# bayespy/bayespy

Measured on AMD Instinct MI355X. Metric: VB iterations/sec, PCA N=10000000 D=128 K=32, higher is better.
Workload: dtype f64

## Files before the change

### bayespy_amd/csrc/vmp_common.h

```cpp
#pragma once

#include <hip/hip_runtime.h>
#include <stdint.h>
#include <stdio.h>
#include <string.h>
#include <math.h>

#include "../../include/vmp_hip.h"

#define VMP_EV_RING 64

constexpr int VMP_NME = 16;

struct vmp_xpass_desc {
    const double *Y;
    int64_t ldy, N;
    int D, K;
    double *X;
    int64_t ldx;
    int lay;
    const double *A;
    int buf;
};

struct vmp_ctx {
    int device;
    hipStream_t stream;
    int num_cu;
    int timing;
    hipEvent_t ev[3 * VMP_EV_RING];
    int64_t ev_n;
    hipStream_t xs;
    hipEvent_t ev_xfork, ev_xdone;
    int x_pending;
    hipEvent_t ev_xbuf[2];
    int x_buf_pending[2];
    int64_t x_count;
    int xs_cus;
    int x_hold, x_held;
    vmp_xpass_desc x_desc;
    int64_t x_launched, x_superseded;
    double *sweep_ctl;
    int64_t sweeps_enqueued;
    unsigned int *sweep_tickets;
    int64_t sweep_mid_launches;
    unsigned long long *sweep_stamps;
    int sweep_stamp_rows;
    double *sweep_sf;
    double sweep_sf_key[7];
    int sweep_sf_valid;
    hipStream_t ms[3];
    hipEvent_t me[VMP_NME];
    int gram_pending;
    int gram_D, gram_K;
    double *gram_state;
    double *gram_P;
    void *comm;
    int comm_rank, comm_world;
    void *queue;
    char err[512];
};

enum { VMP_SWEEP_NSTAMP = VMP_PCA_SWEEP_NSTAMP };

enum { VMP_SWEEP_STOP = 0, VMP_SWEEP_L = 1, VMP_SWEEP_EXECUTED = 2, VMP_SWEEP_SKIPPED = 3,
       VMP_SWEEP_CTL_LEN = 8 };

enum { VMP_SWEEP_SF_TAU = 0, VMP_SWEEP_SF_ALPHA = 4, VMP_SWEEP_SF_LOG2PI = 8, VMP_SWEEP_SF_LOGXPREC = 9,
       VMP_SWEEP_SF_LEN = 10 };

struct vmp_sweep_tail {
    const double *P;
    int nb;
    double *ctl;
    double *slot;
    int first;
    int compare;
    double l0, tol;
    int norder;
    int order[8];
};

int32_t vmp_pca_sweep_covered(int32_t D, int32_t K);
int32_t vmp_pca_launch_sweep_head(vmp_ctx *ctx, int32_t D, int32_t K, int64_t n_total, double x_prec,
                                  double a0t, double b0t, double a0a, double b0a, double *state,
                                  const double *stop);
int32_t vmp_pca_launch_sweep_tail(vmp_ctx *ctx, int32_t D, int32_t K, int64_t n_total, double x_prec,
                                  double a0t, double b0t, double a0a, double b0a, double *state,
                                  const vmp_sweep_tail &t);

int32_t vmp_pca_launch_sweep_mid(vmp_ctx *ctx, int32_t D, int32_t K, int64_t n_total, double x_prec,
                                 double a0t, double b0t, double a0a, double b0a, double *state,
                                 double *P, const vmp_sweep_tail &t, unsigned int *ticket,
                                 unsigned long long *stamps, int32_t stamp_level);
int32_t vmp_pca_sweep_constants(vmp_ctx *ctx, int32_t D, int32_t K, int64_t n_total, double x_prec,
                                double a0t, double b0t, double a0a, double b0a);
int32_t vmp_pca_launch_sweep_head_wide(vmp_ctx *ctx, int32_t D, int32_t K, int64_t n_total,
                                       double x_prec, double a0t, double b0t, double a0a, double b0a,
                                       double *state);
int32_t vmp_pca_launch_gram_fast(vmp_ctx *ctx, int32_t D, int32_t K, double *state);

int32_t vmp_pca_ensure_gram(vmp_ctx *ctx);
int32_t vmp_pca_launch_held(vmp_ctx *ctx);

int32_t vmp_queue_flush(vmp_ctx *ctx);
int32_t vmp_queue_commit(vmp_ctx *ctx);
int32_t destroy_small_queue(vmp_ctx *ctx);
extern const char *vmp_flush_cause;
#define VMP_FLUSH_SMALL(ctx)                                   \
    do {                                                       \
        if ((ctx) && (ctx)->queue) {                           \
            vmp_flush_cause = __func__;                        \
            const int32_t rc__ = vmp_queue_flush(ctx);         \
            if (rc__ != VMP_OK) return rc__;                   \
        }                                                      \
    } while (0)

static inline hipEvent_t *vmp_next_events(vmp_ctx *ctx)
{
    hipEvent_t *e = ctx->ev + 3 * (ctx->ev_n % VMP_EV_RING);
    ctx->ev_n += 1;
    return e;
}

#define VMP_SET_ERR(ctx, ...)                                         \
    do {                                                              \
        if (ctx) snprintf((ctx)->err, sizeof((ctx)->err), __VA_ARGS__); \
    } while (0)

#define VMP_HIP_CHECK(ctx, expr)                                                   \
    do {                                                                           \
        hipError_t e__ = (expr);                                                   \
        if (e__ != hipSuccess) {                                                   \
            VMP_SET_ERR(ctx, "%s failed: %s (%s:%d)", #expr, hipGetErrorString(e__), \
                        __FILE__, __LINE__);                                       \
            return VMP_ERR_HIP;                                                    \
        }                                                                          \
    } while (0)

#define VMP_REQUIRE(ctx, cond, code, ...)   \
    do {                                    \
        if (!(cond)) {                      \
            VMP_SET_ERR(ctx, __VA_ARGS__);  \
            return (code);                  \
        }                                   \
    } while (0)

int vmp_tune_get(const char *key, int dflt);

typedef double v4f64 __attribute__((ext_vector_type(4)));
typedef double v2f64 __attribute__((ext_vector_type(2)));

int32_t vmp_launch_spd_mfma(vmp_ctx *ctx, bool moments, int32_t n, int64_t batch, const double *A,
                            const double *rhs, double *Ainv, double *vec_out, double *logdet,
                            int32_t *info);


__host__ __device__ inline double vmp_digamma(double x)
{
    if (!(x > 0.0)) {
        if (x == 0.0) return -INFINITY;
        double r = 1.0 - x;
        double s = 0.0;
        while (r < 10.0) { s -= 1.0 / r; r += 1.0; }
        double inv = 1.0 / r, inv2 = inv * inv;
        double ser = inv2 * (1.0 / 12 - inv2 * (1.0 / 120 - inv2 * (1.0 / 252 - inv2 * (1.0 / 240 - inv2 * (1.0 / 132 - inv2 * (691.0 / 32760 - inv2 * (1.0 / 12)))))));
        double psi1mx = s + log(r) - 0.5 * inv - ser;
        return psi1mx - M_PI / tan(M_PI * x);
    }
    double s = 0.0;
    while (x < 10.0) { s -= 1.0 / x; x += 1.0; }
    double inv = 1.0 / x, inv2 = inv * inv;
    double ser = inv2 * (1.0 / 12 - inv2 * (1.0 / 120 - inv2 * (1.0 / 252 - inv2 * (1.0 / 240 - inv2 * (1.0 / 132 - inv2 * (691.0 / 32760 - inv2 * (1.0 / 12)))))));
    return s + log(x) - 0.5 * inv - ser;
}

__host__ __device__ inline double vmp_lgamma(double x)
{
    if (!(x > 0.0)) return INFINITY;
    double shift = 0.0;
    double prod = 1.0;
    while (x < 10.0) {
        prod *= x;
        x += 1.0;
        if (prod > 1e150) { shift += log(prod); prod = 1.0; }
    }
    shift += log(prod);
    double inv = 1.0 / x, inv2 = inv * inv;
    double ser = inv * (1.0 / 12 - inv2 * (1.0 / 360 - inv2 * (1.0 / 1260 - inv2 * (1.0 / 1680 - inv2 * (1.0 / 1188 - inv2 * (691.0 / 360360 - inv2 * (1.0 / 156)))))));
    return (x - 0.5) * log(x) - x + 0.91893853320467274178 + ser - shift;
}

#if defined(__clang__)
#define VMP_NO_CONTRACT _Pragma("clang fp contract(off)")
#else
#define VMP_NO_CONTRACT
#endif

__host__ __device__ inline double vmp_two_sum(double a, double b, double *e)
{
    VMP_NO_CONTRACT
    const double s = a + b, bb = s - a;
    *e = (a - (s - bb)) + (b - bb);
    return s;
}

__host__ __device__ inline double vmp_lgamma_dd(double x, double dx, double *lo)
{
    VMP_NO_CONTRACT
    if (!(x >= 10.0) || !(x < 4e15)) {
        *lo = dx == 0.0 ? 0.0 : dx * vmp_digamma(x);
        return vmp_lgamma(x);
    }
    int e;
    double m = frexp(x, &e);
    if (m < 0.70710678118654752440) { m *= 2.0; e -= 1; }
    const double A = (double)e * 6.93147180369123816490e-01;
    const double B = (double)e * 1.90821492927058770002e-10 + log(m);
    const double w = x - 0.5;
    const double p = w * A, pe = fma(w, A, -p);
    const double q = w * B, qe = fma(w, B, -q);
    double e1, e2;
    const double s1 = vmp_two_sum(p, -x, &e1);
    const double s2 = vmp_two_sum(s1, q, &e2);
    const double inv = 1.0 / x, inv2 = inv * inv;
    const double ser = inv * (1.0 / 12 - inv2 * (1.0 / 360 - inv2 * (1.0 / 1260 - inv2 * (1.0 / 1680 - inv2 * (1.0 / 1188 - inv2 * (691.0 / 360360 - inv2 * (1.0 / 156)))))));
    const double small = ((pe + qe) + (e1 + e2)) + (0.91893853320467274178 + ser)
                         + dx * ((A + B) - 0.5 * inv);
    return vmp_two_sum(s2, small, lo);
}

__host__ __device__ inline double vmp_trigamma(double x)
{
    if (!(x > 0.0)) return (x == 0.0) ? INFINITY : NAN;
    double s = 0.0;
    while (x < 10.0) { s += 1.0 / (x * x); x += 1.0; }
    double inv = 1.0 / x, inv2 = inv * inv;
    double ser = inv * inv2 * (1.0 / 6 - inv2 * (1.0 / 30 - inv2 * (1.0 / 42 - inv2 * (1.0 / 30 - inv2 * (5.0 / 66 - inv2 * (691.0 / 2730 - inv2 * (7.0 / 6)))))));
    return s + inv + 0.5 * inv2 + ser;
}

__host__ __device__ inline double vmp_invpsi(double x)
{
    const double psi1 = -0.57721566490153286061;
    double y = x >= -2.22 ? exp(x) + 0.5 : -1.0 / (x - psi1);
    for (int i = 0; i < 5; ++i) y = y - (vmp_digamma(y) - x) / vmp_trigamma(y);
    return y;
}

#ifdef __HIPCC__
__device__ inline void logdet_accumulate(double piv, double &prod, double &ld)
{
    prod *= piv;
    if (!(prod < 1e120 && prod > 1e-120)) {
        ld += log(prod);
        prod = 1.0;
    }
}

__device__ inline double logdet_finish(double prod, double ld) { return ld + log(prod); }

__device__ inline double fast_recip(double x)
{
    double r = __builtin_amdgcn_rcp(x);
    r = r * (2.0 - x * r);
    r = r * (2.0 - x * r);
    return r;
}

__device__ inline void lds_fence()
{
    asm volatile("s_waitcnt lgkmcnt(0)" ::: "memory");
}


__device__ inline double wave_spd_inverse(double v, int D, int i, int j, bool act, double *M,
                                          double *logdet, int *bad)
{
    double ld = 0.0, prod = 1.0;
    const int l = threadIdx.x & 63;
    for (int p = 0; p < D; ++p) {
        M[l] = v;
        lds_fence();
        const double piv = M[p * D + p];
        const double ci = act ? M[i * D + p] : 0.0, rj = act ? M[p * D + j] : 0.0;
        if (!(piv > 0.0)) *bad = 1;
        logdet_accumulate(piv, prod, ld);
        const double d = fast_recip(piv);
        if (i == p) v = (j == p) ? d : rj * d;
        else if (j == p) v = -ci * d;
        else v = v - ci * rj * d;
        lds_fence();
    }
    *logdet = logdet_finish(prod, ld);
    return v;
}

__device__ __forceinline__ double exp_nonpos(double x)
{
    x = fmax(x, -800.0);
    const double k = __builtin_rint(x * 1.4426950408889634074);
    double r = __builtin_fma(k, -6.93147180369123816490e-01, x);
    r = __builtin_fma(k, -1.90821492927058770002e-10, r);
    double p = 1.0 / 479001600.0;
    p = __builtin_fma(p, r, 1.0 / 39916800.0);
    p = __builtin_fma(p, r, 1.0 / 3628800.0);
    p = __builtin_fma(p, r, 1.0 / 362880.0);
    p = __builtin_fma(p, r, 1.0 / 40320.0);
    p = __builtin_fma(p, r, 1.0 / 5040.0);
    p = __builtin_fma(p, r, 1.0 / 720.0);
    p = __builtin_fma(p, r, 1.0 / 120.0);
    p = __builtin_fma(p, r, 1.0 / 24.0);
    p = __builtin_fma(p, r, 1.0 / 6.0);
    p = __builtin_fma(p, r, 0.5);
    p = __builtin_fma(p, r, 1.0);
    p = __builtin_fma(p, r, 1.0);
    return __builtin_ldexp(p, (int)k);
}

__device__ inline double wave_sum(double v)
{
#pragma unroll
    for (int off = 32; off > 0; off >>= 1) v += __shfl_down(v, off, 64);
    return v;
}

template <int NT>
__device__ inline double block_sum(double v, double *red)
{
    v = wave_sum(v);
    __syncthreads();
    if ((threadIdx.x & 63) == 0) red[threadIdx.x >> 6] = v;
    __syncthreads();
    double s = 0.0;
#pragma unroll
    for (int i = 0; i < NT / 64; ++i) s += red[i];
    return s;
}

__device__ __forceinline__ double group16_max(double v)
{
#pragma unroll
    for (int off = 8; off > 0; off >>= 1) v = fmax(v, __shfl_xor(v, off, 16));
    return v;
}

__device__ __forceinline__ double group16_sum(double v)
{
#pragma unroll
    for (int off = 8; off > 0; off >>= 1) v += __shfl_xor(v, off, 16);
    return v;
}

template <int NT>
__device__ __forceinline__ void block_halve_sum(double *v, int tid)
{
    for (int off = NT / 2; off > 0; off >>= 1) {
        if (tid < off) v[tid] += v[tid + off];
        __syncthreads();
    }
}

struct PmmArgs {
    int64_t N, chunk;
    int D, K;
    const uint16_t *x;
    const int32_t *labels;
    const double *l, *lb;
    const double *c;
    double *part;
    double *r_out;
};

void vmp_pmm_launch_pass(vmp_ctx *ctx, int64_t nc, bool hidden, const PmmArgs &a);
#endif
```

### bayespy_amd/csrc/vmp_ctx.hip

```cpp
#include "vmp_common.h"

#include <new>

static char g_err[512] = "no context";

namespace {
struct tune_entry { char key[32]; int value; };
tune_entry g_tune[128];
int g_ntune = 0;
bool g_tune_env = false;
}

extern "C" char **environ;

static void tune_from_env()
{
    g_tune_env = true;
    for (char **e = environ; e && *e; ++e) {
        if (strncmp(*e, "VMP_TUNE_", 9) != 0) continue;
        const char *eq = strchr(*e, '=');
        if (!eq) continue;
        const size_t len = (size_t)(eq - (*e + 9));
        if (len == 0 || len >= sizeof(g_tune[0].key) || g_ntune >= (int)(sizeof(g_tune) / sizeof(g_tune[0])))
            continue;
        memcpy(g_tune[g_ntune].key, *e + 9, len);
        g_tune[g_ntune].key[len] = 0;
        g_tune[g_ntune].value = atoi(eq + 1);
        g_ntune += 1;
    }
}

int vmp_tune_get(const char *key, int dflt)
{
    if (!g_tune_env) tune_from_env();
    for (int i = 0; i < g_ntune; ++i)
        if (strcmp(g_tune[i].key, key) == 0) return g_tune[i].value;
    return dflt;
}

extern "C" {

int32_t vmp_tune_set(const char *key, int32_t value)
{
    if (!key || strlen(key) >= sizeof(g_tune[0].key)) return VMP_ERR_INVALID;
    if (!g_tune_env) tune_from_env();
    for (int i = 0; i < g_ntune; ++i)
        if (strcmp(g_tune[i].key, key) == 0) {
            g_tune[i].value = value;
            return VMP_OK;
        }
    if (g_ntune >= (int)(sizeof(g_tune) / sizeof(g_tune[0]))) return VMP_ERR_INVALID;
    strcpy(g_tune[g_ntune].key, key);
    g_tune[g_ntune].value = value;
    g_ntune += 1;
    return VMP_OK;
}

#ifndef VMP_BUILD_ID
#define VMP_BUILD_ID "unknown"
#endif
const char *vmp_version(void) { return "libvmp_hip 0.2 (gfx950) build " VMP_BUILD_ID; }

int32_t vmp_ctx_create(int32_t device, void *stream, vmp_ctx **out)
{
    if (!out) return VMP_ERR_INVALID;
    *out = nullptr;
    int ndev = 0;
    hipError_t e = hipGetDeviceCount(&ndev);
    if (e != hipSuccess || ndev <= 0) {
        snprintf(g_err, sizeof(g_err), "no HIP device visible (%s)", hipGetErrorString(e));
        return VMP_ERR_HIP;
    }
    if (device < 0 || device >= ndev) {
        snprintf(g_err, sizeof(g_err), "device %d out of range [0,%d)", device, ndev);
        return VMP_ERR_INVALID;
    }
    vmp_ctx *ctx = new (std::nothrow) vmp_ctx();
    if (!ctx) return VMP_ERR_HIP;
    ctx->device = device;
    ctx->stream = (hipStream_t)stream;
    ctx->timing = 0;
    ctx->err[0] = 0;
    for (int i = 0; i < 3 * VMP_EV_RING; ++i) ctx->ev[i] = nullptr;
    ctx->ev_n = 0;
    ctx->xs = nullptr;
    ctx->ev_xfork = ctx->ev_xdone = nullptr;
    ctx->x_pending = 0;
    ctx->x_buf_pending[0] = ctx->x_buf_pending[1] = 0;
    ctx->x_count = 0;
    ctx->ev_xbuf[0] = ctx->ev_xbuf[1] = nullptr;
    ctx->xs_cus = 0;
    ctx->x_hold = ctx->x_held = 0;
    ctx->x_launched = ctx->x_superseded = 0;
    ctx->sweep_ctl = nullptr;
    ctx->sweeps_enqueued = 0;
    ctx->sweep_tickets = nullptr;
    ctx->sweep_mid_launches = 0;
    ctx->sweep_stamps = nullptr;
    ctx->sweep_stamp_rows = 0;
    ctx->sweep_sf = nullptr;
    ctx->sweep_sf_valid = 0;
    for (int i = 0; i < 3; ++i) ctx->ms[i] = nullptr;
    for (int i = 0; i < VMP_NME; ++i) ctx->me[i] = nullptr;
    ctx->comm = nullptr;
    ctx->queue = nullptr;
    ctx->comm_rank = 0;
    ctx->comm_world = 1;
    VMP_HIP_CHECK(ctx, hipSetDevice(device));
    int cu = 0;
    VMP_HIP_CHECK(ctx, hipDeviceGetAttribute(&cu, hipDeviceAttributeMultiprocessorCount, device));
    ctx->num_cu = cu > 0 ? cu : 256;
    *out = ctx;
    return VMP_OK;
}

int32_t vmp_ctx_destroy(vmp_ctx *ctx)
{
    if (!ctx) return VMP_OK;
    (void)destroy_small_queue(ctx);
    (void)vmp_comm_destroy(ctx);
    (void)vmp_pca_launch_held(ctx);
    for (int i = 0; i < 3 * VMP_EV_RING; ++i)
        if (ctx->ev[i]) (void)hipEventDestroy(ctx->ev[i]);
    if (ctx->xs) {
        (void)hipStreamSynchronize(ctx->xs);
        (void)hipStreamDestroy(ctx->xs);
    }
    for (int i = 0; i < 3; ++i)
        if (ctx->ms[i]) {
            (void)hipStreamSynchronize(ctx->ms[i]);
            (void)hipStreamDestroy(ctx->ms[i]);
        }
    for (int i = 0; i < VMP_NME; ++i)
        if (ctx->me[i]) (void)hipEventDestroy(ctx->me[i]);
    if (ctx->sweep_ctl) (void)hipFree(ctx->sweep_ctl);
    if (ctx->sweep_tickets) (void)hipFree(ctx->sweep_tickets);
    if (ctx->sweep_stamps) (void)hipFree(ctx->sweep_stamps);
    if (ctx->sweep_sf) (void)hipFree(ctx->sweep_sf);
    if (ctx->ev_xfork) (void)hipEventDestroy(ctx->ev_xfork);
    if (ctx->ev_xdone) (void)hipEventDestroy(ctx->ev_xdone);
    for (int i = 0; i < 2; ++i)
        if (ctx->ev_xbuf[i]) (void)hipEventDestroy(ctx->ev_xbuf[i]);
    delete ctx;
    return VMP_OK;
}

int32_t vmp_ctx_set_stream(vmp_ctx *ctx, void *stream)
{
    if (!ctx) return VMP_ERR_INVALID;
    if ((hipStream_t)stream != ctx->stream) VMP_FLUSH_SMALL(ctx);
    ctx->stream = (hipStream_t)stream;
    return VMP_OK;
}

int32_t vmp_ctx_sync(vmp_ctx *ctx)
{
    if (!ctx) return VMP_ERR_INVALID;
    VMP_FLUSH_SMALL(ctx);
    {
        const int32_t rcg = vmp_pca_ensure_gram(ctx);
        if (rcg != VMP_OK) return rcg;
        const int32_t rch = vmp_pca_launch_held(ctx);
        if (rch != VMP_OK) return rch;
    }
    VMP_HIP_CHECK(ctx, hipStreamSynchronize(ctx->stream));
    if (ctx->xs) VMP_HIP_CHECK(ctx, hipStreamSynchronize(ctx->xs));
    for (int i = 0; i < 3; ++i)
        if (ctx->ms[i]) VMP_HIP_CHECK(ctx, hipStreamSynchronize(ctx->ms[i]));
    return VMP_OK;
}

int32_t vmp_ctx_num_cu(vmp_ctx *ctx) { return ctx ? ctx->num_cu : 0; }

struct vmp_graph {
    hipGraph_t graph;
    hipGraphExec_t exec;
};

int32_t vmp_graph_begin(vmp_ctx *ctx)
{
    VMP_REQUIRE(ctx, ctx, VMP_ERR_INVALID, "null context");
    VMP_REQUIRE(ctx, ctx->stream != nullptr, VMP_ERR_INVALID,
                "the legacy default stream cannot record: give the context a stream of its own");
    VMP_FLUSH_SMALL(ctx);
    VMP_HIP_CHECK(ctx, hipStreamBeginCapture(ctx->stream, hipStreamCaptureModeThreadLocal));
    return VMP_OK;
}

int32_t vmp_graph_end(vmp_ctx *ctx, void **graph)
{
    VMP_REQUIRE(ctx, ctx && graph, VMP_ERR_INVALID, "null argument");
    *graph = nullptr;
    const int32_t rcq = vmp_queue_flush(ctx);
    hipGraph_t g = nullptr;
    hipError_t e = hipStreamEndCapture(ctx->stream, &g);
    if (rcq != VMP_OK) {
        if (g) (void)hipGraphDestroy(g);
        return rcq;
    }
    VMP_HIP_CHECK(ctx, e);
    hipGraphExec_t x = nullptr;
    e = hipGraphInstantiate(&x, g, nullptr, nullptr, 0);
    if (e != hipSuccess) {
        (void)hipGraphDestroy(g);
        VMP_HIP_CHECK(ctx, e);
    }
    const int32_t rcc = vmp_queue_commit(ctx);
    if (rcc != VMP_OK) {
        (void)hipGraphExecDestroy(x);
        (void)hipGraphDestroy(g);
        return rcc;
    }
    vmp_graph *h = new (std::nothrow) vmp_graph{g, x};
    if (!h) {
        (void)hipGraphExecDestroy(x);
        (void)hipGraphDestroy(g);
        VMP_REQUIRE(ctx, false, VMP_ERR_HIP, "out of host memory");
    }
    *graph = h;
    return VMP_OK;
}

int32_t vmp_graph_launch(vmp_ctx *ctx, void *graph)
{
    VMP_REQUIRE(ctx, ctx && graph, VMP_ERR_INVALID, "null argument");
    VMP_FLUSH_SMALL(ctx);
    VMP_HIP_CHECK(ctx, hipGraphLaunch(reinterpret_cast<vmp_graph *>(graph)->exec, ctx->stream));
    return VMP_OK;
}

int32_t vmp_graph_destroy(vmp_ctx *ctx, void *graph)
{
    (void)ctx;
    if (!graph) return VMP_OK;
    vmp_graph *h = reinterpret_cast<vmp_graph *>(graph);
    (void)hipGraphExecDestroy(h->exec);
    (void)hipGraphDestroy(h->graph);
    delete h;
    return VMP_OK;
}

const char *vmp_last_error(vmp_ctx *ctx) { return ctx ? ctx->err : g_err; }

int32_t vmp_ctx_set_timing(vmp_ctx *ctx, int32_t enabled)
{
    if (!ctx) return VMP_ERR_INVALID;
    if (enabled && !ctx->ev[0]) {
        VMP_HIP_CHECK(ctx, hipSetDevice(ctx->device));
        for (int i = 0; i < 3 * VMP_EV_RING; ++i) VMP_HIP_CHECK(ctx, hipEventCreate(&ctx->ev[i]));
    }
    ctx->timing = enabled ? 1 : 0;
    ctx->ev_n = 0;
    return VMP_OK;
}

int32_t vmp_pass_times_ms(vmp_ctx *ctx, double *ms_pass, double *ms_reduce, int32_t cap,
                          int32_t *count)
{
    VMP_REQUIRE(ctx, ctx && count && cap >= 0, VMP_ERR_INVALID, "null argument");
    VMP_REQUIRE(ctx, ctx->timing && ctx->ev[0], VMP_ERR_INVALID,
                "timing not enabled (vmp_ctx_set_timing)");
    {
        const int32_t rch = vmp_pca_launch_held(ctx);
        if (rch != VMP_OK) return rch;
    }
    int64_t n = ctx->ev_n < VMP_EV_RING ? ctx->ev_n : VMP_EV_RING;
    if (n > cap) n = cap;
    for (int64_t i = 0; i < n; ++i) {
        hipEvent_t *e = ctx->ev + 3 * ((ctx->ev_n - n + i) % VMP_EV_RING);
        VMP_HIP_CHECK(ctx, hipEventSynchronize(e[2]));
        float a = 0.f, b = 0.f;
        VMP_HIP_CHECK(ctx, hipEventElapsedTime(&a, e[0], e[1]));
        VMP_HIP_CHECK(ctx, hipEventElapsedTime(&b, e[1], e[2]));
        if (ms_pass) ms_pass[i] = a;
        if (ms_reduce) ms_reduce[i] = b;
    }
    *count = (int32_t)n;
    ctx->ev_n = 0;
    return VMP_OK;
}

int32_t vmp_malloc(vmp_ctx *ctx, size_t bytes, void **ptr)
{
    if (!ctx || !ptr) return VMP_ERR_INVALID;
    VMP_HIP_CHECK(ctx, hipSetDevice(ctx->device));
    VMP_HIP_CHECK(ctx, hipMalloc(ptr, bytes ? bytes : 8));
    return VMP_OK;
}

int32_t vmp_free(vmp_ctx *ctx, void *ptr)
{
    if (!ctx) return VMP_ERR_INVALID;
    if (ptr) VMP_HIP_CHECK(ctx, hipFree(ptr));
    return VMP_OK;
}

int32_t vmp_memcpy_h2d(vmp_ctx *ctx, void *dst, const void *src, size_t bytes)
{
    VMP_FLUSH_SMALL(ctx);
    if (!ctx) return VMP_ERR_INVALID;
    VMP_HIP_CHECK(ctx, hipMemcpyAsync(dst, src, bytes, hipMemcpyHostToDevice, ctx->stream));
    VMP_HIP_CHECK(ctx, hipStreamSynchronize(ctx->stream));
    return VMP_OK;
}

int32_t vmp_memcpy_d2h(vmp_ctx *ctx, void *dst, const void *src, size_t bytes)
{
    VMP_FLUSH_SMALL(ctx);
    if (!ctx) return VMP_ERR_INVALID;
    VMP_HIP_CHECK(ctx, hipMemcpyAsync(dst, src, bytes, hipMemcpyDeviceToHost, ctx->stream));
    VMP_HIP_CHECK(ctx, hipStreamSynchronize(ctx->stream));
    return VMP_OK;
}

int32_t vmp_memset_zero(vmp_ctx *ctx, void *dst, size_t bytes)
{
    VMP_FLUSH_SMALL(ctx);
    if (!ctx) return VMP_ERR_INVALID;
    VMP_HIP_CHECK(ctx, hipMemsetAsync(dst, 0, bytes, ctx->stream));
    return VMP_OK;
}

struct CopyMany {
    const double *src[24];
    double *dst[24];
    int64_t count[24];
};

__global__ void __launch_bounds__(256) copy_many_kernel(CopyMany a)
{
    const int c = blockIdx.y;
    const double *s = a.src[c];
    double *d = a.dst[c];
    const int64_t n = a.count[c];
    for (int64_t i = (int64_t)blockIdx.x * 256 + threadIdx.x; i < n; i += (int64_t)gridDim.x * 256)
        d[i] = s[i];
}

int32_t vmp_copy_many(vmp_ctx *ctx, int32_t n, const double *const *src, double *const *dst,
                      const int64_t *count)
{
    VMP_REQUIRE(ctx, ctx != nullptr, VMP_ERR_INVALID, "null context");
    VMP_REQUIRE(ctx, n >= 0 && (n == 0 || (src && dst && count)), VMP_ERR_INVALID, "null argument");
    VMP_FLUSH_SMALL(ctx);
    for (int32_t b = 0; b < n; b += 24) {
        CopyMany a;
        memset(&a, 0, sizeof(a));
        const int m = (n - b) < 24 ? (n - b) : 24;
        int64_t most = 0;
        for (int i = 0; i < m; ++i) {
            a.src[i] = src[b + i];
            a.dst[i] = dst[b + i];
            a.count[i] = count[b + i];
            VMP_REQUIRE(ctx, a.count[i] >= 0 && (a.count[i] == 0 || (a.src[i] && a.dst[i])),
                        VMP_ERR_INVALID, "vmp_copy_many: bad entry %d", b + i);
            if (a.count[i] > most) most = a.count[i];
        }
        int64_t gx = (most + 1023) / 1024;
        if (gx < 1) gx = 1;
        if (gx > 1024) gx = 1024;
        hipLaunchKernelGGL(copy_many_kernel, dim3((unsigned)gx, (unsigned)m), dim3(256), 0,
                           ctx->stream, a);
        VMP_HIP_CHECK(ctx, hipGetLastError());
    }
    return VMP_OK;
}

struct PackArgs {
    const void *src[48];
    int64_t count[48];
    int32_t kind[48];
};

__global__ void __launch_bounds__(64) pack_outputs_kernel(PackArgs a, double *__restrict__ out,
                                                           int base)
{
    const int e = blockIdx.x;
    const int kind = a.kind[e];
    if (kind == 0) {
        if (threadIdx.x == 0) out[base + e] = *reinterpret_cast<const double *>(a.src[e]);
        return;
    }
    int bad = 0;
    const int64_t n = a.count[e];
    if (kind == 1) {
        const int32_t *f = reinterpret_cast<const int32_t *>(a.src[e]);
        for (int64_t i = threadIdx.x; i < n; i += 64) bad |= (f[i] != 0);
    } else {
        const double *f = reinterpret_cast<const double *>(a.src[e]);
        for (int64_t i = threadIdx.x; i < n; i += 64) bad |= (f[i] != 0.0);
    }
    const unsigned long long m = __ballot(bad);
    if (threadIdx.x == 0) out[base + e] = m ? 1.0 : 0.0;
}

int32_t vmp_pack_outputs(vmp_ctx *ctx, int32_t n, const void *const *src, const int64_t *count,
                         const int32_t *kind, double *out)
{
    VMP_REQUIRE(ctx, ctx != nullptr, VMP_ERR_INVALID, "null context");
    VMP_REQUIRE(ctx, n >= 0 && (n == 0 || (src && count && kind && out)), VMP_ERR_INVALID,
                "null argument");
    VMP_FLUSH_SMALL(ctx);
    for (int32_t b = 0; b < n; b += 48) {
        PackArgs a;
        memset(&a, 0, sizeof(a));
        const int m = (n - b) < 48 ? (n - b) : 48;
        for (int i = 0; i < m; ++i) {
            a.src[i] = src[b + i];
            a.count[i] = count[b + i];
            a.kind[i] = kind[b + i];
            VMP_REQUIRE(ctx, a.src[i] && a.kind[i] >= 0 && a.kind[i] <= 2 && a.count[i] >= 0,
                        VMP_ERR_INVALID, "vmp_pack_outputs: bad entry %d", b + i);
        }
        hipLaunchKernelGGL(pack_outputs_kernel, dim3((unsigned)m), dim3(64), 0, ctx->stream, a, out,
                           (int)b);
        VMP_HIP_CHECK(ctx, hipGetLastError());
    }
    return VMP_OK;
}

}
```

### bayespy_amd/csrc/vmp_pca.hip

```cpp
#include "vmp_common.h"
#include "vmp_stop_rule.h"

namespace {

constexpr int TN = 32;
constexpr int SZ = TN + 2;
constexpr int NT = 256;
constexpr int MAX_KP = 64;
constexpr int MAX_DP = 256;

inline int pow2_blocks(int x, int unit)
{
    int b = (x + unit - 1) / unit;
    int p = 1;
    while (p < b) p <<= 1;
    return p;
}

inline void fill_layout(int D, int K, vmp_pca_layout *L)
{
    const int64_t DP = 32 * pow2_blocks(D, 32);
    const int64_t KP = 16 * pow2_blocks(K, 16);
    int64_t o = 0;
    L->DP = DP;
    L->KP = KP;
    L->off_S = o;      L->len_S = (DP + KP) * KP; o += L->len_S;
    L->off_Syy = o;    o += 8;
    L->off_tau = o;    o += 8;
    L->off_alpha = o;  o += 4 * KP;
    L->off_W = o;      o += (int64_t)D * KP;
    L->off_CW = o;     o += KP * KP;
    L->off_Sww = o;    o += KP * KP;
    L->off_CX = o;     o += KP * KP;
    L->off_A = o;      o += KP * DP;
    L->off_G = o;      o += DP * DP;
    L->off_scal = o;   o += 8;
    L->off_L = o;      o += 8;
    L->off_mu = o;     o += (int64_t)D * KP;
    L->off_mstat = o;  o += 2 * KP;
    L->total = (o + 7) / 8 * 8;
}

__device__ inline v4f64 mfma_f64(double a, double b, v4f64 c)
{
    return __builtin_amdgcn_mfma_f64_16x16x4f64(a, b, c, 0, 0, 0);
}

template <int DB, int KT, bool COMPUTE_X>
__global__ void __launch_bounds__(NT, (DB >= 8 || DB * KT > 8) ? 1 : 2)
pca_pass_kernel(const double *__restrict__ Y, int64_t ldy, int64_t N, int D, int K,
                const double *__restrict__ Apad, double *__restrict__ X, int64_t ldx,
                double *__restrict__ P, int64_t ntiles)
{
    constexpr int DP = 32 * DB, KP = 16 * KT, ZR = DP + KP;
    constexpr int YP = DP / 16;
    constexpr int XP = KP / 16;
    constexpr int KS1 = DP / 4;
    constexpr int T1 = KT * (TN / 16);
    constexpr int R1 = (T1 + 3) / 4;
    constexpr int T2 = (2 * DB + KT) * KT;
    constexpr int R2 = (T2 + 3) / 4;

    __shared__ double Z[ZR * SZ];

    const int tid = threadIdx.x;
    const int w = tid >> 6, l = tid & 63;
    const int l15 = l & 15, l4 = l >> 4;
    const int lrow = tid >> 4;
    const int lcol = (tid & 15) * 2;
    const int it1 = w % KT;
    const int jt2 = w % KT;

    double afrag[COMPUTE_X ? KS1 : 1];
    if (COMPUTE_X) {
        const double *arow = Apad + (int64_t)(it1 * 16 + l15) * DP;
#pragma unroll
        for (int q = 0; q < KS1; ++q) afrag[q] = arow[32 * (q >> 3) + (q & 7) + 8 * l4];
    }

    v4f64 acc2[R2];
#pragma unroll
    for (int m = 0; m < R2; ++m) acc2[m] = v4f64{0.0, 0.0, 0.0, 0.0};

    v2f64 yreg[YP];

    auto load_tile = [&](int64_t tile) {
        const int64_t n = tile * TN + lcol;
#pragma unroll
        for (int p = 0; p < YP; ++p) {
            const int row = p * 16 + lrow;
            v2f64 v = v2f64{0.0, 0.0};
            if (row < D) {
                const double *src = Y + (int64_t)row * ldy + n;
                if (n + 1 < N) v = *reinterpret_cast<const v2f64 *>(src);
                else if (n < N) v.x = src[0];
            }
            yreg[p] = v;
        }
    };

    int64_t tile = blockIdx.x;
    if (tile < ntiles) load_tile(tile);

    for (; tile < ntiles; tile += gridDim.x) {
        const int64_t n0 = tile * TN;
#pragma unroll
        for (int p = 0; p < YP; ++p)
            *reinterpret_cast<v2f64 *>(&Z[(p * 16 + lrow) * SZ + lcol]) = yreg[p];
        if (!COMPUTE_X) {
#pragma unroll
            for (int p = 0; p < XP; ++p) {
                const int row = p * 16 + lrow;
                const int64_t n = n0 + lcol;
                v2f64 v = v2f64{0.0, 0.0};
                if (row < K) {
                    const double *src = X + (int64_t)row * ldx + n;
                    if (n + 1 < N) { v.x = src[0]; v.y = src[1]; }
                    else if (n < N) v.x = src[0];
                }
                *reinterpret_cast<v2f64 *>(&Z[(DP + row) * SZ + lcol]) = v;
            }
        }
        __syncthreads();

        const int64_t next = tile + gridDim.x;
        if (next < ntiles) load_tile(next);

        if (COMPUTE_X) {
#pragma unroll
            for (int m = 0; m < R1; ++m) {
                const int t1 = w + 4 * m;
                if (t1 < T1) {
                    const int jt = t1 / KT;
                    const double *zb = Z + jt * 16 + l15 + 8 * l4 * SZ;
                    v4f64 c0 = v4f64{0.0, 0.0, 0.0, 0.0};
                    v4f64 c1 = v4f64{0.0, 0.0, 0.0, 0.0};
#pragma unroll
                    for (int q = 0; q < KS1; q += 2) {
                        const double b0 = zb[(32 * (q >> 3) + (q & 7)) * SZ];
                        const double b1 = zb[(32 * ((q + 1) >> 3) + ((q + 1) & 7)) * SZ];
                        c0 = mfma_f64(afrag[q], b0, c0);
                        c1 = mfma_f64(afrag[q + 1], b1, c1);
                    }
                    c0 += c1;
                    const int n = jt * 16 + l15;
                    const bool nok = (n0 + n) < N;
#pragma unroll
                    for (int r = 0; r < 4; ++r) {
                        const int k = it1 * 16 + l4 + 4 * r;
                        Z[(DP + k) * SZ + n] = c0[r];
                        if (nok && k < K) X[(int64_t)k * ldx + n0 + n] = c0[r];
                    }
                }
            }
            __syncthreads();
        }

        {
            const double *zbB = Z + (DP + jt2 * 16 + l15) * SZ + l4;
            const double *zbA = Z + l15 * SZ + l4;
#pragma unroll
            for (int q = 0; q < TN / 4; ++q) {
                const double b = zbB[4 * q];
#pragma unroll
                for (int m = 0; m < R2; ++m) {
                    const int t2 = w + 4 * m;
                    if (t2 < T2) {
                        const int it2 = t2 / KT;
                        const double a = zbA[it2 * 16 * SZ + 4 * q];
                        acc2[m] = mfma_f64(a, b, acc2[m]);
                    }
                }
            }
        }
        __syncthreads();
    }

    double *Pb = P + (int64_t)blockIdx.x * (ZR * KP);
#pragma unroll
    for (int m = 0; m < R2; ++m) {
        const int t2 = w + 4 * m;
        if (t2 < T2) {
            const int it2 = t2 / KT;
#pragma unroll
            for (int r = 0; r < 4; ++r) {
                const int row = it2 * 16 + l4 + 4 * r;
                Pb[row * KP + jt2 * 16 + l15] = acc2[m][r];
            }
        }
    }
}

__global__ void __launch_bounds__(NT)
reduce_partials_kernel(const double *__restrict__ P, int nb, int len, double *__restrict__ S)
{
    const int e = blockIdx.x * NT + threadIdx.x;
    if (e >= len) return;
    double s0 = 0.0, s1 = 0.0, s2 = 0.0, s3 = 0.0;
    int b = 0;
    for (; b + 3 < nb; b += 4) {
        s0 += P[(int64_t)b * len + e];
        s1 += P[(int64_t)(b + 1) * len + e];
        s2 += P[(int64_t)(b + 2) * len + e];
        s3 += P[(int64_t)(b + 3) * len + e];
    }
    for (; b < nb; ++b) s0 += P[(int64_t)b * len + e];
    S[e] = (s0 + s1) + (s2 + s3);
}

__global__ void __launch_bounds__(NT)
sumsq_kernel(const double *__restrict__ Y, int64_t ldy, int64_t N, int D,
             double *__restrict__ partial)
{
    __shared__ double red[NT / 64];
    double s = 0.0;
    const int64_t npairs = (N + 1) / 2;
    const int64_t total = npairs * D;
    for (int64_t i = (int64_t)blockIdx.x * NT + threadIdx.x; i < total;
         i += (int64_t)gridDim.x * NT) {
        const int64_t d = i / npairs;
        const int64_t n = (i - d * npairs) * 2;
        const double *src = Y + d * ldy + n;
        if (n + 1 < N) {
            const v2f64 v = *reinterpret_cast<const v2f64 *>(src);
            s += v.x * v.x + v.y * v.y;
        } else {
            s += src[0] * src[0];
        }
    }
    s = block_sum<NT>(s, red);
    if (threadIdx.x == 0) partial[blockIdx.x] = s;
}

__global__ void __launch_bounds__(NT)
sum_partials_kernel(const double *__restrict__ partial, int n, double *__restrict__ out)
{
    __shared__ double red[NT / 64];
    double s = 0.0;
    for (int i = threadIdx.x; i < n; i += NT) s += partial[i];
    s = block_sum<NT>(s, red);
    if (threadIdx.x == 0) out[0] = s;
}

constexpr int xpass_occ(int DB, int KT, int OCC)
{
    return KT * DB * 4096 > 80 * 1024 ? 1 : (KT * DB * 4096 > 53 * 1024 ? (OCC < 2 ? OCC : 2) : OCC);
}

template <int DB, int KT, bool GUARD, int OCC, int NTM = 0, int LAY = 0, int MF = 0, bool IL = false>
__global__ void __launch_bounds__(NT, xpass_occ(DB, KT, OCC))
pca_xpass_kernel(const double *__restrict__ Y, int64_t ldy, int64_t N, int D, int K,
                 const double *__restrict__ Apad, double *__restrict__ X, int64_t ldx,
                 int64_t tile0, int64_t tile1)
{
    constexpr int DP = 32 * DB;
    constexpr int KS = DP / 4;
    constexpr int NCH = (DB < 2) ? 2 : DB;
    constexpr int CH = KS / NCH;
    constexpr bool YT = (LAY & 1) != 0, XT = (LAY & 2) != 0;
    static_assert(!(GUARD && LAY != 0), "tile-major arrays are padded: no guarded instance");

    __shared__ double Af[KT * KS * 64];

    const int tid = threadIdx.x;
    const int l = tid & 63;
    const int l15 = l & 15, l4 = l >> 4;
    const int w = __builtin_amdgcn_readfirstlane(tid >> 6);

    for (int e = tid; e < KT * KS * 64; e += NT) {
        const int lane = e & 63, fq = e >> 6;
        const int it = fq / KS, q = fq - it * KS;
        Af[e] = Apad[(int64_t)(it * 16 + (lane & 15)) * DP + 4 * q + (lane >> 4)];
    }
    __syncthreads();

    const double *Afl = MF ? Af + 16 * l4 + (l & 3) : Af + l;
    const uint32_t yoff = (uint32_t)(((int64_t)l4 * ldy + 2 * l15) * 8);
    const uint32_t xoff = (uint32_t)(((int64_t)l4 * ldx + 2 * l15) * 8);

    v2f64 buf[2][CH];
    const int64_t stride = (int64_t)gridDim.x * 4;

    auto issue = [&](int64_t tile, int c, v2f64 *dst) {
        if (YT) {
            const char *base = reinterpret_cast<const char *>(Y)
                               + ((tile * ((DP + (IL ? 16 * KT : 0)) * TN)
                                   + (int64_t)(c * CH) * (4 * TN)) << 3);
#pragma unroll
            for (int i = 0; i < CH; ++i) {
                const v2f64 *src = reinterpret_cast<const v2f64 *>(base + i * (4 * TN * 8) + l * 16);
                dst[i] = (NTM & 1) ? __builtin_nontemporal_load(src) : *src;
            }
            return;
        }
        const char *base = reinterpret_cast<const char *>(Y)
                           + ((tile * TN + (int64_t)(4 * c * CH) * ldy) << 3);
        if (!GUARD) {
#pragma unroll
            for (int i = 0; i < CH; ++i) {
                const v2f64 *src = reinterpret_cast<const v2f64 *>(
                    base + ((int64_t)(4 * i) * ldy << 3) + yoff);
                dst[i] = (NTM & 1) ? __builtin_nontemporal_load(src) : *src;
            }
        } else {
            const int64_t n = tile * TN + 2 * l15;
#pragma unroll
            for (int i = 0; i < CH; ++i) {
                const int row = 4 * (c * CH + i) + l4;
                v2f64 v = v2f64{0.0, 0.0};
                if (row < D) {
                    const double *src = reinterpret_cast<const double *>(
                        base + ((int64_t)(4 * i) * ldy << 3) + yoff);
                    if (n + 1 < N) v = *reinterpret_cast<const v2f64 *>(src);
                    else if (n < N) v.x = src[0];
                }
                dst[i] = v;
            }
        }
    };

    constexpr bool STG = false;
    auto first_chunk = [&](int64_t t) { return STG ? (int)(t & (NCH - 1)) : 0; };
    int64_t tile = tile0 + (int64_t)blockIdx.x * 4 + w;
    if (tile < tile1) issue(tile, first_chunk(tile), buf[0]);

    for (; tile < tile1; tile += stride) {
        v4f64 acc[KT][2];
#pragma unroll
        for (int it = 0; it < KT; ++it) {
            acc[it][0] = v4f64{0.0, 0.0, 0.0, 0.0};
            acc[it][1] = v4f64{0.0, 0.0, 0.0, 0.0};
        }
        const int rot = first_chunk(tile);
#pragma unroll
        for (int c = 0; c < NCH; ++c) {
            const int cc = STG ? ((c + rot) & (NCH - 1)) : c;
            if (c + 1 < NCH) issue(tile, STG ? ((c + 1 + rot) & (NCH - 1)) : c + 1, buf[(c + 1) & 1]);
            else if (tile + stride < tile1) issue(tile + stride, first_chunk(tile + stride), buf[(c + 1) & 1]);
            asm volatile("" ::: "memory");
            const double *Afc = Afl + cc * (CH * 64);
#pragma unroll
            for (int i = 0; i < CH; ++i) {
                const v2f64 b = buf[c & 1][i];
#pragma unroll
                for (int it = 0; it < KT; ++it) {
                    if (MF) {
#pragma unroll
                        for (int R = 0; R < 4; ++R) {
                            const double a = Afc[(it * KS + i) * 64 + 4 * R];
                            acc[it][0][R] = __builtin_amdgcn_mfma_f64_4x4x4f64(a, b.x, acc[it][0][R], 0, 0, 0);
                            acc[it][1][R] = __builtin_amdgcn_mfma_f64_4x4x4f64(a, b.y, acc[it][1][R], 0, 0, 0);
                        }
                    } else {
                        const double a = Afc[(it * KS + i) * 64];
                        acc[it][0] = mfma_f64(a, b.x, acc[it][0]);
                        acc[it][1] = mfma_f64(a, b.y, acc[it][1]);
                    }
                }
            }
        }
        char *xbase = reinterpret_cast<char *>(X) + ((tile * TN) << 3);
        if (XT) {
            char *xt = reinterpret_cast<char *>(X)
                       + ((tile * (((IL ? DP : 0) + 16 * KT) * TN)) << 3) + l * 16;
#pragma unroll
            for (int it = 0; it < KT; ++it)
#pragma unroll
                for (int r = 0; r < 4; ++r) {
                    v2f64 *dstp = reinterpret_cast<v2f64 *>(xt + (it * 16 + 4 * r) * (TN * 8));
                    const v2f64 val = v2f64{acc[it][0][r], acc[it][1][r]};
                    if (NTM & 2) __builtin_nontemporal_store(val, dstp);
                    else *dstp = val;
                }
        } else if (!GUARD) {
#pragma unroll
            for (int it = 0; it < KT; ++it)
#pragma unroll
                for (int r = 0; r < 4; ++r) {
                    v2f64 *dstp = reinterpret_cast<v2f64 *>(
                        xbase + ((int64_t)(it * 16 + 4 * r) * ldx << 3) + xoff);
                    const v2f64 val = v2f64{acc[it][0][r], acc[it][1][r]};
                    if (NTM & 2) __builtin_nontemporal_store(val, dstp);
                    else *dstp = val;
                }
        } else {
            const int64_t n = tile * TN + 2 * l15;
#pragma unroll
            for (int it = 0; it < KT; ++it) {
#pragma unroll
                for (int r = 0; r < 4; ++r) {
                    const int k = it * 16 + l4 + 4 * r;
                    if (k < K) {
                        double *dst = reinterpret_cast<double *>(
                            xbase + ((int64_t)(it * 16 + 4 * r) * ldx << 3) + xoff);
                        if (n + 1 < N)
                            *reinterpret_cast<v2f64 *>(dst) = v2f64{acc[it][0][r], acc[it][1][r]};
                        else if (n < N)
                            dst[0] = acc[it][0][r];
                    }
                }
            }
        }
    }
}

constexpr int LD = MAX_KP + 1;

__global__ void __launch_bounds__(NT)
pca_init_state_kernel(vmp_pca_layout L, int K, double a0t, double b0t, double a0a, double b0a,
                      double *st)
{
    const int tid = threadIdx.x;
    if (tid == 0) {
        st[L.off_tau + 0] = a0t;
        st[L.off_tau + 1] = b0t;
        st[L.off_tau + 2] = a0t / b0t;
        st[L.off_tau + 3] = vmp_digamma(a0t) - log(b0t);
    }
    for (int k = tid; k < K; k += NT) {
        st[L.off_alpha + 0 * L.KP + k] = a0a;
        st[L.off_alpha + 1 * L.KP + k] = b0a;
        st[L.off_alpha + 2 * L.KP + k] = a0a / b0a;
        st[L.off_alpha + 3 * L.KP + k] = vmp_digamma(a0a) - log(b0a);
    }
}

constexpr int GR = 8;
__global__ void __launch_bounds__(NT)
pca_gram_stats_kernel(vmp_pca_layout L, int D, int K, const double *__restrict__ st_in,
                      double *__restrict__ st, double *__restrict__ P, const double *stop)
{
    extern __shared__ double lds[];
    if (stop && stop[VMP_SWEEP_STOP] != 0.0) return;
    const int DP = (int)L.DP, KP = (int)L.KP;
    const int LA = DP + 1;
    double *As = lds;
    double *Gs = As + KP * LA;
    double *Ss = Gs + GR * DP;
    const int tid = threadIdx.x;
    const int r0 = blockIdx.x * GR;
    const double *A = st_in + L.off_A;
    const double *G = st_in + L.off_G;
    for (int e = tid; e < K * DP; e += NT) {
        const int k = e / DP, d = e - k * DP;
        As[k * LA + d] = A[(int64_t)k * DP + d];
    }
    for (int e = tid; e < GR * DP; e += NT) Gs[e] = G[(int64_t)r0 * DP + e];
    __syncthreads();
    for (int e = tid; e < GR * K; e += NT) {
        const int r = e / K, k = e - r * K;
        double s = 0.0;
        for (int d = 0; d < D; ++d) s += Gs[r * DP + d] * As[k * LA + d];
        Ss[r * LD + k] = s;
        if (r0 + r < D) st[L.off_S + (int64_t)(r0 + r) * KP + k] = s;
    }
    __syncthreads();
    double *Pb = P + (int64_t)blockIdx.x * KP * KP;
    for (int e = tid; e < KP * KP; e += NT) {
        const int k = e / KP, k2 = e - k * KP;
        double s = 0.0;
        if (k < K && k2 < K) {
#pragma unroll
            for (int r = 0; r < GR; ++r) s += As[k * LA + r0 + r] * Ss[r * LD + k2];
        }
        Pb[e] = s;
    }
}

__global__ void __launch_bounds__(NT)
pca_gram_copy_kernel(const double *__restrict__ Stmp, int KPx, int D, int Kx, int j0, int DP,
                     double *__restrict__ G)
{
    const int e = blockIdx.x * NT + threadIdx.x;
    if (e >= D * Kx) return;
    const int i = e / Kx, j = e - i * Kx;
    G[(int64_t)i * DP + j0 + j] = Stmp[(int64_t)i * KPx + j];
}

int env_int(const char *name, int dflt, int lo, int hi)
{
    const char *e = getenv(name);
    int v = e ? atoi(e) : dflt;
    if (v < lo) v = lo;
    if (v > hi) v = hi;
    return v;
}

int wgs_per_cu()
{
    static int v = -1;
    if (v < 0) v = env_int("VMP_PCA_WGS_PER_CU", 2, 1, 8);
    return v;
}

int pca_interleave() { return vmp_tune_get("pca_interleave", 0); }

int xpass_wgs_per_cu()
{
    static int v = -1;
    if (v < 0) v = env_int("VMP_PCA_XPASS_WGS_PER_CU", 3, 1, 8);
    return vmp_tune_get("xpass_wgs_per_cu", v);
}

int xpass_occupancy()
{
    static int v = -1;
    if (v < 0) v = env_int("VMP_PCA_XPASS_OCC", 3, 2, 3);
    return vmp_tune_get("xpass_occ", v);
}

int64_t max_grid(vmp_ctx *ctx) { return (int64_t)ctx->num_cu * wgs_per_cu(); }

int64_t partial_len(const vmp_pca_layout &L) { return (L.DP + MAX_KP) * MAX_KP; }

template <int DB, int KT>
void launch_fused(bool compute_x, dim3 grid, hipStream_t s, const double *Y, int64_t ldy,
                  int64_t N, int D, int K, const double *A, double *X, int64_t ldx, double *P,
                  int64_t ntiles)
{
    if (compute_x)
        hipLaunchKernelGGL((pca_pass_kernel<DB, KT, true>), grid, dim3(NT), 0, s, Y, ldy, N, D, K,
                           A, X, ldx, P, ntiles);
    else
        hipLaunchKernelGGL((pca_pass_kernel<DB, KT, false>), grid, dim3(NT), 0, s, Y, ldy, N, D,
                           K, A, X, ldx, P, ntiles);
}

#define VMP_FOR_EACH_INSTANCE(M)                                       \
    M(1, 1) M(2, 1) M(4, 1) M(8, 1) M(1, 2) M(2, 2) M(4, 2) M(8, 2)    \
    M(1, 4) M(2, 4) M(4, 4) M(8, 4)

int32_t check_pass_args(vmp_ctx *ctx, const void *Y, const void *X, const void *state,
                        const void *workspace, int64_t ldy, int64_t ldx, int64_t N, int D, int K)
{
    VMP_REQUIRE(ctx, ctx != nullptr, VMP_ERR_INVALID, "null context");
    VMP_REQUIRE(ctx, Y && X && state && workspace, VMP_ERR_INVALID, "null pointer argument");
    VMP_REQUIRE(ctx, D >= 1 && K >= 1 && N >= 0, VMP_ERR_INVALID, "bad dims D=%d K=%d N=%lld", D,
                K, (long long)N);
    VMP_REQUIRE(ctx, D <= MAX_DP && K <= MAX_KP, VMP_ERR_UNSUPPORTED,
                "fused PCA block supports D <= %d, K <= %d (got D=%d, K=%d)", MAX_DP, MAX_KP, D, K);
    VMP_REQUIRE(ctx, ldy >= N && ldx >= N, VMP_ERR_INVALID, "leading dimension smaller than N");
    VMP_REQUIRE(ctx, (ldy % 2) == 0 && ((uintptr_t)Y % 16) == 0, VMP_ERR_INVALID,
                "Y must be 16-byte aligned with an even leading dimension (ldy=%lld)",
                (long long)ldy);
    VMP_REQUIRE(ctx, (ldx % 2) == 0 && ((uintptr_t)X % 16) == 0, VMP_ERR_INVALID,
                "X must be 16-byte aligned with an even leading dimension (ldx=%lld)",
                (long long)ldx);
    VMP_REQUIRE(ctx, ldy < (int64_t)170000000 && ldx < (int64_t)170000000, VMP_ERR_UNSUPPORTED,
                "leading dimension >= 1.7e8 elements per shard is not supported "
                "(32-bit lane offsets); shard the plate over more ranks");
    return VMP_OK;
}

int32_t run_stats(vmp_ctx *ctx, bool compute_x, const double *Y, int64_t ldy, int64_t N, int D,
                  int Kx, double *Xs, int64_t ldx, const double *A, double *out_S, double *P,
                  bool timed)
{
    vmp_pca_layout Lx;
    fill_layout(D, Kx, &Lx);
    const int DB = (int)(Lx.DP / 32), KT = (int)(Lx.KP / 16);
    const int64_t ntiles = (N + TN - 1) / TN;
    int64_t g = ntiles < max_grid(ctx) ? ntiles : max_grid(ctx);
    if (g < 1) g = 1;
    hipStream_t s = ctx->stream;
    dim3 grid((unsigned)g);
    hipEvent_t *ev = (timed && ctx->timing) ? vmp_next_events(ctx) : nullptr;
    if (ev) VMP_HIP_CHECK(ctx, hipEventRecord(ev[0], s));
#define VMP_CASE(db, kt)                                                                     \
    if (DB == db && KT == kt)                                                                \
        launch_fused<db, kt>(compute_x, grid, s, Y, ldy, N, D, Kx, A, Xs, ldx, P, ntiles);   \
    else
    VMP_FOR_EACH_INSTANCE(VMP_CASE)
    {
        VMP_SET_ERR(ctx, "no kernel instance for DB=%d KT=%d", DB, KT);
        return VMP_ERR_UNSUPPORTED;
    }
#undef VMP_CASE
    VMP_HIP_CHECK(ctx, hipGetLastError());
    if (ev) VMP_HIP_CHECK(ctx, hipEventRecord(ev[1], s));
    const int len = (int)Lx.len_S;
    hipLaunchKernelGGL(reduce_partials_kernel, dim3((len + NT - 1) / NT), dim3(NT), 0, s, P,
                       (int)g, len, out_S);
    VMP_HIP_CHECK(ctx, hipGetLastError());
    if (ev) VMP_HIP_CHECK(ctx, hipEventRecord(ev[2], s));
    return VMP_OK;
}

int32_t ensure_plate_stream(vmp_ctx *ctx)
{
    if (ctx->xs) return VMP_OK;
    static const int reserve = env_int("VMP_PCA_RESERVE_CUS", 0, 0, 64);
    hipStream_t xs = nullptr;
    const int ncu = ctx->num_cu;
    ctx->xs_cus = ncu;
    if (reserve > 0 && ncu > 2 * reserve) {
        const int words = (ncu + 31) / 32;
        uint32_t mask[64];
        for (int w = 0; w < words && w < 64; ++w) mask[w] = 0;
        for (int c = 0; c < ncu; ++c) mask[c >> 5] |= (1u << (c & 31));
        const int step = ncu / reserve;
        for (int r = 0; r < reserve; ++r) {
            const int c = r * step + step / 2;
            mask[c >> 5] &= ~(1u << (c & 31));
        }
        if (hipExtStreamCreateWithCUMask(&xs, (uint32_t)words, mask) != hipSuccess) {
            (void)hipGetLastError();
            xs = nullptr;
        } else {
            ctx->xs_cus = ncu - reserve;
        }
    }
    if (!xs) VMP_HIP_CHECK(ctx, hipStreamCreateWithFlags(&xs, hipStreamNonBlocking));
    ctx->xs = xs;
    VMP_HIP_CHECK(ctx, hipEventCreateWithFlags(&ctx->ev_xfork, hipEventDisableTiming));
    VMP_HIP_CHECK(ctx, hipEventCreateWithFlags(&ctx->ev_xdone, hipEventDisableTiming));
    for (int i = 0; i < 2; ++i)
        VMP_HIP_CHECK(ctx, hipEventCreateWithFlags(&ctx->ev_xbuf[i], hipEventDisableTiming));
    return VMP_OK;
}

int64_t plate_stream_A_offset(vmp_ctx *ctx, const vmp_pca_layout &L)
{
    return (max_grid(ctx) + 1) * partial_len(L) + 4096;
}

double *plate_stream_A(vmp_ctx *ctx, const vmp_pca_layout &L, void *workspace)
{
    return reinterpret_cast<double *>(workspace) + plate_stream_A_offset(ctx, L);
}

int32_t join_plate_stream(vmp_ctx *ctx)
{
    const int32_t rc = vmp_pca_launch_held(ctx);
    if (rc != VMP_OK) return rc;
    if (ctx->x_pending) {
        VMP_HIP_CHECK(ctx, hipStreamWaitEvent(ctx->stream, ctx->ev_xdone, 0));
        ctx->x_pending = 0;
    }
    return VMP_OK;
}

int32_t run_gram_stats(vmp_ctx *ctx, const vmp_pca_layout &L, int D, int K, double *state,
                       double *P, hipStream_t s, const double *stop = nullptr, bool reduce = true)
{
    const int nb = (int)(L.DP / GR);
    const size_t lds = ((size_t)L.KP * (L.DP + 1) + (size_t)GR * L.DP + (size_t)GR * LD)
                       * sizeof(double);
    static bool attr_set = false;
    if (!attr_set) {
        VMP_HIP_CHECK(ctx, hipFuncSetAttribute((const void *)pca_gram_stats_kernel,
                                               hipFuncAttributeMaxDynamicSharedMemorySize,
                                               160 * 1024));
        attr_set = true;
    }
    hipLaunchKernelGGL(pca_gram_stats_kernel, dim3(nb), dim3(NT), lds, s, L, D, K, state, state,
                       P, stop);
    VMP_HIP_CHECK(ctx, hipGetLastError());
    if (!reduce) return VMP_OK;
    const int len = (int)(L.KP * L.KP);
    hipLaunchKernelGGL(reduce_partials_kernel, dim3((len + NT - 1) / NT), dim3(NT), 0, s, P, nb,
                       len, state + L.off_S + L.DP * L.KP);
    VMP_HIP_CHECK(ctx, hipGetLastError());
    return VMP_OK;
}

template <bool TO_TILED>
__global__ void __launch_bounds__(NT)
pca_tile_kernel(double *__restrict__ R, int64_t ld, int64_t N, int rows, int RP,
                double *__restrict__ T, int64_t ntiles, int64_t tstride)
{
    const int tid = threadIdx.x;
    const int c2 = (tid & 15) * 2;
    for (int64_t tile = blockIdx.x; tile < ntiles; tile += gridDim.x) {
        const int64_t n = tile * TN + c2;
        double *tb = T + tile * tstride;
        for (int row = tid >> 4; row < RP; row += NT / 16) {
            double *rp = R + (int64_t)row * ld + n;
            v2f64 *tp = reinterpret_cast<v2f64 *>(tb + row * TN + c2);
            if (TO_TILED) {
                v2f64 v = v2f64{0.0, 0.0};
                if (row < rows) {
                    if (n + 1 < N) v = *reinterpret_cast<const v2f64 *>(rp);
                    else if (n < N) v.x = rp[0];
                }
                *tp = v;
            } else if (row < rows) {
                const v2f64 v = *tp;
                if (n + 1 < N) *reinterpret_cast<v2f64 *>(rp) = v;
                else if (n < N) rp[0] = v.x;
            }
        }
    }
}

int32_t launch_xpass(vmp_ctx *ctx, const vmp_xpass_desc &d, bool on_plate)
{
    const double *Y = d.Y, *A = d.A;
    double *X = d.X;
    const int64_t ldy = d.ldy, N = d.N, ldx = d.ldx;
    const int D = d.D, K = d.K, lay = d.lay;
    vmp_pca_layout L;
    fill_layout(D, K, &L);
    const int DB = (int)(L.DP / 32), KT = (int)(L.KP / 16);
    const int64_t ntiles = (N + TN - 1) / TN;
    const bool exact = (D == L.DP && K == L.KP);
    const bool padded = (ldy >= ntiles * TN && ldx >= ntiles * TN);
    const int64_t nfast = lay ? ntiles : (exact ? (padded ? ntiles : N / TN) : 0);
    const int occ = xpass_occupancy();
    const int ntm = vmp_tune_get("xpass_nt", env_int("VMP_PCA_XPASS_NT", 3, 0, 3));
    const int mf4 = vmp_tune_get("xpass_mfma4", env_int("VMP_PCA_XPASS_MFMA4", 0, 0, 1));
    hipStream_t s = on_plate ? ctx->xs : ctx->stream;
    const int64_t gmax = (int64_t)(on_plate ? ctx->xs_cus : ctx->num_cu) * xpass_wgs_per_cu();
    hipEvent_t *ev = ctx->timing ? vmp_next_events(ctx) : nullptr;
    if (ev) VMP_HIP_CHECK(ctx, hipEventRecord(ev[0], s));
    for (int pass = 0; pass < 2; ++pass) {
        const bool guard = (pass == 1);
        const int64_t t0 = guard ? nfast : 0, t1 = guard ? ntiles : nfast;
        if (t1 <= t0) continue;
        int64_t g = (t1 - t0 + 3) / 4;
        if (g > gmax) g = gmax;
        const dim3 grid((unsigned)g);
#define VMP_XP(db, kt, gd, oc, nt, ly)                                                          \
    hipLaunchKernelGGL((pca_xpass_kernel<db, kt, gd, oc, nt, ly>), grid, dim3(NT), 0, s, Y, ldy, \
                       N, D, K, A, X, ldx, t0, t1)
#define VMP_XP4(db, kt, oc, ly)                                                                  \
    hipLaunchKernelGGL((pca_xpass_kernel<db, kt, false, oc, 3, ly, 1>), grid, dim3(NT), 0, s, Y,  \
                       ldy, N, D, K, A, X, ldx, t0, t1)
        if (lay == 3 && pca_interleave()) {
            if (DB == 4 && KT == 2)
                hipLaunchKernelGGL((pca_xpass_kernel<4, 2, false, 3, 3, 3, 0, true>), grid, dim3(NT),
                                   0, s, Y, ldy, N, D, K, A, X, ldx, t0, t1);
            else if (DB == 2 && KT == 1)
                hipLaunchKernelGGL((pca_xpass_kernel<2, 1, false, 3, 3, 3, 0, true>), grid, dim3(NT),
                                   0, s, Y, ldy, N, D, K, A, X, ldx, t0, t1);
            else {
                VMP_SET_ERR(ctx, "pca_interleave: no instance for DB=%d KT=%d", DB, KT);
                return VMP_ERR_UNSUPPORTED;
            }
            VMP_HIP_CHECK(ctx, hipGetLastError());
            continue;
        }
#define VMP_CASE(db, kt)                                                                        \
    if (DB == db && KT == kt) {                                                                 \
        if (guard) VMP_XP(db, kt, true, 2, 0, 0);                                               \
        else if (mf4 && lay == 1 && ntm == 3) VMP_XP4(db, kt, 2, 1);                            \
        else if (mf4 && lay == 0 && ntm == 3) VMP_XP4(db, kt, 2, 0);                            \
        else if (lay == 3 && kt < 4 && ntm == 3) VMP_XP(db, kt, false, 3, 3, 3);                \
        else if (lay == 3 && kt < 4) VMP_XP(db, kt, false, 3, 0, 3);                            \
        else if (lay == 3) VMP_XP(db, kt, false, 2, 0, 3);                                      \
        else if (lay == 1 && kt < 4 && ntm == 3) VMP_XP(db, kt, false, 3, 3, 1);                \
        else if (lay == 1 && kt < 4) VMP_XP(db, kt, false, 3, 0, 1);                            \
        else if (lay == 1) VMP_XP(db, kt, false, 2, 0, 1);                                      \
        else if (ntm == 3 && kt < 4) VMP_XP(db, kt, false, 3, 3, 0);                            \
        else if (occ >= 3 && kt < 4) VMP_XP(db, kt, false, 3, 0, 0);                            \
        else VMP_XP(db, kt, false, 2, 0, 0);                                                    \
    } else
        VMP_FOR_EACH_INSTANCE(VMP_CASE)
        {
            VMP_SET_ERR(ctx, "no kernel instance for DB=%d KT=%d", DB, KT);
            return VMP_ERR_UNSUPPORTED;
        }
#undef VMP_CASE
#undef VMP_XP4
#undef VMP_XP
        VMP_HIP_CHECK(ctx, hipGetLastError());
    }
    if (ev) {
        VMP_HIP_CHECK(ctx, hipEventRecord(ev[1], s));
        VMP_HIP_CHECK(ctx, hipEventRecord(ev[2], s));
    }
    if (on_plate) {
        VMP_HIP_CHECK(ctx, hipEventRecord(ctx->ev_xdone, s));
        ctx->x_pending = 1;
        VMP_HIP_CHECK(ctx, hipEventRecord(ctx->ev_xbuf[d.buf], s));
        ctx->x_buf_pending[d.buf] = 1;
    }
    ctx->x_launched += 1;
    return VMP_OK;
}

int64_t xpass_written_cols(const vmp_xpass_desc &d)
{
    vmp_pca_layout L;
    fill_layout(d.D, d.K, &L);
    const int64_t whole = (d.N + TN - 1) / TN * TN;
    const bool exact = (d.D == L.DP && d.K == L.KP);
    return (d.lay || (exact && d.ldy >= whole && d.ldx >= whole)) ? whole : d.N;
}

bool xpass_supersedes(const vmp_xpass_desc &d, const vmp_xpass_desc &old)
{
    return d.X == old.X && d.N == old.N && d.D == old.D && d.K == old.K && d.ldx == old.ldx &&
           d.lay == old.lay && xpass_written_cols(d) >= xpass_written_cols(old);
}

int32_t issue_xpass(vmp_ctx *ctx, const double *Y, int64_t ldy, int64_t N, int D, int K, double *X,
                    int64_t ldx, double *state, void *workspace, int lay)
{
    int32_t rc;
    vmp_pca_layout L;
    fill_layout(D, K, &L);
    hipStream_t m = ctx->stream;
    const int overlap = vmp_tune_get("plate_stream", env_int("VMP_PCA_PLATE_STREAM", 1, 0, 1));
    vmp_xpass_desc d = {Y, ldy, N, D, K, X, ldx, lay, state + L.off_A, -1};
    if (!overlap) {
        rc = join_plate_stream(ctx);
        if (rc != VMP_OK) return rc;
    } else {
        rc = ensure_plate_stream(ctx);
        if (rc != VMP_OK) return rc;
        if (ctx->x_held) {
            if (xpass_supersedes(d, ctx->x_desc)) {
                ctx->x_held = 0;
                ctx->x_superseded += 1;
            } else {
                rc = vmp_pca_launch_held(ctx);
                if (rc != VMP_OK) return rc;
            }
        }
        const int b = (int)(ctx->x_count & 1);
        ctx->x_count += 1;
        double *Ax = plate_stream_A(ctx, L, workspace) + (int64_t)b * L.KP * L.DP;
        if (ctx->x_buf_pending[b]) {
            VMP_HIP_CHECK(ctx, hipStreamWaitEvent(m, ctx->ev_xbuf[b], 0));
            ctx->x_buf_pending[b] = 0;
        }
        VMP_HIP_CHECK(ctx, hipMemcpyAsync(Ax, state + L.off_A,
                                          (size_t)(L.KP * L.DP) * sizeof(double),
                                          hipMemcpyDeviceToDevice, m));
        VMP_HIP_CHECK(ctx, hipEventRecord(ctx->ev_xfork, m));
        VMP_HIP_CHECK(ctx, hipStreamWaitEvent(ctx->xs, ctx->ev_xfork, 0));
        d.A = Ax;
        d.buf = b;
    }
    if (overlap && ctx->x_hold) {
        ctx->x_desc = d;
        ctx->x_held = 1;
    } else {
        rc = launch_xpass(ctx, d, overlap != 0);
        if (rc != VMP_OK) return rc;
    }
    return VMP_OK;
}

int32_t run_xpass(vmp_ctx *ctx, const double *Y, int64_t ldy, int64_t N, int D, int K, double *X,
                  int64_t ldx, double *state, void *workspace, int lay)
{
    int32_t rc = issue_xpass(ctx, Y, ldy, N, D, K, X, ldx, state, workspace, lay);
    if (rc != VMP_OK) return rc;
    vmp_pca_layout L;
    fill_layout(D, K, &L);
    hipStream_t m = ctx->stream;
    if (vmp_tune_get("pca_fuse_gram", env_int("VMP_PCA_FUSE_GRAM", 0, 0, 1)) && L.KP <= 32 &&
        D <= 128) {
        ctx->gram_pending = 1;
        ctx->gram_D = D;
        ctx->gram_K = K;
        ctx->gram_state = state;
        ctx->gram_P = reinterpret_cast<double *>(workspace);
        return VMP_OK;
    }
    return run_gram_stats(ctx, L, D, K, state, reinterpret_cast<double *>(workspace), m);
}

}

int32_t vmp_pca_launch_held(vmp_ctx *ctx)
{
    if (!ctx || !ctx->x_held) return VMP_OK;
    ctx->x_held = 0;
    return launch_xpass(ctx, ctx->x_desc, true);
}

int32_t vmp_pca_ensure_gram(vmp_ctx *ctx)
{
    if (!ctx || !ctx->gram_pending) return VMP_OK;
    ctx->gram_pending = 0;
    vmp_pca_layout L;
    fill_layout(ctx->gram_D, ctx->gram_K, &L);
    return run_gram_stats(ctx, L, ctx->gram_D, ctx->gram_K, ctx->gram_state, ctx->gram_P,
                          ctx->stream);
}

extern "C" {

int32_t vmp_pca_get_layout(int32_t D, int32_t K, vmp_pca_layout *out)
{
    if (!out || D < 1 || K < 1) return VMP_ERR_INVALID;
    if (D > MAX_DP || K > MAX_KP) return VMP_ERR_UNSUPPORTED;
    fill_layout(D, K, out);
    return VMP_OK;
}

int32_t vmp_pca_workspace_bytes(vmp_ctx *ctx, int32_t D, int32_t K, size_t *bytes)
{
    VMP_REQUIRE(ctx, ctx && bytes, VMP_ERR_INVALID, "null argument");
    VMP_REQUIRE(ctx, D >= 1 && K >= 1, VMP_ERR_INVALID, "bad dims");
    VMP_REQUIRE(ctx, D <= MAX_DP && K <= MAX_KP, VMP_ERR_UNSUPPORTED,
                "fused PCA block supports D <= %d, K <= %d", MAX_DP, MAX_KP);
    vmp_pca_layout L;
    fill_layout(D, K, &L);
    *bytes = (size_t)(plate_stream_A_offset(ctx, L) + 2 * L.KP * L.DP) * sizeof(double);
    return VMP_OK;
}

int32_t vmp_pca_init_state(vmp_ctx *ctx, int32_t D, int32_t K, double a0_tau, double b0_tau,
                           double a0_alpha, double b0_alpha, double *state)
{
    VMP_REQUIRE(ctx, ctx && state, VMP_ERR_INVALID, "null argument");
    vmp_pca_layout L;
    int32_t rc = vmp_pca_get_layout(D, K, &L);
    VMP_REQUIRE(ctx, rc == VMP_OK, rc, "unsupported dims D=%d K=%d", D, K);
    VMP_REQUIRE(ctx, a0_tau > 0 && b0_tau > 0 && a0_alpha > 0 && b0_alpha > 0, VMP_ERR_INVALID,
                "Gamma prior parameters must be positive");
    VMP_HIP_CHECK(ctx, hipMemsetAsync(state, 0, (size_t)L.total * sizeof(double), ctx->stream));
    hipLaunchKernelGGL(pca_init_state_kernel, dim3(1), dim3(NT), 0, ctx->stream, L, K, a0_tau,
                       b0_tau, a0_alpha, b0_alpha, state);
    VMP_HIP_CHECK(ctx, hipGetLastError());
    return VMP_OK;
}

int32_t vmp_pca_syy(vmp_ctx *ctx, const double *Y, int64_t ldy, int64_t N, int32_t D, int32_t K,
                    double *state, void *workspace)
{
    VMP_REQUIRE(ctx, ctx && Y && state && workspace, VMP_ERR_INVALID, "null argument");
    VMP_REQUIRE(ctx, (ldy % 2) == 0 && ((uintptr_t)Y % 16) == 0 && ldy >= N, VMP_ERR_INVALID,
                "Y must be 16-byte aligned with an even leading dimension >= N");
    vmp_pca_layout L;
    int32_t rc = vmp_pca_get_layout(D, K, &L);
    VMP_REQUIRE(ctx, rc == VMP_OK, rc, "unsupported dims D=%d K=%d", D, K);
    double *partial = reinterpret_cast<double *>(workspace);
    int64_t work = ((N + 1) / 2) * D;
    int64_t g = (work + NT - 1) / NT;
    if (g > 2048) g = 2048;
    if (g < 1) g = 1;
    hipLaunchKernelGGL(sumsq_kernel, dim3((unsigned)g), dim3(NT), 0, ctx->stream, Y, ldy, N, D,
                       partial);
    hipLaunchKernelGGL(sum_partials_kernel, dim3(1), dim3(NT), 0, ctx->stream, partial, (int)g,
                       state + L.off_Syy);
    VMP_HIP_CHECK(ctx, hipGetLastError());
    return VMP_OK;
}

int32_t vmp_pca_gram(vmp_ctx *ctx, const double *Y, int64_t ldy, int64_t N, int32_t D, int32_t K,
                     double *state, void *workspace)
{
    if (ctx) ctx->gram_pending = 0;
    int32_t rc = check_pass_args(ctx, Y, Y, state, workspace, ldy, ldy, N, D, K);
    if (rc != VMP_OK) return rc;
    vmp_pca_layout L;
    fill_layout(D, K, &L);
    double *P = reinterpret_cast<double *>(workspace);
    double *tmpS = P + max_grid(ctx) * partial_len(L);
    for (int j0 = 0; j0 < D; j0 += MAX_KP) {
        const int Kx = (D - j0) < MAX_KP ? (D - j0) : MAX_KP;
        vmp_pca_layout Lx;
        fill_layout(D, Kx, &Lx);
        double *Xs = const_cast<double *>(Y) + (int64_t)j0 * ldy;
        rc = run_stats(ctx, false, Y, ldy, N, D, Kx, Xs, ldy, state + L.off_A, tmpS, P, false);
        if (rc != VMP_OK) return rc;
        const int n = D * Kx;
        hipLaunchKernelGGL(pca_gram_copy_kernel, dim3((n + NT - 1) / NT), dim3(NT), 0, ctx->stream,
                           tmpS, (int)Lx.KP, D, Kx, j0, (int)L.DP, state + L.off_G);
        VMP_HIP_CHECK(ctx, hipGetLastError());
    }
    return VMP_OK;
}

int32_t vmp_pca_stats_from_x(vmp_ctx *ctx, const double *Y, int64_t ldy, int64_t N, int32_t D,
                             int32_t K, const double *X, int64_t ldx, double *state,
                             void *workspace)
{
    if (ctx) ctx->gram_pending = 0;
    int32_t rc = check_pass_args(ctx, Y, X, state, workspace, ldy, ldx, N, D, K);
    if (rc != VMP_OK) return rc;
    vmp_pca_layout L;
    fill_layout(D, K, &L);
    rc = join_plate_stream(ctx);
    if (rc != VMP_OK) return rc;
    return run_stats(ctx, false, Y, ldy, N, D, K, const_cast<double *>(X), ldx, state + L.off_A,
                     state + L.off_S, reinterpret_cast<double *>(workspace), false);
}

int32_t vmp_pca_pass(vmp_ctx *ctx, const double *Y, int64_t ldy, int64_t N, int32_t D, int32_t K,
                     double *X, int64_t ldx, double *state, void *workspace)
{
    if (ctx) ctx->gram_pending = 0;
    int32_t rc = check_pass_args(ctx, Y, X, state, workspace, ldy, ldx, N, D, K);
    if (rc != VMP_OK) return rc;
    vmp_pca_layout L;
    fill_layout(D, K, &L);
    rc = join_plate_stream(ctx);
    if (rc != VMP_OK) return rc;
    return run_stats(ctx, true, Y, ldy, N, D, K, X, ldx, state + L.off_A, state + L.off_S,
                     reinterpret_cast<double *>(workspace), true);
}

int32_t vmp_pca_xpass(vmp_ctx *ctx, const double *Y, int64_t ldy, int64_t N, int32_t D, int32_t K,
                      double *X, int64_t ldx, double *state, void *workspace)
{
    int32_t rc = check_pass_args(ctx, Y, X, state, workspace, ldy, ldx, N, D, K);
    if (rc != VMP_OK) return rc;
    return run_xpass(ctx, Y, ldy, N, D, K, X, ldx, state, workspace, 0);
}

int32_t vmp_pca_tiled_doubles(int32_t D, int32_t K, int64_t N, int64_t *y_doubles,
                              int64_t *x_doubles)
{
    if (D < 1 || K < 1 || N < 0) return VMP_ERR_INVALID;
    if (D > MAX_DP || K > MAX_KP) return VMP_ERR_UNSUPPORTED;
    vmp_pca_layout L;
    fill_layout(D, K, &L);
    const int64_t ntiles = (N + TN - 1) / TN;
    if (y_doubles) *y_doubles = ntiles * (L.DP + (pca_interleave() ? L.KP : 0)) * TN;
    if (x_doubles) *x_doubles = ntiles * L.KP * TN;
    return VMP_OK;
}

int32_t vmp_pca_tile_y(vmp_ctx *ctx, const double *Y, int64_t ldy, int64_t N, int32_t D, int32_t K,
                       double *Yt)
{
    VMP_REQUIRE(ctx, ctx && Y && Yt, VMP_ERR_INVALID, "null argument");
    VMP_REQUIRE(ctx, (ldy % 2) == 0 && ((uintptr_t)Y % 16) == 0 && ((uintptr_t)Yt % 16) == 0
                && ldy >= N, VMP_ERR_INVALID,
                "Y must be 16-byte aligned with an even leading dimension >= N");
    vmp_pca_layout L;
    int32_t rc = vmp_pca_get_layout(D, K, &L);
    VMP_REQUIRE(ctx, rc == VMP_OK, rc, "unsupported dims D=%d K=%d", D, K);
    const int64_t ntiles = (N + TN - 1) / TN;
    if (ntiles == 0) return VMP_OK;
    int64_t g = ntiles < (int64_t)ctx->num_cu * 16 ? ntiles : (int64_t)ctx->num_cu * 16;
    hipLaunchKernelGGL(pca_tile_kernel<true>, dim3((unsigned)g), dim3(NT), 0, ctx->stream,
                       const_cast<double *>(Y), ldy, N, D, (int)L.DP, Yt, ntiles,
                       (int64_t)(L.DP + (pca_interleave() ? L.KP : 0)) * TN);
    VMP_HIP_CHECK(ctx, hipGetLastError());
    return VMP_OK;
}

int32_t vmp_pca_tile_x(vmp_ctx *ctx, int32_t to_tiled, double *X, int64_t ldx, int64_t N,
                       int32_t D, int32_t K, double *Xt)
{
    VMP_REQUIRE(ctx, ctx && X && Xt, VMP_ERR_INVALID, "null argument");
    VMP_REQUIRE(ctx, (ldx % 2) == 0 && ((uintptr_t)X % 16) == 0 && ((uintptr_t)Xt % 16) == 0
                && ldx >= N, VMP_ERR_INVALID,
                "X must be 16-byte aligned with an even leading dimension >= N");
    vmp_pca_layout L;
    int32_t rc = vmp_pca_get_layout(D, K, &L);
    VMP_REQUIRE(ctx, rc == VMP_OK, rc, "unsupported dims D=%d K=%d", D, K);
    rc = join_plate_stream(ctx);
    if (rc != VMP_OK) return rc;
    const int64_t ntiles = (N + TN - 1) / TN;
    if (ntiles == 0) return VMP_OK;
    int64_t g = ntiles < (int64_t)ctx->num_cu * 16 ? ntiles : (int64_t)ctx->num_cu * 16;
    const int64_t xts = (int64_t)(L.KP + (pca_interleave() ? L.DP : 0)) * TN;
    if (to_tiled)
        hipLaunchKernelGGL(pca_tile_kernel<true>, dim3((unsigned)g), dim3(NT), 0, ctx->stream, X,
                           ldx, N, K, (int)L.KP, Xt, ntiles, xts);
    else
        hipLaunchKernelGGL(pca_tile_kernel<false>, dim3((unsigned)g), dim3(NT), 0, ctx->stream, X,
                           ldx, N, K, (int)L.KP, Xt, ntiles, xts);
    VMP_HIP_CHECK(ctx, hipGetLastError());
    return VMP_OK;
}

int32_t vmp_pca_xpass_tiled(vmp_ctx *ctx, const double *Yt, int64_t N, int32_t D, int32_t K,
                            double *X, int64_t ldx, int32_t x_tiled, double *state,
                            void *workspace)
{
    VMP_REQUIRE(ctx, ctx != nullptr, VMP_ERR_INVALID, "null context");
    VMP_REQUIRE(ctx, Yt && X && state && workspace, VMP_ERR_INVALID, "null pointer argument");
    VMP_REQUIRE(ctx, D >= 1 && K >= 1 && N >= 0, VMP_ERR_INVALID, "bad dims D=%d K=%d N=%lld", D,
                K, (long long)N);
    VMP_REQUIRE(ctx, D <= MAX_DP && K <= MAX_KP, VMP_ERR_UNSUPPORTED,
                "fused PCA block supports D <= %d, K <= %d (got D=%d, K=%d)", MAX_DP, MAX_KP, D, K);
    VMP_REQUIRE(ctx, ((uintptr_t)Yt % 16) == 0 && ((uintptr_t)X % 16) == 0, VMP_ERR_INVALID,
                "tile-major arrays must be 16-byte aligned");
    const int64_t ntiles = (N + TN - 1) / TN;
    if (!x_tiled) {
        VMP_REQUIRE(ctx, (ldx % 2) == 0 && ldx >= ntiles * TN, VMP_ERR_INVALID,
                    "row-major X beside a tile-major Y needs KP rows of an even leading "
                    "dimension >= 32 ceil(N/32) (ldx=%lld)", (long long)ldx);
        VMP_REQUIRE(ctx, ldx < (int64_t)170000000, VMP_ERR_UNSUPPORTED,
                    "leading dimension >= 1.7e8 elements per shard is not supported");
    }
    return run_xpass(ctx, Yt, 0, N, D, K, X, ldx, state, workspace, x_tiled ? 3 : 1);
}

int32_t vmp_pca_xjoin(vmp_ctx *ctx)
{
    {
        const int32_t rcg = vmp_pca_ensure_gram(ctx);
        if (rcg != VMP_OK) return rcg;
    }
    VMP_REQUIRE(ctx, ctx, VMP_ERR_INVALID, "null argument");
    return join_plate_stream(ctx);
}

int32_t vmp_pca_hold_passes(vmp_ctx *ctx, int32_t on)
{
    VMP_REQUIRE(ctx, ctx, VMP_ERR_INVALID, "null argument");
    if (on) {
        if (vmp_tune_get("pca_hold_passes", env_int("VMP_PCA_HOLD_PASSES", 1, 0, 1)))
            ctx->x_hold = 1;
        return VMP_OK;
    }
    ctx->x_hold = 0;
    return vmp_pca_launch_held(ctx);
}

int32_t vmp_pca_pass_counts(vmp_ctx *ctx, int64_t *launched, int64_t *superseded)
{
    VMP_REQUIRE(ctx, ctx, VMP_ERR_INVALID, "null argument");
    if (launched) *launched = ctx->x_launched;
    if (superseded) *superseded = ctx->x_superseded;
    return VMP_OK;
}

int32_t vmp_pca_sweeps(vmp_ctx *ctx, int32_t D, int32_t K, int64_t n_total, double x_prec,
                       double a0_tau, double b0_tau, double a0_alpha, double b0_alpha,
                       const double *Y, int64_t ldy, int64_t N, double *X, int64_t ldx, int32_t lay,
                       double *state, void *workspace, int32_t n, double *ring, double tol,
                       int32_t compare, double l0, int32_t norder, const int32_t *order)
{
    VMP_REQUIRE(ctx, ctx != nullptr, VMP_ERR_INVALID, "null context");
    if (!vmp_tune_get("pca_sweeps", env_int("VMP_PCA_SWEEPS", 1, 0, 1)))
        return VMP_PCA_SWEEPS_NOT_BUILT;
    if (vmp_pca_sweep_covered(D, K) != VMP_OK) return VMP_PCA_SWEEPS_NOT_BUILT;
    VMP_REQUIRE(ctx, ring && order, VMP_ERR_INVALID, "null pointer argument");
    VMP_REQUIRE(ctx, n >= 1 && n <= VMP_PCA_MAX_SWEEPS, VMP_ERR_INVALID,
                "between 1 and %d sweeps per call", VMP_PCA_MAX_SWEEPS);
    VMP_REQUIRE(ctx, norder >= 1 && norder <= VMP_BOUND_MAX_ORDER, VMP_ERR_INVALID,
                "between 1 and %d bound terms", VMP_BOUND_MAX_ORDER);
    for (int i = 0; i < norder; ++i)
        VMP_REQUIRE(ctx, order[i] >= -1 && order[i] < VMP_BOUND_TERMS, VMP_ERR_INVALID,
                    "bound term %d out of range", order[i]);
    VMP_REQUIRE(ctx, lay == 0 || lay == 1 || lay == 3, VMP_ERR_INVALID, "unknown layout %d", lay);
    VMP_REQUIRE(ctx, x_prec > 0 && a0_tau > 0 && b0_tau > 0 && a0_alpha > 0 && b0_alpha > 0,
                VMP_ERR_INVALID, "x_prec and the Gamma prior parameters must be positive");
    int32_t rc;
    if (lay == 0) {
        rc = check_pass_args(ctx, Y, X, state, workspace, ldy, ldx, N, D, K);
        if (rc != VMP_OK) return rc;
    } else {
        VMP_REQUIRE(ctx, Y && X && state && workspace && N >= 0, VMP_ERR_INVALID,
                    "null pointer argument");
        VMP_REQUIRE(ctx, ((uintptr_t)Y % 16) == 0 && ((uintptr_t)X % 16) == 0, VMP_ERR_INVALID,
                    "tile-major arrays must be 16-byte aligned");
        if (lay == 1)
            VMP_REQUIRE(ctx, (ldx % 2) == 0 && ldx >= (N + TN - 1) / TN * TN && ldx < (int64_t)170000000,
                        VMP_ERR_INVALID, "row-major X beside a tile-major Y needs KP rows of an even "
                        "leading dimension >= 32 ceil(N/32) (ldx=%lld)", (long long)ldx);
    }
    rc = vmp_pca_ensure_gram(ctx);
    if (rc != VMP_OK) return rc;
    if (!ctx->sweep_ctl) {
        VMP_HIP_CHECK(ctx, hipMalloc(&ctx->sweep_ctl, VMP_SWEEP_CTL_LEN * sizeof(double)));
        VMP_HIP_CHECK(ctx, hipMemsetAsync(ctx->sweep_ctl, 0, VMP_SWEEP_CTL_LEN * sizeof(double),
                                          ctx->stream));
    }
    vmp_pca_layout L;
    fill_layout(D, K, &L);
    double *P = reinterpret_cast<double *>(workspace);
    vmp_sweep_tail t;
    t.P = P;
    t.nb = (int)(L.DP / GR);
    t.ctl = ctx->sweep_ctl;
    t.compare = compare ? 1 : 0;
    t.l0 = l0;
    t.tol = tol;
    t.norder = norder;
    for (int i = 0; i < 8; ++i) t.order[i] = i < norder ? order[i] : -1;
    const bool ticket = n > 1 && ((uintptr_t)state % 16) == 0 &&
                        vmp_tune_get("pca_sweep_ticket", env_int("VMP_PCA_SWEEP_TICKET", 1, 0, 1));
    if (ticket) {
        rc = vmp_pca_sweep_constants(ctx, D, K, n_total, x_prec, a0_tau, b0_tau, a0_alpha, b0_alpha);
        if (rc != VMP_OK) return rc;
    }
    const int stamp_level = ticket ? vmp_tune_get("pca_sweep_stamps", 0) : 0;
    const bool stamps = stamp_level != 0;
    if (stamps) {
        const size_t bytes = (size_t)VMP_PCA_MAX_SWEEPS * VMP_SWEEP_NSTAMP * sizeof(unsigned long long);
        if (!ctx->sweep_stamps) VMP_HIP_CHECK(ctx, hipMalloc(&ctx->sweep_stamps, bytes));
        VMP_HIP_CHECK(ctx, hipMemsetAsync(ctx->sweep_stamps, 0,
                                          (size_t)(n - 1) * VMP_SWEEP_NSTAMP * sizeof(unsigned long long),
                                          ctx->stream));
        ctx->sweep_stamp_rows = n - 1;
    }
    if (ticket) {
        if (!ctx->sweep_tickets) {
            VMP_HIP_CHECK(ctx, hipMalloc(&ctx->sweep_tickets,
                                         VMP_PCA_MAX_SWEEPS * sizeof(unsigned int)));
            VMP_HIP_CHECK(ctx, hipMemsetAsync(ctx->sweep_tickets, 0,
                                              VMP_PCA_MAX_SWEEPS * sizeof(unsigned int), ctx->stream));
        }
    }
    bool head_wide = ticket;
    if (head_wide && ctx->x_pending) {
        head_wide = hipEventQuery(ctx->ev_xdone) == hipSuccess;
        (void)hipGetLastError();
    }
    for (int i = 0; i < n; ++i) {
        const double *stop = i == 0 ? nullptr : ctx->sweep_ctl;
        const bool last = i + 1 == n;
        if (i == 0 && head_wide) {
            rc = vmp_pca_launch_sweep_head_wide(ctx, D, K, n_total, x_prec, a0_tau, b0_tau, a0_alpha,
                                                b0_alpha, state);
            if (rc != VMP_OK) return rc;
        } else if (!ticket || i == 0) {
            rc = vmp_pca_launch_sweep_head(ctx, D, K, n_total, x_prec, a0_tau, b0_tau, a0_alpha,
                                           b0_alpha, state, stop);
            if (rc != VMP_OK) return rc;
        }
        if (last) {
            rc = issue_xpass(ctx, Y, ldy, N, D, K, X, ldx, state, workspace, lay);
            if (rc != VMP_OK) return rc;
        } else {
            ctx->x_superseded += 1;
        }
        t.slot = ring + (int64_t)i * VMP_PCA_SWEEP_SLOT;
        t.first = i == 0;
        if (ticket && !last) {
            rc = vmp_pca_launch_sweep_mid(ctx, D, K, n_total, x_prec, a0_tau, b0_tau, a0_alpha,
                                          b0_alpha, state, P, t, ctx->sweep_tickets + i,
                                          stamps ? ctx->sweep_stamps + (size_t)i * VMP_SWEEP_NSTAMP
                                                 : nullptr, stamp_level);
            if (rc != VMP_OK) return rc;
            ctx->sweep_mid_launches += 1;
        } else {
            rc = run_gram_stats(ctx, L, D, K, state, P, ctx->stream, stop, false);
            if (rc != VMP_OK) return rc;
            rc = vmp_pca_launch_sweep_tail(ctx, D, K, n_total, x_prec, a0_tau, b0_tau, a0_alpha,
                                           b0_alpha, state, t);
            if (rc != VMP_OK) return rc;
        }
        ctx->sweeps_enqueued += 1;
    }
    return VMP_OK;
}

int32_t vmp_pca_sweep_counts(vmp_ctx *ctx, int64_t *enqueued, int64_t *executed, int64_t *skipped)
{
    VMP_REQUIRE(ctx, ctx, VMP_ERR_INVALID, "null argument");
    double c[VMP_SWEEP_CTL_LEN] = {0.0};
    if (ctx->sweep_ctl) {
        VMP_HIP_CHECK(ctx, hipStreamSynchronize(ctx->stream));
        VMP_HIP_CHECK(ctx, hipMemcpy(c, ctx->sweep_ctl, sizeof(c), hipMemcpyDeviceToHost));
    }
    if (enqueued) *enqueued = ctx->sweeps_enqueued;
    if (executed) *executed = (int64_t)c[VMP_SWEEP_EXECUTED];
    if (skipped) *skipped = (int64_t)c[VMP_SWEEP_SKIPPED];
    return VMP_OK;
}

int32_t vmp_pca_sweep_mid_count(vmp_ctx *ctx, int64_t *launches)
{
    VMP_REQUIRE(ctx, ctx && launches, VMP_ERR_INVALID, "null argument");
    *launches = ctx->sweep_mid_launches;
    return VMP_OK;
}

int32_t vmp_pca_sweep_stamps(vmp_ctx *ctx, uint64_t *out, int32_t max_rows, int32_t *rows,
                             int32_t *allocated)
{
    VMP_REQUIRE(ctx, ctx && rows && max_rows >= 0 && (out || max_rows == 0), VMP_ERR_INVALID,
                "null argument");
    if (allocated) *allocated = ctx->sweep_stamps ? 1 : 0;
    *rows = 0;
    if (!ctx->sweep_stamps) return VMP_OK;
    const int n = ctx->sweep_stamp_rows < max_rows ? ctx->sweep_stamp_rows : max_rows;
    if (n > 0) {
        VMP_HIP_CHECK(ctx, hipStreamSynchronize(ctx->stream));
        VMP_HIP_CHECK(ctx, hipMemcpy(out, ctx->sweep_stamps,
                                     (size_t)n * VMP_SWEEP_NSTAMP * sizeof(unsigned long long),
                                     hipMemcpyDeviceToHost));
    }
    *rows = n;
    return VMP_OK;
}

int32_t vmp_pca_gram_stats_form(vmp_ctx *ctx, int32_t D, int32_t K, double *state, void *workspace,
                                int32_t form)
{
    VMP_REQUIRE(ctx, ctx && state && workspace, VMP_ERR_INVALID, "null argument");
    vmp_pca_layout L;
    const int32_t rc = vmp_pca_get_layout(D, K, &L);
    VMP_REQUIRE(ctx, rc == VMP_OK, rc, "unsupported dims D=%d K=%d", D, K);
    double *P = reinterpret_cast<double *>(workspace);
    if (form == 0) return run_gram_stats(ctx, L, D, K, state, P, ctx->stream, nullptr, false);
    VMP_REQUIRE(ctx, form == 1, VMP_ERR_INVALID, "form %d (0 or 1)", form);
    return vmp_pca_launch_gram_fast(ctx, D, K, state);
}

int32_t vmp_pca_last_pass_ms(vmp_ctx *ctx, double *ms_pass, double *ms_reduce)
{
    VMP_REQUIRE(ctx, ctx != nullptr, VMP_ERR_INVALID, "null argument");
    {
        const int32_t rch = vmp_pca_launch_held(ctx);
        if (rch != VMP_OK) return rch;
    }
    VMP_REQUIRE(ctx, ctx->timing && ctx->ev[0] && ctx->ev_n > 0, VMP_ERR_INVALID,
                "no timed pass (vmp_ctx_set_timing)");
    hipEvent_t *e = ctx->ev + 3 * ((ctx->ev_n - 1) % VMP_EV_RING);
    VMP_HIP_CHECK(ctx, hipEventSynchronize(e[2]));
    float a = 0.f, b = 0.f;
    VMP_HIP_CHECK(ctx, hipEventElapsedTime(&a, e[0], e[1]));
    VMP_HIP_CHECK(ctx, hipEventElapsedTime(&b, e[1], e[2]));
    if (ms_pass) *ms_pass = a;
    if (ms_reduce) *ms_reduce = b;
    return VMP_OK;
}

}
```

### bayespy_amd/csrc/vmp_pca_small.hip

```cpp
#include "vmp_common.h"
#include "vmp_sweep.h"
#include "vmp_stop_rule.h"

#include <stdlib.h>
#include <string.h>
#include <type_traits>

namespace {


struct small_args {
    vmp_pca_layout L;
    int D, K;
    double n_total, x_prec, a0t, b0t, a0a, b0a;
    int has_mean;
};

__device__ inline double ww_centred(const small_args &a, const double *st, int k)
{
    const vmp_pca_layout &L = a.L;
    double v = st[L.off_Sww + k * L.KP + k];
    if (a.has_mean) v += st[L.off_mstat + L.KP + k] - 2.0 * st[L.off_mstat + k];
    return v;
}

__device__ inline double sxx_total(const double *st, const vmp_pca_layout &L, double n_total,
                                   int i, int j)
{
    const double *S = st + L.off_S;
    const double m = 0.5 * (S[(L.DP + i) * L.KP + j] + S[(L.DP + j) * L.KP + i]);
    return n_total * st[L.off_CX + i * L.KP + j] + m;
}

__device__ __noinline__ double sf_lgamma(double x) { return vmp_lgamma(x); }
__device__ __noinline__ double sf_digamma(double x) { return vmp_digamma(x); }
__device__ __noinline__ double sf_log(double x) { return log(x); }

template <int KP, int NTQ>
__device__ void gj_inverse(double *M, int n, double *logdet, int *bad)
{
    constexpr int LDM = KP + 1;
    constexpr int E = KP * KP / NTQ;
    const int tid = threadIdx.x;
    double ld = 0.0, prod = 1.0;
    int isbad = 0;
#pragma unroll 1
    for (int p = 0; p < n; ++p) {
        __syncthreads();
        const double piv = M[p * LDM + p];
        double ci[E], rj[E], me[E];
#pragma unroll
        for (int m = 0; m < E; ++m) {
            const int e = tid + m * NTQ;
            const int i = e / KP, j = e % KP;
            ci[m] = M[i * LDM + p];
            rj[m] = M[p * LDM + j];
            me[m] = M[i * LDM + j];
        }
        if (!(piv > 0.0)) isbad = 1;
        prod *= piv;
        if (!(prod < 1e120 && prod > 1e-120)) {
            ld += sf_log(prod);
            prod = 1.0;
        }
        const double d = fast_recip(piv);
        __syncthreads();
#pragma unroll
        for (int m = 0; m < E; ++m) {
            const int e = tid + m * NTQ;
            const int i = e / KP, j = e % KP;
            double v;
            if (i == p) v = (j == p) ? d : rj[m] * d;
            else if (j == p) v = -ci[m] * d;
            else v = me[m] - ci[m] * rj[m] * d;
            M[i * LDM + j] = v;
        }
    }
    __syncthreads();
    if (tid == 0) {
        *logdet = ld + sf_log(prod);
        if (isbad) *bad = 1;
    }
    __syncthreads();
}

struct no_side {
    __device__ __forceinline__ void operator()() const {}
};
template <int KP, class SIDE = no_side>
__device__ __forceinline__ void sweep_inverse(double *M, int n, double *logdet, int *bad,
                                              const SIDE &side = SIDE())
{
    static_assert(KP == 16 || KP == 32, "one 32 x 32 register tile set");
    constexpr int LDM = KP + 1;
    __syncthreads();
    if (threadIdx.x < 64) {
        const int l = threadIdx.x, l15 = l & 15, l4 = l >> 4;
        v4f64 T[2][2];
#pragma unroll
        for (int tr = 0; tr < 2; ++tr)
#pragma unroll
            for (int tc = 0; tc < 2; ++tc)
#pragma unroll
                for (int r = 0; r < 4; ++r) {
                    const int row = 16 * tr + l4 + 4 * r, col = 16 * tc + l15;
                    T[tr][tc][r] = (row < KP && col < KP) ? M[row * LDM + col]
                                                          : (row == col ? 1.0 : 0.0);
                }
        double prod = 1.0, ld = 0.0;
        int isbad = 0;
        vmp_sweep::sweep_upto<0>(T, (n + 3) / 4, l15, l4, prod, ld, isbad);
#pragma unroll
        for (int tr = 0; tr < KP / 16; ++tr)
#pragma unroll
            for (int tc = 0; tc < KP / 16; ++tc)
#pragma unroll
                for (int r = 0; r < 4; ++r) {
                    const int row = 16 * tr + l4 + 4 * r, col = 16 * tc + l15;
                    M[row * LDM + col] = (row < 4 * ((n + 3) / 4) && col < 4 * ((n + 3) / 4))
                                             ? -T[tr][tc][r] : T[tr][tc][r];
                }
        if (l == 0) {
            *logdet = vmp_sweep::sweep_logdet(prod, ld);
            if (isbad) *bad = 1;
        }
    } else {
        side();
    }
    __syncthreads();
}

enum { SP_ENTRY = 0, SP_LDS_FILLED, SP_SYX, SP_PXX, SP_TICKET, SP_ACQUIRE,
       SP_T_PARTIALS, SP_T_LOADS, SP_T_PXX, SP_T_BLOCKSUMS, SP_T_TAU_ALPHA, SP_T_BOUND, SP_T_RING,
       SP_H_LAMBDA, SP_H_INV1, SP_H_W, SP_H_SWW, SP_H_INV2, SP_H_A, SP_COUNT,
       SP_S_STATE = SP_COUNT, SP_S_RING, SP_COUNT2 };
static_assert(SP_COUNT2 <= VMP_SWEEP_NSTAMP, "stamp row length");
struct stamps_off {
    __device__ __forceinline__ void operator()(int) const {}
    __device__ __forceinline__ void side(int) const {}
    __device__ __forceinline__ void drain() const {}
};
struct stamps_on {
    unsigned long long *t;
    int level;
    __device__ __forceinline__ void operator()(int i) const
    {
        if (threadIdx.x == 0) t[i] = wall_clock64();
    }
    __device__ __forceinline__ void side(int i) const
    {
        if (level >= 2 && threadIdx.x == 64) t[i] = wall_clock64();
    }
    __device__ __forceinline__ void drain() const { asm volatile("s_waitcnt vmcnt(0)" ::: "memory"); }
};

template <int KP, int NTQ>
struct small_lds {
    static constexpr int LDM = KP + 1;
    static constexpr int RB = (KP == 64) ? 16 : 32;
    double M[KP * LDM];
    double Sb[RB * LDM];
    double Wb[RB * LDM];
    double red[NTQ / 64 + 1];
    double logdet;
    int bad;
};

template <int KP, int NTQ>
__device__ void op_update_w(const small_args &a, double *st, small_lds<KP, NTQ> &s)
{
    constexpr int LDM = KP + 1, RB = small_lds<KP, NTQ>::RB, E = KP * KP / NTQ;
    const vmp_pca_layout &L = a.L;
    const int tid = threadIdx.x, D = a.D, K = a.K;
    const double tau = st[L.off_tau + 2];
#pragma unroll
    for (int m = 0; m < E; ++m) {
        const int e = tid + m * NTQ;
        const int i = e / KP, j = e % KP;
        double v = (i == j) ? 1.0 : 0.0;
        if (i < K && j < K) {
            v = tau * sxx_total(st, L, a.n_total, i, j);
            if (i == j) v += st[L.off_alpha + 2 * KP + i];
        }
        s.M[i * LDM + j] = v;
    }
    gj_inverse<KP, NTQ>(s.M, K, &s.logdet, &s.bad);
#pragma unroll
    for (int m = 0; m < E; ++m) {
        const int e = tid + m * NTQ;
        const int i = e / KP, j = e % KP;
        if (i < K && j < K) st[L.off_CW + i * KP + j] = s.M[i * LDM + j];
    }
    const double *Syx = st + L.off_S;
    double *W = st + L.off_W;
    double sw[E];
#pragma unroll
    for (int m = 0; m < E; ++m) sw[m] = 0.0;
    for (int r0 = 0; r0 < D; r0 += RB) {
        const int nr = (D - r0) < RB ? (D - r0) : RB;
        __syncthreads();
#pragma unroll 1
        for (int e = tid; e < RB * KP; e += NTQ) {
            const int r = e / KP, k = e % KP;
            double v = (r < nr && k < K) ? Syx[(r0 + r) * KP + k] : 0.0;
            if (a.has_mean && r < nr && k < K)
                v = tau * v + st[L.off_alpha + 2 * KP + k] * st[L.off_mu + (r0 + r) * KP + k];
            s.Sb[r * LDM + k] = v;
        }
        __syncthreads();
#pragma unroll 1
        for (int e = tid; e < RB * KP; e += NTQ) {
            const int r = e / KP, k = e % KP;
            double acc = 0.0;
            if (k < K)
#pragma unroll 4
                for (int j = 0; j < K; ++j) acc += s.Sb[r * LDM + j] * s.M[j * LDM + k];
            if (!a.has_mean) acc *= tau;
            s.Wb[r * LDM + k] = acc;
            if (r < nr && k < K) W[(r0 + r) * KP + k] = acc;
        }
        __syncthreads();
#pragma unroll
        for (int m = 0; m < E; ++m) {
            const int e = tid + m * NTQ;
            const int i = e / KP, j = e % KP;
            double acc = 0.0;
#pragma unroll 4
            for (int r = 0; r < RB; ++r) acc += s.Wb[r * LDM + i] * s.Wb[r * LDM + j];
            sw[m] += acc;
        }
    }
#pragma unroll
    for (int m = 0; m < E; ++m) {
        const int e = tid + m * NTQ;
        const int i = e / KP, j = e % KP;
        if (i < K && j < K)
            st[L.off_Sww + i * KP + j] = (double)D * s.M[i * LDM + j] + sw[m];
    }
    if (tid == 0) st[L.off_scal + 0] = s.logdet;
    if (a.has_mean) {
        __threadfence_block();
        __syncthreads();
        for (int k = tid; k < K; k += NTQ) {
            double m1 = 0.0, m2 = 0.0;
            for (int d = 0; d < D; ++d) {
                const double mu = st[L.off_mu + d * KP + k];
                m1 += mu * W[d * KP + k];
                m2 += mu * mu;
            }
            st[L.off_mstat + k] = m1;
            st[L.off_mstat + KP + k] = m2;
        }
    }
}

template <int KP, int NTQ>
__device__ void op_prepare_x(const small_args &a, double *st, small_lds<KP, NTQ> &s)
{
    constexpr int LDM = KP + 1, RB = small_lds<KP, NTQ>::RB, E = KP * KP / NTQ;
    const vmp_pca_layout &L = a.L;
    const int tid = threadIdx.x, D = a.D, K = a.K;
    const int DP = (int)L.DP;
    const double tau = st[L.off_tau + 2];
#pragma unroll
    for (int m = 0; m < E; ++m) {
        const int e = tid + m * NTQ;
        const int i = e / KP, j = e % KP;
        double v = (i == j) ? 1.0 : 0.0;
        if (i < K && j < K) {
            v = tau * 0.5 * (st[L.off_Sww + i * KP + j] + st[L.off_Sww + j * KP + i]);
            if (i == j) v += a.x_prec;
        }
        s.M[i * LDM + j] = v;
    }
    gj_inverse<KP, NTQ>(s.M, K, &s.logdet, &s.bad);
#pragma unroll
    for (int m = 0; m < E; ++m) {
        const int e = tid + m * NTQ;
        const int i = e / KP, j = e % KP;
        if (i < K && j < K) st[L.off_CX + i * KP + j] = s.M[i * LDM + j];
    }
    const double *W = st + L.off_W;
    for (int r0 = 0; r0 < D; r0 += RB) {
        const int nr = (D - r0) < RB ? (D - r0) : RB;
        __syncthreads();
#pragma unroll 1
        for (int e = tid; e < RB * KP; e += NTQ) {
            const int r = e / KP, k = e % KP;
            s.Wb[r * LDM + k] = (r < nr && k < K) ? W[(r0 + r) * KP + k] : 0.0;
        }
        __syncthreads();
#pragma unroll 1
        for (int e = tid; e < RB * KP; e += NTQ) {
            const int k = e / RB, r = e % RB;
            if (k < K && r < nr) {
                double acc = 0.0;
#pragma unroll 4
                for (int j = 0; j < K; ++j) acc += s.M[k * LDM + j] * s.Wb[r * LDM + j];
                st[L.off_A + (int64_t)k * DP + r0 + r] = tau * acc;
            }
        }
    }
    if (tid == 0) st[L.off_scal + 1] = s.logdet;
}

template <int NTQ>
__device__ double pca_residual(const small_args &a, const double *st, double *red)
{
    const vmp_pca_layout &L = a.L;
    const int tid = threadIdx.x, D = a.D, K = a.K;
    const int KP = (int)L.KP;
    double t1 = 0.0, t2 = 0.0;
#pragma unroll 4
    for (int e = tid; e < D * KP; e += NTQ) t1 += st[L.off_W + e] * st[L.off_S + e];
    for (int e = tid; e < K * K; e += NTQ) {
        const int i = e / K, j = e - i * K;
        t2 += st[L.off_Sww + i * KP + j] * sxx_total(st, L, a.n_total, i, j);
    }
    t1 = block_sum<NTQ>(t1, red);
    t2 = block_sum<NTQ>(t2, red);
    return st[L.off_Syy] - 2.0 * t1 + t2;
}

template <int NTQ>
__device__ void op_update_tau(const small_args &a, double *st, double *red)
{
    const vmp_pca_layout &L = a.L;
    const double resid = pca_residual<NTQ>(a, st, red);
    if (threadIdx.x == 0) {
        const double al = a.a0t + 0.5 * (double)a.D * a.n_total;
        const double be = a.b0t + 0.5 * resid;
        st[L.off_tau + 0] = al;
        st[L.off_tau + 1] = be;
        st[L.off_tau + 2] = al / be;
        st[L.off_tau + 3] = sf_digamma(al) - sf_log(be);
        st[L.off_scal + 2] = resid;
        if (!(be > 0.0)) st[L.off_scal + 3] = (double)VMP_ERR_FLOATING;
    }
}

template <int NTQ>
__device__ void op_update_alpha(const small_args &a, double *st)
{
    const vmp_pca_layout &L = a.L;
    const int KP = (int)L.KP;
    for (int k = threadIdx.x; k < a.K; k += NTQ) {
        const double al = a.a0a + 0.5 * (double)a.D;
        const double be = a.b0a + 0.5 * ww_centred(a, st, k);
        st[L.off_alpha + 0 * KP + k] = al;
        st[L.off_alpha + 1 * KP + k] = be;
        st[L.off_alpha + 2 * KP + k] = al / be;
        st[L.off_alpha + 3 * KP + k] = sf_digamma(al) - sf_log(be);
    }
}

__device__ inline double gamma_elbo(double a0, double b0, double a, double b, double x,
                                    double logx)
{
    const double g_p = a0 * sf_log(b0) - sf_lgamma(a0);
    const double g_q = a * sf_log(b) - sf_lgamma(a);
    return g_p - g_q + (b - b0) * x + (a0 - a) * logx;
}

template <int NTQ>
__device__ void op_lower_bound(const small_args &a, double *st, double *red)
{
    const vmp_pca_layout &L = a.L;
    const int tid = threadIdx.x, D = a.D, K = a.K;
    const int KP = (int)L.KP;
    const double resid = pca_residual<NTQ>(a, st, red);
    double trx = 0.0, sla = 0.0, saw = 0.0, lal = 0.0;
#pragma unroll 1
    for (int k = tid; k <= K; k += NTQ) {
        const bool is_tau = (k == K);
        const int64_t oa = is_tau ? L.off_tau : L.off_alpha + k;
        const int64_t sa = is_tau ? 1 : KP;
        const double al = st[oa], be = st[oa + sa], x = st[oa + 2 * sa], lx = st[oa + 3 * sa];
        const double g = gamma_elbo(is_tau ? a.a0t : a.a0a, is_tau ? a.b0t : a.b0a, al, be, x, lx);
        if (is_tau) {
            red[NTQ / 64] = g;
        } else {
            trx += sxx_total(st, L, a.n_total, k, k);
            sla += lx;
            saw += x * ww_centred(a, st, k);
            lal += g;
        }
    }
    trx = block_sum<NTQ>(trx, red);
    sla = block_sum<NTQ>(sla, red);
    saw = block_sum<NTQ>(saw, red);
    lal = block_sum<NTQ>(lal, red);
    if (tid == 0) {
        const double tau = st[L.off_tau + 2], logtau = st[L.off_tau + 3];
        const double Dd = (double)D, Kd = (double)K;
        const double LY = Dd * a.n_total * (-0.5 * sf_log(2.0 * M_PI) + 0.5 * logtau)
                          - 0.5 * tau * resid;
        const double LX = -0.5 * a.x_prec * trx
                          + a.n_total * (0.5 * Kd * sf_log(a.x_prec) - 0.5 * st[L.off_scal + 1]
                                         + 0.5 * Kd);
        const double LW = 0.5 * Dd * sla - 0.5 * saw + Dd * (-0.5 * st[L.off_scal + 0] + 0.5 * Kd);
        const double Lt = red[NTQ / 64];
        st[L.off_L + 0] = LY;
        st[L.off_L + 1] = LX;
        st[L.off_L + 2] = LW;
        st[L.off_L + 3] = Lt;
        st[L.off_L + 4] = lal;
        st[L.off_L + 5] = LY + LX + LW + Lt + lal;
        st[L.off_scal + 2] = resid;
    }
}

template <int KP, int NTQ, int OP>
__device__ __forceinline__ void run_op(const small_args &a, double *st, small_lds<KP, NTQ> &s)
{
    if constexpr (OP != 0) {
        __threadfence_block();
        __syncthreads();
    }
    if constexpr (OP == VMP_PCA_OP_W) op_update_w<KP, NTQ>(a, st, s);
    if constexpr (OP == VMP_PCA_OP_XPREP) op_prepare_x<KP, NTQ>(a, st, s);
    if constexpr (OP == VMP_PCA_OP_TAU) op_update_tau<NTQ>(a, st, s.red);
    if constexpr (OP == VMP_PCA_OP_ALPHA) op_update_alpha<NTQ>(a, st);
    if constexpr (OP == VMP_PCA_OP_ELBO) op_lower_bound<NTQ>(a, st, s.red);
}

template <int KP, int NTQ, int O0, int O1, int O2>
__global__ void __launch_bounds__(NTQ)
pca_small_kernel(small_args a, double *st)
{
    __shared__ small_lds<KP, NTQ> s;
    __builtin_amdgcn_s_setprio(3);
    if (threadIdx.x == 0) s.bad = 0;
    run_op<KP, NTQ, O0>(a, st, s);
    run_op<KP, NTQ, O1>(a, st, s);
    run_op<KP, NTQ, O2>(a, st, s);
    __syncthreads();
    if (threadIdx.x == 0 && s.bad) st[a.L.off_scal + 3] = (double)VMP_ERR_NOT_POSDEF;
}

constexpr int FAST_D = 128;
constexpr int NTF = 256;

struct lay32 {
    int DP, KP, off_S, off_Syy, off_tau, off_alpha, off_W, off_CW, off_Sww, off_CX, off_A,
        off_scal, off_L;
    __device__ explicit lay32(const vmp_pca_layout &l)
        : DP((int)l.DP), KP((int)l.KP), off_S((int)l.off_S), off_Syy((int)l.off_Syy),
          off_tau((int)l.off_tau), off_alpha((int)l.off_alpha), off_W((int)l.off_W),
          off_CW((int)l.off_CW), off_Sww((int)l.off_Sww), off_CX((int)l.off_CX),
          off_A((int)l.off_A), off_scal((int)l.off_scal), off_L((int)l.off_L) {}
};

__device__ __forceinline__ v4f64 wave_tile_mma(const double *As, int am, int ak, const double *Bs,
                                               int bk, int bn, int kc)
{
    const int l = threadIdx.x & 63, l15 = l & 15, l4 = l >> 4;
    v4f64 acc = {0.0, 0.0, 0.0, 0.0};
#pragma unroll 4
    for (int q = 0; q < kc; q += 4)
        acc = __builtin_amdgcn_mfma_f64_16x16x4f64(As[l15 * am + (q + l4) * ak],
                                                   Bs[(q + l4) * bk + l15 * bn], acc, 0, 0, 0);
    return acc;
}

__device__ __forceinline__ v4f64 wave_tile_mma_acc(v4f64 acc, const double *As, int am, int ak,
                                                   const double *Bs, int bk, int bn, int kc)
{
    const int l = threadIdx.x & 63, l15 = l & 15, l4 = l >> 4;
#pragma unroll 4
    for (int q = 0; q < kc; q += 4)
        acc = __builtin_amdgcn_mfma_f64_16x16x4f64(As[l15 * am + (q + l4) * ak],
                                                   Bs[(q + l4) * bk + l15 * bn], acc, 0, 0, 0);
    return acc;
}

template <int KP>
__device__ __forceinline__ void pca_head_body(const small_args &a, double *st)
{
    constexpr int LDM = KP + 1, E = KP * KP / NTF, RB = 32;
    __shared__ double M[KP * LDM];
    __shared__ double T[KP * LDM];
    __shared__ double SWb[RB * LDM];
    __shared__ double alm[KP];
    __shared__ double logdet;
    __shared__ int bad;
    constexpr int KT = KP / 16;
    constexpr int NB = FAST_D / RB;
    constexpr int NLB = RB * KP / NTF;
    constexpr int TPB = 2 * KT;
    constexpr int WT = (TPB + 3) / 4;
    constexpr int ST = (KT * KT + 3) / 4;
    const lay32 L(a.L);
    int tid = threadIdx.x;
    const int D = a.D, K = a.K;
    const int DP = (int)L.DP;
    const int nb = (D + RB - 1) / RB;
    __builtin_amdgcn_s_setprio(3);
    if (tid == 0) bad = 0;
    const double tau = st[L.off_tau + 2];
    {
        double cx[E], sx[E];
#pragma unroll
        for (int m = 0; m < E; ++m) {
            const int e = tid + m * NTF;
            const int i = e / KP, j = e % KP;
            const bool in = (i < K && j < K);
            cx[m] = in ? st[L.off_CX + i * KP + j] : 0.0;
            sx[m] = in ? st[L.off_S + (L.DP + i) * KP + j] : 0.0;
        }
        if (tid < KP) alm[tid] = tid < K ? st[L.off_alpha + 2 * KP + tid] : 0.0;
#pragma unroll
        for (int m = 0; m < E; ++m) {
            const int e = tid + m * NTF;
            M[(e / KP) * LDM + (e % KP)] = cx[m];
            T[(e / KP) * LDM + (e % KP)] = sx[m];
        }
    }
    __syncthreads();
    {
        double lam[E];
#pragma unroll
        for (int m = 0; m < E; ++m) {
            const int e = tid + m * NTF;
            const int i = e / KP, j = e % KP;
            double x = (i == j) ? 1.0 : 0.0;
            if (i < K && j < K) {
                x = tau * (a.n_total * M[i * LDM + j] + 0.5 * (T[i * LDM + j] + T[j * LDM + i]));
                if (i == j) x += alm[i];
            }
            lam[m] = x;
        }
        __syncthreads();
#pragma unroll
        for (int m = 0; m < E; ++m) {
            const int e = tid + m * NTF;
            M[(e / KP) * LDM + (e % KP)] = lam[m];
        }
    }
    asm volatile("" : "+v"(tid));
    sweep_inverse<KP>(M, K, &logdet, &bad);
    asm volatile("" : "+v"(tid));
#pragma unroll
    for (int m = 0; m < E; ++m) {
        const int e = tid + m * NTF;
        const int i = e / KP, j = e % KP;
        if (i < K && j < K) st[L.off_CW + i * KP + j] = M[i * LDM + j];
    }
    if (tid == 0) st[L.off_scal + 0] = logdet;
    int w = tid >> 6, l15 = tid & 15, l4 = (tid & 63) >> 4;
    double v[NB][NLB];
#pragma unroll
    for (int b = 0; b < NB; ++b)
#pragma unroll
        for (int m = 0; m < NLB; ++m) {
            const int e = tid + m * NTF;
            const int r = b * RB + e / KP, k = e % KP;
            v[b][m] = (r < D && k < K) ? st[L.off_S + r * KP + k] : 0.0;
        }
    v4f64 wt[WT];
    v4f64 sacc[ST];
#pragma unroll
    for (int t = 0; t < ST; ++t) sacc[t] = v4f64{0.0, 0.0, 0.0, 0.0};
#pragma unroll
    for (int b = 0; b < NB; ++b) {
        if (b < nb) {
#pragma unroll
            for (int m = 0; m < NLB; ++m) {
                const int e = tid + m * NTF;
                SWb[(e / KP) * LDM + (e % KP)] = v[b][m];
            }
            __syncthreads();
#pragma unroll
            for (int t = 0; t < WT; ++t) {
                const int tile = w + 4 * t;
                if (tile < TPB)
                    wt[t] = wave_tile_mma(SWb + (tile / KT) * 16 * LDM, LDM, 1,
                                             M + (tile % KT) * 16, LDM, 1, KP);
            }
            __syncthreads();
#pragma unroll
            for (int t = 0; t < WT; ++t) {
                const int tile = w + 4 * t;
                if (tile < TPB) {
#pragma unroll
                    for (int r = 0; r < 4; ++r) {
                        const int lr = (tile / KT) * 16 + l4 + 4 * r, k = (tile % KT) * 16 + l15;
                        const double x = tau * wt[t][r];
                        SWb[lr * LDM + k] = x;
                        const int row = b * RB + lr;
                        if (row < D && k < K) st[L.off_W + row * KP + k] = x;
                    }
                }
            }
            __syncthreads();
#pragma unroll
            for (int t = 0; t < ST; ++t) {
                const int tile = w + 4 * t;
                if (tile < KT * KT)
                    sacc[t] = wave_tile_mma_acc(sacc[t], SWb + (tile / KT) * 16, 1, LDM,
                                                SWb + (tile % KT) * 16, LDM, 1, RB);
            }
            __syncthreads();
        }
    }
#pragma unroll
    for (int t = 0; t < ST; ++t) {
        const int tile = w + 4 * t;
        if (tile < KT * KT) {
#pragma unroll
            for (int r = 0; r < 4; ++r) {
                const int i = (tile / KT) * 16 + l4 + 4 * r, j = (tile % KT) * 16 + l15;
                const double sww = (double)D * M[i * LDM + j] + sacc[t][r];
                T[i * LDM + j] = sww;
                if (i < K && j < K) st[L.off_Sww + i * KP + j] = sww;
            }
        }
    }
    __syncthreads();
#pragma unroll
    for (int m = 0; m < E; ++m) {
        const int e = tid + m * NTF;
        const int i = e / KP, j = e % KP;
        double x = (i == j) ? 1.0 : 0.0;
        if (i < K && j < K) {
            x = tau * 0.5 * (T[i * LDM + j] + T[j * LDM + i]);
            if (i == j) x += a.x_prec;
        }
        M[i * LDM + j] = x;
    }
    asm volatile("" : "+v"(tid));
    sweep_inverse<KP>(M, K, &logdet, &bad);
    asm volatile("" : "+v"(tid));
    w = tid >> 6, l15 = tid & 15, l4 = (tid & 63) >> 4;
#pragma unroll
    for (int m = 0; m < E; ++m) {
        const int e = tid + m * NTF;
        const int i = e / KP, j = e % KP;
        if (i < K && j < K) st[L.off_CX + i * KP + j] = M[i * LDM + j];
    }
    double wv[NB][NLB];
#pragma unroll
    for (int b = 0; b < NB; ++b)
#pragma unroll
        for (int m = 0; m < NLB; ++m) {
            const int e = tid + m * NTF;
            const int r = b * RB + e / KP, k = e % KP;
            wv[b][m] = (r < D && k < K) ? st[L.off_W + r * KP + k] : 0.0;
        }
#pragma unroll
    for (int b = 0; b < NB; ++b) {
        if (b < nb) {
#pragma unroll
            for (int m = 0; m < NLB; ++m) {
                const int e = tid + m * NTF;
                SWb[(e / KP) * LDM + (e % KP)] = wv[b][m];
            }
            __syncthreads();
#pragma unroll
            for (int t = 0; t < WT; ++t) {
                const int tile = w + 4 * t;
                if (tile < TPB) {
                    const int tk = tile % KT, td = tile / KT;
                    const v4f64 acc = wave_tile_mma(M + tk * 16 * LDM, LDM, 1, SWb + td * 16 * LDM, 1,
                                                    LDM, KP);
#pragma unroll
                    for (int r = 0; r < 4; ++r) {
                        const int k = tk * 16 + l4 + 4 * r, d = b * RB + td * 16 + l15;
                        if (k < K && d < D) st[L.off_A + k * DP + d] = tau * acc[r];
                    }
                }
            }
            __syncthreads();
        }
    }
    if (tid == 0) {
        st[L.off_scal + 1] = logdet;
        if (bad) st[L.off_scal + 3] = (double)VMP_ERR_NOT_POSDEF;
    }
}

template <int KP>
__global__ void __launch_bounds__(NTF, 5)
pca_head_fast_kernel(small_args a, double *st, const double *stop)
{
    if (stop && stop[VMP_SWEEP_STOP] != 0.0) return;
    pca_head_body<KP>(a, st);
}

constexpr int GB = 32;
constexpr int GRA = 8;
constexpr int TAIL_PLAIN = 0, TAIL_GRAM = 1, TAIL_SWEEP = 2;
template <int KP>
struct alignas(16) tail_lds {
    double Sw[KP * (KP + 1)];
    double Cx[KP * (KP + 1)];
    double Sx[KP * (KP + 1)];
    double al[4 * KP];
    double sc[8];
    double red[NTF / 64 + 1];
    double stop;
};
static_assert(sizeof(tail_lds<16>) % 16 == 0 && sizeof(tail_lds<32>) % 16 == 0, "tail_lds size");
template <int KP, int MODE>
__device__ __forceinline__ void pca_tail_body(const small_args &a, double *st, const vmp_sweep_tail *sw,
                                              tail_lds<KP> &s)
{
    constexpr bool GRAM = (MODE == TAIL_GRAM);
    constexpr int LDM = KP + 1, E = KP * KP / NTF;
    extern __shared__ __align__(16) double gl[];
    double *Sw = s.Sw, *Cx = s.Cx, *Sx = s.Sx, *al = s.al, *sc = s.sc, *red = s.red;
    const lay32 L(a.L);
    const int tid = threadIdx.x, D = a.D, K = a.K;
    if constexpr (MODE == TAIL_SWEEP) {
        if (!sw->first && sw->ctl[VMP_SWEEP_STOP] != 0.0) {
            if (tid == 0) {
                sw->slot[7] = 0.0;
                sw->ctl[VMP_SWEEP_SKIPPED] += 1.0;
            }
            return;
        }
    }
    __builtin_amdgcn_s_setprio(3);
    double t1 = 0.0;
    double sxx[E];
#pragma unroll
    for (int m = 0; m < E; ++m) sxx[m] = 0.0;
    if constexpr (MODE == TAIL_SWEEP) {
        const int nb = sw->nb;
#pragma unroll
        for (int m = 0; m < E; ++m) {
            const int e = tid + m * NTF;
            const double *p = sw->P + e;
            double s0 = 0.0, s1 = 0.0, s2 = 0.0, s3 = 0.0;
            int b = 0;
            for (; b + 3 < nb; b += 4) {
                s0 += p[b * (KP * KP)];
                s1 += p[(b + 1) * (KP * KP)];
                s2 += p[(b + 2) * (KP * KP)];
                s3 += p[(b + 3) * (KP * KP)];
            }
            for (; b < nb; ++b) s0 += p[b * (KP * KP)];
            sxx[m] = (s0 + s1) + (s2 + s3);
            st[L.off_S + L.DP * KP + e] = sxx[m];
        }
    }
    if constexpr (GRAM) {
        const int DP = L.DP, LA = DP + 1;
        double *As = gl, *Gs = As + KP * LA, *Ss = Gs + GB * LA;
        for (int e = tid; e < KP * DP; e += NTF) {
            const int k = e / DP, d = e - k * DP;
            As[k * LA + d] = (k < K && d < D) ? st[L.off_A + k * DP + d] : 0.0;
        }
        for (int r0 = 0; r0 < D; r0 += GB) {
            for (int e = tid; e < GB * DP; e += NTF) {
                const int r = e / DP, d = e - r * DP;
                Gs[r * LA + d] = (r0 + r < D && d < D) ? st[(int)a.L.off_G + (r0 + r) * DP + d] : 0.0;
            }
            __syncthreads();
#pragma unroll
            for (int m = 0; m < GB * KP / NTF; ++m) {
                const int e = tid + m * NTF;
                const int r = e / KP, k = e % KP;
                const double *gr = Gs + r * LA, *ar = As + k * LA;
                double s0 = 0.0, s1 = 0.0;
                for (int d = 0; d < D; d += 2) {
                    s0 += gr[d] * ar[d];
                    s1 += gr[d + 1] * ar[d + 1];
                }
                const double sv = s0 + s1;
                Ss[r * LDM + k] = sv;
                if (r0 + r < D) {
                    st[L.off_S + (r0 + r) * KP + k] = sv;
                    if (k < K) t1 += st[L.off_W + (r0 + r) * KP + k] * sv;
                }
            }
            __syncthreads();
#pragma unroll
            for (int m = 0; m < E; ++m) {
                const int e = tid + m * NTF;
                const int i = e / KP, j = e % KP;
                double s0 = 0.0;
#pragma unroll 8
                for (int r = 0; r < GB; ++r) s0 += As[i * LA + r0 + r] * Ss[r * LDM + j];
                sxx[m] += s0;
            }
            __syncthreads();
        }
#pragma unroll
        for (int m = 0; m < E; ++m) {
            const int e = tid + m * NTF;
            const int i = e / KP, j = e % KP;
            st[L.off_S + (L.DP + i) * KP + j] = (i < K && j < K) ? sxx[m] : 0.0;
        }
    }
    {
        double v0[E], v1[E], v2[E];
#pragma unroll
        for (int m = 0; m < E; ++m) {
            const int e = tid + m * NTF;
            const int i = e / KP, j = e % KP;
            const bool in = (i < K && j < K);
            v0[m] = in ? st[L.off_Sww + i * KP + j] : 0.0;
            v1[m] = in ? st[L.off_CX + i * KP + j] : 0.0;
            if constexpr (MODE != TAIL_PLAIN) v2[m] = in ? sxx[m] : 0.0;
            else v2[m] = in ? st[L.off_S + (L.DP + i) * KP + j] : 0.0;
        }
        if (tid == 0) {
            sc[4] = st[L.off_Syy];
            sc[5] = st[L.off_scal + 0];
            sc[6] = st[L.off_scal + 1];
        }
#pragma unroll
        for (int m = 0; m < E; ++m) {
            const int e = tid + m * NTF;
            const int i = e / KP, j = e % KP;
            Sw[i * LDM + j] = v0[m];
            Cx[i * LDM + j] = v1[m];
            Sx[i * LDM + j] = v2[m];
        }
    }
    if constexpr (!GRAM) {
        const int n = D * KP;
#pragma unroll 1
        for (int e0 = 0; e0 < n; e0 += 8 * NTF) {
            double w[8], y[8];
#pragma unroll
            for (int m = 0; m < 8; ++m) {
                const int e = e0 + tid + m * NTF;
                w[m] = e < n ? st[L.off_W + e] : 0.0;
                y[m] = e < n ? st[L.off_S + e] : 0.0;
            }
#pragma unroll
            for (int m = 0; m < 8; ++m) t1 += w[m] * y[m];
        }
    }
    __syncthreads();
    double t2 = 0.0, trx = 0.0;
#pragma unroll
    for (int m = 0; m < E; ++m) {
        const int e = tid + m * NTF;
        const int i = e / KP, j = e % KP;
        const double sxx = a.n_total * Cx[i * LDM + j] + 0.5 * (Sx[i * LDM + j] + Sx[j * LDM + i]);
        t2 += Sw[i * LDM + j] * sxx;
        if (i == j) trx += sxx;
    }
    t1 = block_sum<NTF>(t1, red);
    t2 = block_sum<NTF>(t2, red);
    trx = block_sum<NTF>(trx, red);
    const double resid = sc[4] - 2.0 * t1 + t2;
    if (tid == 64) {
        const double ta = a.a0t + 0.5 * (double)D * a.n_total;
        const double tb = a.b0t + 0.5 * resid;
        sc[0] = ta;
        sc[1] = tb;
        sc[2] = ta / tb;
        sc[3] = sf_digamma(ta) - sf_log(tb);
        st[L.off_tau + 0] = ta;
        st[L.off_tau + 1] = tb;
        st[L.off_tau + 2] = sc[2];
        st[L.off_tau + 3] = sc[3];
        st[L.off_scal + 2] = resid;
        if (!(tb > 0.0)) st[L.off_scal + 3] = (double)VMP_ERR_FLOATING;
        if constexpr (MODE == TAIL_SWEEP)
            sc[7] = !(tb > 0.0) ? (double)VMP_ERR_FLOATING : st[L.off_scal + 3];
        red[NTF / 64] = gamma_elbo(a.a0t, a.b0t, ta, tb, sc[2], sc[3]);
    }
    double sla = 0.0, saw = 0.0, lal = 0.0;
    if (tid < K) {
        const double aa = a.a0a + 0.5 * (double)D;
        const double ab = a.b0a + 0.5 * Sw[tid * LDM + tid];
        const double am = aa / ab, alg = sf_digamma(aa) - sf_log(ab);
        al[0 * KP + tid] = aa;
        al[1 * KP + tid] = ab;
        al[2 * KP + tid] = am;
        al[3 * KP + tid] = alg;
        st[L.off_alpha + 0 * KP + tid] = aa;
        st[L.off_alpha + 1 * KP + tid] = ab;
        st[L.off_alpha + 2 * KP + tid] = am;
        st[L.off_alpha + 3 * KP + tid] = alg;
        sla = alg;
        saw = am * Sw[tid * LDM + tid];
        lal = gamma_elbo(a.a0a, a.b0a, aa, ab, am, alg);
    }
    sla = block_sum<NTF>(sla, red);
    saw = block_sum<NTF>(saw, red);
    lal = block_sum<NTF>(lal, red);
    if (tid == 0) {
        const double tau = sc[2], logtau = sc[3];
        const double Dd = (double)D, Kd = (double)K;
        const double LY = Dd * a.n_total * (-0.5 * sf_log(2.0 * M_PI) + 0.5 * logtau)
                          - 0.5 * tau * resid;
        const double LX = -0.5 * a.x_prec * trx
                          + a.n_total * (0.5 * Kd * sf_log(a.x_prec) - 0.5 * sc[6] + 0.5 * Kd);
        const double LW = 0.5 * Dd * sla - 0.5 * saw + Dd * (-0.5 * sc[5] + 0.5 * Kd);
        const double Lt = red[NTF / 64];
        st[L.off_L + 0] = LY;
        st[L.off_L + 1] = LX;
        st[L.off_L + 2] = LW;
        st[L.off_L + 3] = Lt;
        st[L.off_L + 4] = lal;
        st[L.off_L + 5] = LY + LX + LW + Lt + lal;
        if constexpr (MODE == TAIL_SWEEP) {
            const double status = sc[7];
            double *slot = sw->slot;
            slot[0] = LY;
            slot[1] = LX;
            slot[2] = LW;
            slot[3] = Lt;
            slot[4] = lal;
            slot[5] = LY + LX + LW + Lt + lal;
            slot[6] = status;
            slot[7] = 1.0;
            al[0] = LY;
            al[1] = LX;
            al[2] = LW;
            al[3] = Lt;
            al[4] = lal;
            const double Lb = vmp_bound_sum(al, sw->order, sw->norder);
            const double L0 = sw->first ? sw->l0 : sw->ctl[VMP_SWEEP_L];
            int stop = status != 0.0;
            if (sw->compare && vmp_stop_rule(Lb, L0, sw->tol)) stop = 1;
            sw->ctl[VMP_SWEEP_STOP] = stop ? 1.0 : 0.0;
            s.stop = stop ? 1.0 : 0.0;
            sw->ctl[VMP_SWEEP_L] = Lb;
            sw->ctl[VMP_SWEEP_EXECUTED] += 1.0;
        }
    }
}

template <int KP, bool GRAM>
__global__ void __launch_bounds__(NTF)
pca_tail_fast_kernel(small_args a, double *st)
{
    __shared__ tail_lds<KP> s;
    pca_tail_body<KP, GRAM ? TAIL_GRAM : TAIL_PLAIN>(a, st, nullptr, s);
}

template <int KP>
__global__ void __launch_bounds__(NTF)
pca_tail_sweep_kernel(small_args a, double *st, vmp_sweep_tail sw)
{
    __shared__ tail_lds<KP> s;
    pca_tail_body<KP, TAIL_SWEEP>(a, st, &sw, s);
}

__host__ __device__ inline size_t gram_phase_a_wide_lds(int KP, int DP)
{
    return ((size_t)KP * (DP + 2) + (size_t)GRA * DP + (size_t)GRA * (KP + 1)) * sizeof(double);
}

template <int KP, class STAMP = stamps_off>
__device__ __forceinline__ void gram_phase_a_wide(const vmp_pca_layout &L, int D, int K, double *st,
                                                  double *lds, int blk, const STAMP &stamp = STAMP())
{
    constexpr int LDS_S = KP + 1, KT = KP / 16;
    constexpr int NA = KP * (FAST_D / 2) / NTF, NG = GRA * (FAST_D / 2) / NTF;
    const int DP = (int)L.DP, LA = DP + 2;
    const int DP2 = DP >> 1, sh = __builtin_ctz(DP2);
    double *As = lds;
    double *Gs = As + KP * LA;
    double *Ss = Gs + GRA * DP;
    const int tid = threadIdx.x;
    const int r0 = blk * GRA;
    const double *A = st + L.off_A;
    const double *G = st + L.off_G + (int64_t)r0 * DP;
    v2f64 av[NA], gv[NG];
#pragma unroll
    for (int m = 0; m < NA; ++m) {
        const int e = tid + m * NTF;
        const int k = e >> sh, c = (e & (DP2 - 1)) * 2;
        av[m] = *reinterpret_cast<const v2f64 *>(A + (k < K ? k : K - 1) * DP + c);
    }
#pragma unroll
    for (int m = 0; m < NG; ++m) {
        const int e = tid + m * NTF;
        gv[m] = *reinterpret_cast<const v2f64 *>(G + 2 * (e < GRA * DP2 ? e : GRA * DP2 - 1));
    }
#pragma unroll
    for (int m = 0; m < NA; ++m) {
        const int e = tid + m * NTF;
        const int k = e >> sh, c = (e & (DP2 - 1)) * 2;
        if (e < KP * DP2) *reinterpret_cast<v2f64 *>(As + k * LA + c) = k < K ? av[m] : v2f64{0.0, 0.0};
    }
#pragma unroll
    for (int m = 0; m < NG; ++m) {
        const int e = tid + m * NTF;
        if (e < GRA * DP2) *reinterpret_cast<v2f64 *>(Gs + 2 * e) = gv[m];
    }
    __syncthreads();
    stamp(SP_LDS_FILLED);
    {
        const int w = tid >> 6, l = tid & 63;
        if (w < 2 * KT) {
            const int k = (l & 15) + 16 * (w % KT), r = (l >> 4) + 4 * (w / KT);
            double s = 0.0;
            const int sl = l >> 4;
            const double *gx = Gs + (r - sl + (l & 3)) * DP + sl, *ax = As + k * LA + sl;
            const int D4 = D & ~3;
            int d = 0;
            for (; d + 32 <= D4; d += 32) {
                double gq[8], aq[8];
#pragma unroll
                for (int q = 0; q < 8; ++q) {
                    gq[q] = gx[d + 4 * q];
                    aq[q] = ax[d + 4 * q];
                }
#pragma unroll
                for (int q = 0; q < 8; ++q) s = __builtin_amdgcn_mfma_f64_4x4x4f64(gq[q], aq[q], s, 0, 0, 0);
            }
            for (; d < D4; d += 4) s = __builtin_amdgcn_mfma_f64_4x4x4f64(gx[d], ax[d], s, 0, 0, 0);
            if (D4 < D) {
                const double g4 = gx[D4], a4 = ax[D4];
                const bool in = D4 + sl < D;
                s = __builtin_amdgcn_mfma_f64_4x4x4f64(in ? g4 : 0.0, in ? a4 : 0.0, s, 0, 0, 0);
            }
            Ss[r * LDS_S + k] = s;
            if (r0 + r < D && k < K) st[L.off_S + (r0 + r) * KP + k] = s;
        }
    }
    __syncthreads();
    stamp(SP_SYX);
}

template <int KP>
__global__ void __launch_bounds__(NTF)
pca_gram_wide_kernel(vmp_pca_layout L, int D, int K, double *st)
{
    extern __shared__ __align__(16) double gl[];
    gram_phase_a_wide<KP>(L, D, K, st, gl, blockIdx.x);
}

template <int KP, class STAMP>
__device__ __forceinline__ void sweep_tail_wide(const small_args &a, double *st, const vmp_sweep_tail &sw,
                                                tail_lds<KP> &s, double *SW, const double *AL,
                                                const STAMP &stamp)
{
    constexpr int LDM = KP + 1, E = KP * KP / NTF, NW = FAST_D * KP / NTF;
    double *Sw = s.Sw, *Cx = s.Cx, *Sx = s.Sx, *al = s.al, *sc = s.sc, *red = s.red;
    const lay32 L(a.L);
    const int tid = threadIdx.x, D = a.D, K = a.K;
    __builtin_amdgcn_s_setprio(3);
    double t1 = 0.0;
    double ww[NW], wy[NW], es0[E], es1[E];
    {
        const int n = D * KP;
#pragma unroll
        for (int j = 0; j < NW; ++j) {
            const int e = tid + j * NTF;
            ww[j] = e < n ? st[L.off_W + e] : 0.0;
            wy[j] = e < n ? st[L.off_S + e] : 0.0;
        }
#pragma unroll
        for (int m = 0; m < E; ++m) {
            const int e = tid + m * NTF;
            const int i = e / KP, j = e % KP;
            const bool in = (i < K && j < K);
            es0[m] = in ? st[L.off_Sww + i * KP + j] : 0.0;
            es1[m] = in ? st[L.off_CX + i * KP + j] : 0.0;
        }
    }
    if (tid == 0) {
        sc[4] = st[L.off_Syy];
        sc[5] = st[L.off_scal + 0];
        sc[6] = st[L.off_scal + 1];
    }
#pragma unroll
    for (int m = 0; m < E; ++m) {
        const int e = tid + m * NTF;
        const int i = e / KP, j = e % KP;
        Sw[i * LDM + j] = es0[m];
        Cx[i * LDM + j] = es1[m];
    }
    {
        const int n = D * KP, jn = (n + 8 * NTF - 1) / (8 * NTF) * 8;
        const int nsw = L.DP * KP;
#pragma unroll
        for (int j = 0; j < NW; ++j) {
            const int e = tid + j * NTF;
            if (j < jn) t1 += ww[j] * wy[j];
            if (e < nsw) SW[(e / KP) * LDM + (e % KP)] = (e < n && e % KP < K) ? wy[j] : 0.0;
        }
    }
    __syncthreads();
    stamp(SP_T_LOADS);
    {
        constexpr int KT = KP / 16;
        const int LA = L.DP + 2;
        const int w = tid >> 6, l15 = tid & 15, l4 = (tid & 63) >> 4;
        const int nb = sw.nb, nb4 = nb & ~3;
        if (w < KT * KT) {
            const int ti = w / KT, tj = w % KT;
            const double *ar = AL + (16 * ti + l15) * LA + l4;
            const double *sr = SW + l4 * LDM + 16 * tj + l15;
            const auto group = [&](int b) {
                v4f64 p = {0.0, 0.0, 0.0, 0.0};
#pragma unroll
                for (int h = 0; h < GRA; h += 4)
                    p = __builtin_amdgcn_mfma_f64_16x16x4f64(ar[b * GRA + h], sr[(b * GRA + h) * LDM], p,
                                                             0, 0, 0);
                return p;
            };
            v4f64 acc[4];
#pragma unroll
            for (int q = 0; q < 4; ++q) acc[q] = v4f64{0.0, 0.0, 0.0, 0.0};
#pragma unroll 1
            for (int b = 0; b < nb4; b += 4) {
#pragma unroll
                for (int q = 0; q < 4; ++q) acc[q] += group(b + q);
            }
#pragma unroll 1
            for (int b = nb4; b < nb; ++b) acc[0] += group(b);
#pragma unroll
            for (int r = 0; r < 4; ++r) {
                const int k = 16 * ti + l4 + 4 * r, k2 = 16 * tj + l15;
                const bool in = (k < K && k2 < K);
                const double x = in ? (acc[0][r] + acc[1][r]) + (acc[2][r] + acc[3][r]) : 0.0;
                st[L.off_S + (L.DP + k) * KP + k2] = x;
                Sx[k * LDM + k2] = x;
            }
        }
    }
    __syncthreads();
    stamp(SP_T_PXX);
    double t2 = 0.0, trx = 0.0;
#pragma unroll
    for (int m = 0; m < E; ++m) {
        const int e = tid + m * NTF;
        const int i = e / KP, j = e % KP;
        const double sxx = a.n_total * Cx[i * LDM + j] + 0.5 * (Sx[i * LDM + j] + Sx[j * LDM + i]);
        t2 += Sw[i * LDM + j] * sxx;
        if (i == j) trx += sxx;
    }
    {
        double *r3 = al + 3 * KP;
        static_assert(KP >= 3 * (NTF / 64), "twelve words");
        t1 = wave_sum(t1);
        t2 = wave_sum(t2);
        trx = wave_sum(trx);
        if ((tid & 63) == 0) {
            r3[tid >> 6] = t1;
            r3[NTF / 64 + (tid >> 6)] = t2;
            r3[2 * (NTF / 64) + (tid >> 6)] = trx;
        }
        __syncthreads();
        t1 = t2 = trx = 0.0;
#pragma unroll
        for (int i = 0; i < NTF / 64; ++i) {
            t1 += r3[i];
            t2 += r3[NTF / 64 + i];
            trx += r3[2 * (NTF / 64) + i];
        }
    }
    stamp(SP_T_BLOCKSUMS);
    const double resid = sc[4] - 2.0 * t1 + t2;
    if (tid == 64) {
        const double ta = a.a0t + 0.5 * (double)D * a.n_total;
        const double tb = a.b0t + 0.5 * resid;
        sc[0] = ta;
        sc[1] = tb;
        sc[2] = ta / tb;
        red[0] = resid;
        red[1] = trx;
        st[L.off_tau + 0] = ta;
        st[L.off_tau + 1] = tb;
        st[L.off_tau + 2] = sc[2];
        st[L.off_scal + 2] = resid;
        if (!(tb > 0.0)) st[L.off_scal + 3] = (double)VMP_ERR_FLOATING;
    }
    if (tid < K) {
        const double aa = a.a0a + 0.5 * (double)D;
        const double ab = a.b0a + 0.5 * Sw[tid * LDM + tid];
        const double am = aa / ab;
        al[0 * KP + tid] = aa;
        al[1 * KP + tid] = ab;
        al[2 * KP + tid] = am;
        st[L.off_alpha + 0 * KP + tid] = aa;
        st[L.off_alpha + 1 * KP + tid] = ab;
        st[L.off_alpha + 2 * KP + tid] = am;
    }
    stamp(SP_T_TAU_ALPHA);
    stamp(SP_T_BOUND);
    stamp(SP_T_RING);
}

template <int KP, class STAMP>
struct defer_side {
    const small_args &a;
    double *st;
    const vmp_sweep_tail &sw;
    tail_lds<KP> &s;
    const double *sf;
    const STAMP &stamp;
    __device__ __forceinline__ void operator()() const
    {
        constexpr int LDM = KP + 1;
        if (threadIdx.x >= 128) return;
        const lay32 L(a.L);
        const int l = threadIdx.x - 64, D = a.D, K = a.K;
        const bool isa = l < K;
        const int k = isa ? l : 0;
        const double a0 = isa ? a.a0a : a.a0t, b0 = isa ? a.b0a : a.b0t;
        const double av = isa ? s.al[0 * KP + k] : s.sc[0];
        const double bv = isa ? s.al[1 * KP + k] : s.sc[1];
        const double mean = isa ? s.al[2 * KP + k] : s.sc[2];
        const double *c = sf + (isa ? VMP_SWEEP_SF_ALPHA : VMP_SWEEP_SF_TAU);
        const double dg = c[0], lga = c[1], lga0 = c[2], logb0 = c[3];
        const double logb = sf_log(bv);
        const double logx = dg - logb;
        const double g_p = a0 * logb0 - lga0;
        const double g_q = av * logb - lga;
        const double g = g_p - g_q + (bv - b0) * mean + (a0 - av) * logx;
        if (isa) st[L.off_alpha + 3 * KP + k] = logx;
        if (l == 32) st[L.off_tau + 3] = logx;
        stamp.side(SP_S_STATE);
        const double sla = 0.0 + wave_sum(isa ? logx : 0.0);
        const double saw = 0.0 + wave_sum(isa ? mean * s.Sw[k * LDM + k] : 0.0);
        const double lal = 0.0 + wave_sum(isa ? g : 0.0);
        const double logtau = __shfl(logx, 32, 64), Lt = __shfl(g, 32, 64);
        if (l == 0) {
            const double tau = s.sc[2], resid = s.red[0], trx = s.red[1];
            const double Dd = (double)D, Kd = (double)K;
            const double LY = Dd * a.n_total * (-0.5 * sf[VMP_SWEEP_SF_LOG2PI] + 0.5 * logtau)
                              - 0.5 * tau * resid;
            const double LX = -0.5 * a.x_prec * trx
                              + a.n_total * (0.5 * Kd * sf[VMP_SWEEP_SF_LOGXPREC] - 0.5 * s.sc[6] + 0.5 * Kd);
            const double LW = 0.5 * Dd * sla - 0.5 * saw + Dd * (-0.5 * s.sc[5] + 0.5 * Kd);
            st[L.off_L + 0] = LY;
            st[L.off_L + 1] = LX;
            st[L.off_L + 2] = LW;
            st[L.off_L + 3] = Lt;
            st[L.off_L + 4] = lal;
            st[L.off_L + 5] = LY + LX + LW + Lt + lal;
            const double status = !(s.sc[1] > 0.0) ? (double)VMP_ERR_FLOATING : st[L.off_scal + 3];
            double *slot = sw.slot;
            slot[0] = LY;
            slot[1] = LX;
            slot[2] = LW;
            slot[3] = Lt;
            slot[4] = lal;
            slot[5] = LY + LX + LW + Lt + lal;
            slot[6] = status;
            slot[7] = 1.0;
            double *al = s.al;
            al[0] = LY;
            al[1] = LX;
            al[2] = LW;
            al[3] = Lt;
            al[4] = lal;
            const double Lb = vmp_bound_sum(al, sw.order, sw.norder);
            const double L0 = sw.first ? sw.l0 : sw.ctl[VMP_SWEEP_L];
            int stop = status != 0.0;
            if (sw.compare && vmp_stop_rule(Lb, L0, sw.tol)) stop = 1;
            sw.ctl[VMP_SWEEP_STOP] = stop ? 1.0 : 0.0;
            s.stop = stop ? 1.0 : 0.0;
            sw.ctl[VMP_SWEEP_L] = Lb;
            sw.ctl[VMP_SWEEP_EXECUTED] += 1.0;
        }
        stamp.side(SP_S_RING);
    }
};

template <int KP, class STAMP, class SIDE = no_side>
__device__ __forceinline__ void pca_head_wide(const small_args &a, double *st, double *M, double *T,
                                              const double *alm, double tau, double *SW,
                                              const STAMP &stamp, const SIDE &side = SIDE(),
                                              const double *stopw = nullptr)
{
    constexpr bool DEFER = !std::is_same<SIDE, no_side>::value;
    constexpr int LDM = KP + 1, E = KP * KP / NTF, KT = KP / 16;
    constexpr int WT = FAST_D / 16 * KT / 4;
    constexpr int ST = (KT * KT + 3) / 4;
    __shared__ double logdet;
    __shared__ int bad;
    const lay32 L(a.L);
    const int tid = threadIdx.x, D = a.D, K = a.K, DP = (int)L.DP;
    const int nr = (D + 31) / 32 * 32;
    const int nt = nr / 16 * KT;
    const int w = tid >> 6, l15 = tid & 15, l4 = (tid & 63) >> 4;
    if (tid == 0) bad = 0;
    {
        double lam[E];
#pragma unroll
        for (int m = 0; m < E; ++m) {
            const int e = tid + m * NTF;
            const int i = e / KP, j = e % KP;
            double x = (i == j) ? 1.0 : 0.0;
            if (i < K && j < K) {
                x = tau * (a.n_total * M[i * LDM + j] + 0.5 * (T[i * LDM + j] + T[j * LDM + i]));
                if (i == j) x += alm[i];
            }
            lam[m] = x;
        }
        __syncthreads();
#pragma unroll
        for (int m = 0; m < E; ++m) {
            const int e = tid + m * NTF;
            M[(e / KP) * LDM + (e % KP)] = lam[m];
        }
    }
    stamp(SP_H_LAMBDA);
    if constexpr (DEFER) {
        sweep_inverse<KP>(M, K, &logdet, &bad, side);
        if (*stopw != 0.0) return;
    } else {
        sweep_inverse<KP>(M, K, &logdet, &bad);
    }
    stamp(SP_H_INV1);
#pragma unroll
    for (int m = 0; m < E; ++m) {
        const int e = tid + m * NTF;
        const int i = e / KP, j = e % KP;
        if (i < K && j < K) st[L.off_CW + i * KP + j] = M[i * LDM + j];
    }
    if (tid == 0) st[L.off_scal + 0] = logdet;
    v4f64 wt[WT];
#pragma unroll
    for (int t = 0; t < WT; ++t) {
        const int tile = w + 4 * t;
        if (tile < nt)
            wt[t] = wave_tile_mma(SW + (tile / KT) * 16 * LDM, LDM, 1, M + (tile % KT) * 16, LDM, 1, KP);
    }
    __syncthreads();
#pragma unroll
    for (int t = 0; t < WT; ++t) {
        const int tile = w + 4 * t;
        if (tile < nt) {
#pragma unroll
            for (int r = 0; r < 4; ++r) {
                const int row = (tile / KT) * 16 + l4 + 4 * r, k = (tile % KT) * 16 + l15;
                const double x = tau * wt[t][r];
                SW[row * LDM + k] = x;
                if (row < D && k < K) st[L.off_W + row * KP + k] = x;
            }
        }
    }
    __syncthreads();
    stamp(SP_H_W);
#pragma unroll
    for (int t = 0; t < ST; ++t) {
        const int tile = w + 4 * t;
        if (tile < KT * KT) {
            const v4f64 sacc = wave_tile_mma_acc(v4f64{0.0, 0.0, 0.0, 0.0}, SW + (tile / KT) * 16, 1, LDM,
                                                 SW + (tile % KT) * 16, LDM, 1, nr);
#pragma unroll
            for (int r = 0; r < 4; ++r) {
                const int i = (tile / KT) * 16 + l4 + 4 * r, j = (tile % KT) * 16 + l15;
                const double sww = (double)D * M[i * LDM + j] + sacc[r];
                T[i * LDM + j] = sww;
                if (i < K && j < K) st[L.off_Sww + i * KP + j] = sww;
            }
        }
    }
    __syncthreads();
    stamp(SP_H_SWW);
#pragma unroll
    for (int m = 0; m < E; ++m) {
        const int e = tid + m * NTF;
        const int i = e / KP, j = e % KP;
        double x = (i == j) ? 1.0 : 0.0;
        if (i < K && j < K) {
            x = tau * 0.5 * (T[i * LDM + j] + T[j * LDM + i]);
            if (i == j) x += a.x_prec;
        }
        M[i * LDM + j] = x;
    }
    const auto pad = [&]() {
        if (D == nr && K == KP) return;
        for (int e = tid - 64; e < nr * KP; e += NTF - 64)
            if (e / KP >= D || e % KP >= K) SW[(e / KP) * LDM + (e % KP)] = 0.0;
    };
    sweep_inverse<KP>(M, K, &logdet, &bad, pad);
    stamp(SP_H_INV2);
#pragma unroll
    for (int m = 0; m < E; ++m) {
        const int e = tid + m * NTF;
        const int i = e / KP, j = e % KP;
        if (i < K && j < K) st[L.off_CX + i * KP + j] = M[i * LDM + j];
    }
#pragma unroll
    for (int t = 0; t < WT; ++t) {
        const int tile = w + 4 * t;
        if (tile < nt) {
            const int tk = tile % KT, td = tile / KT;
            const v4f64 acc = wave_tile_mma(M + tk * 16 * LDM, LDM, 1, SW + td * 16 * LDM, 1, LDM, KP);
#pragma unroll
            for (int r = 0; r < 4; ++r) {
                const int k = tk * 16 + l4 + 4 * r, d = td * 16 + l15;
                if (k < K && d < D) st[L.off_A + k * DP + d] = tau * acc[r];
            }
        }
    }
    if (tid == 0) {
        st[L.off_scal + 1] = logdet;
        if (bad) st[L.off_scal + 3] = (double)VMP_ERR_NOT_POSDEF;
    }
    stamp.drain();
    stamp(SP_H_A);
}

__host__ __device__ inline size_t sweep_local_lds(int KP, int DP)
{
    return ((size_t)KP * (DP + 2) + (size_t)DP * (KP + 1) + 2) * sizeof(double);
}

template <int KP, class STAMP>
__device__ __forceinline__ void pca_sweep_mid_body(const small_args &a, double *st,
                                                   const vmp_sweep_tail &sw, unsigned int *ticket,
                                                   const double *sf, const STAMP &stamp)
{
    extern __shared__ __align__(16) double gl[];
    __shared__ tail_lds<KP> ts;
    const int tid = threadIdx.x;
    if (!sw.first && sw.ctl[VMP_SWEEP_STOP] != 0.0) {
        if (blockIdx.x == 0 && tid == 0) {
            sw.slot[7] = 0.0;
            sw.ctl[VMP_SWEEP_SKIPPED] += 1.0;
        }
        return;
    }
    stamp(SP_ENTRY);
    gram_phase_a_wide<KP, STAMP>(a.L, a.D, a.K, st, gl, blockIdx.x, stamp);
    asm volatile("s_waitcnt vmcnt(0)" ::: "memory");
    __syncthreads();
    stamp(SP_PXX);
    const int na = KP * ((int)a.L.DP + 2);
    double *SW = gl + na;
    unsigned int *word = reinterpret_cast<unsigned int *>(SW + (int)a.L.DP * (KP + 1));
    if (tid == 0) {
        __builtin_amdgcn_fence(__ATOMIC_RELEASE, "agent");
        asm volatile("s_waitcnt vmcnt(0)" ::: "memory");
        *word = __hip_atomic_fetch_add(ticket, 1u, __ATOMIC_RELAXED, __HIP_MEMORY_SCOPE_AGENT);
    }
    __syncthreads();
    if (*word != gridDim.x - 1) return;
    stamp(SP_TICKET);
    if (tid == 0) {
        __builtin_amdgcn_fence(__ATOMIC_ACQUIRE, "agent");
        asm volatile("s_waitcnt vmcnt(0)" ::: "memory");
        *ticket = 0u;
    }
    __syncthreads();
    stamp(SP_ACQUIRE);
    sweep_tail_wide<KP>(a, st, sw, ts, SW, gl, stamp);
    __syncthreads();
    const defer_side<KP, STAMP> side{a, st, sw, ts, sf, stamp};
    pca_head_wide<KP>(a, st, ts.Cx, ts.Sx, ts.al + 2 * KP, ts.sc[2], SW, stamp, side, &ts.stop);
}

template <int KP>
__global__ void __launch_bounds__(NTF)
pca_sweep_mid_kernel(small_args a, double *st, double *P, vmp_sweep_tail sw, unsigned int *ticket,
                     const double *sf)
{
    pca_sweep_mid_body<KP>(a, st, sw, ticket, sf, stamps_off());
}

template <int KP>
__global__ void __launch_bounds__(NTF)
pca_sweep_mid_stamped_kernel(small_args a, double *st, double *P, vmp_sweep_tail sw,
                             unsigned int *ticket, const double *sf, unsigned long long *out, int level)
{
    __shared__ unsigned long long stl[VMP_SWEEP_NSTAMP];
    if (threadIdx.x < VMP_SWEEP_NSTAMP) stl[threadIdx.x] = 0;
    __syncthreads();
    const stamps_on stamp{stl, level};
    pca_sweep_mid_body<KP>(a, st, sw, ticket, sf, stamp);
    if (threadIdx.x == 0 && stl[SP_T_LOADS] != 0)
        for (int i = 0; i < VMP_SWEEP_NSTAMP; ++i) out[i] = stl[i];
}

template <int KP>
__global__ void __launch_bounds__(NTF)
pca_head_wide_kernel(small_args a, double *st)
{
    constexpr int LDM = KP + 1, E = KP * KP / NTF, NW = FAST_D * KP / NTF;
    __shared__ __align__(16) double M[KP * LDM], T[KP * LDM], SW[FAST_D * LDM], alm[KP];
    const lay32 L(a.L);
    const int tid = threadIdx.x, D = a.D, K = a.K;
    const int n = D * KP, nsw = (D + 31) / 32 * 32 * KP;
    double cx[E], sx[E], wy[NW];
#pragma unroll
    for (int m = 0; m < E; ++m) {
        const int e = tid + m * NTF;
        const int i = e / KP, j = e % KP;
        const bool in = (i < K && j < K);
        cx[m] = in ? st[L.off_CX + i * KP + j] : 0.0;
        sx[m] = in ? st[L.off_S + (L.DP + i) * KP + j] : 0.0;
    }
#pragma unroll
    for (int j = 0; j < NW; ++j) {
        const int e = tid + j * NTF;
        wy[j] = (e < n && e % KP < K) ? st[L.off_S + e] : 0.0;
    }
    const double tau = st[L.off_tau + 2];
    if (tid < KP) alm[tid] = tid < K ? st[L.off_alpha + 2 * KP + tid] : 0.0;
#pragma unroll
    for (int m = 0; m < E; ++m) {
        const int e = tid + m * NTF;
        M[(e / KP) * LDM + (e % KP)] = cx[m];
        T[(e / KP) * LDM + (e % KP)] = sx[m];
    }
#pragma unroll
    for (int j = 0; j < NW; ++j) {
        const int e = tid + j * NTF;
        if (e < nsw) SW[(e / KP) * LDM + (e % KP)] = wy[j];
    }
    __syncthreads();
    pca_head_wide<KP>(a, st, M, T, alm, tau, SW, stamps_off());
}

__global__ void __launch_bounds__(64)
pca_sweep_sf_kernel(small_args a, double *sf)
{
    const int l = threadIdx.x;
    if (l >= VMP_SWEEP_SF_LEN) return;
    const double ta = a.a0t + 0.5 * (double)a.D * a.n_total;
    const double aa = a.a0a + 0.5 * (double)a.D;
    double v;
    switch (l) {
    case VMP_SWEEP_SF_TAU + 0: v = sf_digamma(ta); break;
    case VMP_SWEEP_SF_TAU + 1: v = sf_lgamma(ta); break;
    case VMP_SWEEP_SF_TAU + 2: v = sf_lgamma(a.a0t); break;
    case VMP_SWEEP_SF_TAU + 3: v = sf_log(a.b0t); break;
    case VMP_SWEEP_SF_ALPHA + 0: v = sf_digamma(aa); break;
    case VMP_SWEEP_SF_ALPHA + 1: v = sf_lgamma(aa); break;
    case VMP_SWEEP_SF_ALPHA + 2: v = sf_lgamma(a.a0a); break;
    case VMP_SWEEP_SF_ALPHA + 3: v = sf_log(a.b0a); break;
    case VMP_SWEEP_SF_LOG2PI: v = sf_log(2.0 * M_PI); break;
    default: v = sf_log(a.x_prec); break;
    }
    sf[l] = v;
}

template <int FORM>
__global__ void __launch_bounds__(64)
mfma_order_probe_kernel(int n, const double *A, const double *B, const double *C, double *Dm)
{
    const int l = threadIdx.x, lo = l & 15, k = l >> 4;
    for (int t = 0; t < n; ++t) {
        if constexpr (FORM == 0) {
            const double *Ct = C + (size_t)t * 256;
            double *Dt = Dm + (size_t)t * 256;
            v4f64 c;
#pragma unroll
            for (int r = 0; r < 4; ++r) c[r] = Ct[(k + 4 * r) * 16 + lo];
            const v4f64 d = __builtin_amdgcn_mfma_f64_16x16x4f64(A[(size_t)t * 64 + lo * 4 + k],
                                                                 B[(size_t)t * 64 + k * 16 + lo], c, 0, 0, 0);
#pragma unroll
            for (int r = 0; r < 4; ++r) Dt[(k + 4 * r) * 16 + lo] = d[r];
        } else {
            const int x = l & 3, b = (l >> 2) & 3;
            const size_t o = (size_t)t * 64 + b * 16;
            Dm[o + k * 4 + x] = __builtin_amdgcn_mfma_f64_4x4x4f64(A[o + x * 4 + k], B[o + k * 4 + x],
                                                                   C[o + k * 4 + x], 0, 0, 0);
        }
    }
}

bool fast_small_enabled()
{
    static const int v = getenv("VMP_PCA_FAST_SMALL") ? atoi(getenv("VMP_PCA_FAST_SMALL")) : 1;
    return v != 0;
}

int32_t fill_small_args(vmp_ctx *ctx, small_args &a, int32_t D, int32_t K, int64_t n_total,
                        double x_prec, double a0t, double b0t, double a0a, double b0a)
{
    const int32_t rc = vmp_pca_get_layout(D, K, &a.L);
    VMP_REQUIRE(ctx, rc == VMP_OK, rc, "unsupported dims D=%d K=%d", D, K);
    a.D = D;
    a.K = K;
    a.n_total = (double)n_total;
    a.x_prec = x_prec;
    a.a0t = a0t; a.b0t = b0t; a.a0a = a0a; a.b0a = b0a;
    a.has_mean = 0;
    return VMP_OK;
}

template <int O0, int O1, int O2>
void launch_sequence(vmp_ctx *ctx, const small_args &a, double *state)
{
    constexpr bool has_inverse = (O0 == VMP_PCA_OP_W || O0 == VMP_PCA_OP_XPREP ||
                                  O1 == VMP_PCA_OP_W || O1 == VMP_PCA_OP_XPREP);
    constexpr int NT64 = has_inverse ? 1024 : 256;
    if (a.L.KP == 16)
        hipLaunchKernelGGL((pca_small_kernel<16, 256, O0, O1, O2>), dim3(1), dim3(256), 0,
                           ctx->stream, a, state);
    else if (a.L.KP == 32)
        hipLaunchKernelGGL((pca_small_kernel<32, 256, O0, O1, O2>), dim3(1), dim3(256), 0,
                           ctx->stream, a, state);
    else
        hipLaunchKernelGGL((pca_small_kernel<64, NT64, O0, O1, O2>), dim3(1), dim3(NT64), 0,
                           ctx->stream, a, state);
}

int32_t launch_small(vmp_ctx *ctx, int32_t D, int32_t K, int64_t n_total, double x_prec,
                     double a0t, double b0t, double a0a, double b0a, int32_t nops,
                     const int32_t *ops, double *state, int32_t has_mean = 0)
{
    VMP_REQUIRE(ctx, ctx && state && ops, VMP_ERR_INVALID, "null argument");
    VMP_REQUIRE(ctx, nops >= 1 && nops <= VMP_PCA_MAX_OPS, VMP_ERR_INVALID,
                "between 1 and %d operations per call", VMP_PCA_MAX_OPS);
    small_args a;
    int32_t rc = vmp_pca_get_layout(D, K, &a.L);
    VMP_REQUIRE(ctx, rc == VMP_OK, rc, "unsupported dims D=%d K=%d", D, K);
    a.D = D;
    a.K = K;
    a.n_total = (double)n_total;
    a.x_prec = x_prec;
    a.a0t = a0t; a.b0t = b0t; a.a0a = a0a; a.b0a = b0a;
    a.has_mean = has_mean ? 1 : 0;
    for (int i = 0; i < nops; ++i) {
        const int op = ops[i];
        VMP_REQUIRE(ctx, op >= VMP_PCA_OP_W && op <= VMP_PCA_OP_ELBO, VMP_ERR_INVALID,
                    "unknown operation code %d", op);
        if (op == VMP_PCA_OP_XPREP || op == VMP_PCA_OP_ELBO)
            VMP_REQUIRE(ctx, x_prec > 0, VMP_ERR_INVALID, "x_prec must be positive");
        if (op == VMP_PCA_OP_TAU || op == VMP_PCA_OP_ELBO)
            VMP_REQUIRE(ctx, a0t > 0 && b0t > 0, VMP_ERR_INVALID,
                        "Gamma prior parameters must be positive");
        if (op == VMP_PCA_OP_ALPHA || op == VMP_PCA_OP_ELBO)
            VMP_REQUIRE(ctx, a0a > 0 && b0a > 0, VMP_ERR_INVALID,
                        "Gamma prior parameters must be positive");
    }
    const bool fast_enabled = fast_small_enabled();
    const bool fast = fast_enabled && a.L.KP <= 32 && D <= FAST_D && !a.has_mean;
    bool gram_here = false;
    if (ctx->gram_pending) {
        const bool tail_first = nops >= 3 && ops[0] == VMP_PCA_OP_TAU && ops[1] == VMP_PCA_OP_ALPHA
                                && ops[2] == VMP_PCA_OP_ELBO;
        if (fast && tail_first && ctx->gram_state == state && ctx->gram_D == D && ctx->gram_K == K) {
            gram_here = true;
            ctx->gram_pending = 0;
        } else {
            rc = vmp_pca_ensure_gram(ctx);
            if (rc != VMP_OK) return rc;
        }
    }
    int i = 0;
    while (i < nops) {
        const int o0 = ops[i], o1 = i + 1 < nops ? ops[i + 1] : 0, o2 = i + 2 < nops ? ops[i + 2] : 0;
        if (o0 == VMP_PCA_OP_W && o1 == VMP_PCA_OP_XPREP) {
            if (fast && a.L.KP == 16)
                hipLaunchKernelGGL(pca_head_fast_kernel<16>, dim3(1), dim3(NTF), 0, ctx->stream, a,
                                   state, (const double *)nullptr);
            else if (fast)
                hipLaunchKernelGGL(pca_head_fast_kernel<32>, dim3(1), dim3(NTF), 0, ctx->stream, a,
                                   state, (const double *)nullptr);
            else
                launch_sequence<VMP_PCA_OP_W, VMP_PCA_OP_XPREP, 0>(ctx, a, state);
            i += 2;
        } else if (o0 == VMP_PCA_OP_TAU && o1 == VMP_PCA_OP_ALPHA && o2 == VMP_PCA_OP_ELBO) {
            if (fast && gram_here) {
                const size_t lds = ((size_t)(a.L.KP + GB) * (a.L.DP + 1) + (size_t)GB * (a.L.KP + 1))
                                   * sizeof(double);
                static bool raised[64] = {false};
                const int dev = ctx->device & 63;
                if (!raised[dev]) {
                    VMP_HIP_CHECK(ctx, hipFuncSetAttribute(
                        (const void *)pca_tail_fast_kernel<16, true>,
                        hipFuncAttributeMaxDynamicSharedMemorySize, 128 * 1024));
                    VMP_HIP_CHECK(ctx, hipFuncSetAttribute(
                        (const void *)pca_tail_fast_kernel<32, true>,
                        hipFuncAttributeMaxDynamicSharedMemorySize, 128 * 1024));
                    raised[dev] = true;
                }
                if (a.L.KP == 16)
                    hipLaunchKernelGGL((pca_tail_fast_kernel<16, true>), dim3(1), dim3(NTF), lds,
                                       ctx->stream, a, state);
                else
                    hipLaunchKernelGGL((pca_tail_fast_kernel<32, true>), dim3(1), dim3(NTF), lds,
                                       ctx->stream, a, state);
                gram_here = false;
            } else if (fast && a.L.KP == 16)
                hipLaunchKernelGGL((pca_tail_fast_kernel<16, false>), dim3(1), dim3(NTF), 0,
                                   ctx->stream, a, state);
            else if (fast)
                hipLaunchKernelGGL((pca_tail_fast_kernel<32, false>), dim3(1), dim3(NTF), 0,
                                   ctx->stream, a, state);
            else
                launch_sequence<VMP_PCA_OP_TAU, VMP_PCA_OP_ALPHA, VMP_PCA_OP_ELBO>(ctx, a, state);
            i += 3;
        } else {
            switch (o0) {
            case VMP_PCA_OP_W: launch_sequence<VMP_PCA_OP_W, 0, 0>(ctx, a, state); break;
            case VMP_PCA_OP_XPREP: launch_sequence<VMP_PCA_OP_XPREP, 0, 0>(ctx, a, state); break;
            case VMP_PCA_OP_TAU: launch_sequence<VMP_PCA_OP_TAU, 0, 0>(ctx, a, state); break;
            case VMP_PCA_OP_ALPHA: launch_sequence<VMP_PCA_OP_ALPHA, 0, 0>(ctx, a, state); break;
            default: launch_sequence<VMP_PCA_OP_ELBO, 0, 0>(ctx, a, state); break;
            }
            i += 1;
        }
        VMP_HIP_CHECK(ctx, hipGetLastError());
    }
    return VMP_OK;
}

}

int32_t vmp_pca_sweep_covered(int32_t D, int32_t K)
{
    vmp_pca_layout L;
    if (vmp_pca_get_layout(D, K, &L) != VMP_OK) return VMP_PCA_SWEEPS_NOT_BUILT;
    return (fast_small_enabled() && L.KP <= 32 && D <= FAST_D) ? VMP_OK : VMP_PCA_SWEEPS_NOT_BUILT;
}

int32_t vmp_pca_launch_sweep_head(vmp_ctx *ctx, int32_t D, int32_t K, int64_t n_total, double x_prec,
                                  double a0t, double b0t, double a0a, double b0a, double *state,
                                  const double *stop)
{
    small_args a;
    const int32_t rc = fill_small_args(ctx, a, D, K, n_total, x_prec, a0t, b0t, a0a, b0a);
    if (rc != VMP_OK) return rc;
    if (a.L.KP == 16)
        hipLaunchKernelGGL(pca_head_fast_kernel<16>, dim3(1), dim3(NTF), 0, ctx->stream, a, state, stop);
    else
        hipLaunchKernelGGL(pca_head_fast_kernel<32>, dim3(1), dim3(NTF), 0, ctx->stream, a, state, stop);
    VMP_HIP_CHECK(ctx, hipGetLastError());
    return VMP_OK;
}

int32_t vmp_pca_launch_sweep_tail(vmp_ctx *ctx, int32_t D, int32_t K, int64_t n_total, double x_prec,
                                  double a0t, double b0t, double a0a, double b0a, double *state,
                                  const vmp_sweep_tail &t)
{
    small_args a;
    const int32_t rc = fill_small_args(ctx, a, D, K, n_total, x_prec, a0t, b0t, a0a, b0a);
    if (rc != VMP_OK) return rc;
    if (a.L.KP == 16)
        hipLaunchKernelGGL(pca_tail_sweep_kernel<16>, dim3(1), dim3(NTF), 0, ctx->stream, a, state, t);
    else
        hipLaunchKernelGGL(pca_tail_sweep_kernel<32>, dim3(1), dim3(NTF), 0, ctx->stream, a, state, t);
    VMP_HIP_CHECK(ctx, hipGetLastError());
    return VMP_OK;
}

template <typename F>
static int32_t raise_lds_once(vmp_ctx *ctx, F *k16, F *k32, bool *raised)
{
    const int dev = ctx->device & 63;
    if (raised[dev]) return VMP_OK;
    VMP_HIP_CHECK(ctx, hipFuncSetAttribute((const void *)k16,
                                           hipFuncAttributeMaxDynamicSharedMemorySize, 96 * 1024));
    VMP_HIP_CHECK(ctx, hipFuncSetAttribute((const void *)k32,
                                           hipFuncAttributeMaxDynamicSharedMemorySize, 96 * 1024));
    raised[dev] = true;
    return VMP_OK;
}

int32_t vmp_pca_launch_gram_fast(vmp_ctx *ctx, int32_t D, int32_t K, double *state)
{
    vmp_pca_layout L;
    const int32_t rc = vmp_pca_get_layout(D, K, &L);
    VMP_REQUIRE(ctx, rc == VMP_OK, rc, "unsupported dims D=%d K=%d", D, K);
    VMP_REQUIRE(ctx, L.KP <= 32 && D <= FAST_D, VMP_ERR_UNSUPPORTED,
                "the fast Gram statistics cover K <= 32, D <= %d", FAST_D);
    VMP_REQUIRE(ctx, ((uintptr_t)state % 16) == 0, VMP_ERR_INVALID, "state must be 16-byte aligned");
    static bool raised[64] = {false};
    const int32_t rr = raise_lds_once(ctx, pca_gram_wide_kernel<16>, pca_gram_wide_kernel<32>, raised);
    if (rr != VMP_OK) return rr;
    const int nb = (int)(L.DP / GRA);
    const size_t lds = gram_phase_a_wide_lds((int)L.KP, (int)L.DP);
    if (L.KP == 16)
        hipLaunchKernelGGL(pca_gram_wide_kernel<16>, dim3(nb), dim3(NTF), lds, ctx->stream, L, D, K,
                           state);
    else
        hipLaunchKernelGGL(pca_gram_wide_kernel<32>, dim3(nb), dim3(NTF), lds, ctx->stream, L, D, K,
                           state);
    VMP_HIP_CHECK(ctx, hipGetLastError());
    return VMP_OK;
}

template <int KP>
static int32_t launch_mid(vmp_ctx *ctx, const small_args &a, double *state, double *P,
                          const vmp_sweep_tail &t, unsigned int *ticket, unsigned long long *stamps,
                          int stamp_level)
{
    VMP_REQUIRE(ctx, ctx->sweep_sf, VMP_ERR_INVALID,
                "the one-launch sweep needs vmp_pca_sweep_constants first");
    static bool raised[2][64] = {{false}};
    const int dev = ctx->device & 63, s = stamps ? 1 : 0;
    if (!raised[s][dev]) {
        const void *f = stamps ? (const void *)pca_sweep_mid_stamped_kernel<KP>
                               : (const void *)pca_sweep_mid_kernel<KP>;
        VMP_HIP_CHECK(ctx, hipFuncSetAttribute(f, hipFuncAttributeMaxDynamicSharedMemorySize,
                                               96 * 1024));
        raised[s][dev] = true;
    }
    const size_t lds = sweep_local_lds((int)a.L.KP, (int)a.L.DP);
    const dim3 nb((unsigned)(a.L.DP / GRA));
    if (stamps)
        hipLaunchKernelGGL(pca_sweep_mid_stamped_kernel<KP>, nb, dim3(NTF), lds, ctx->stream, a, state,
                           P, t, ticket, (const double *)ctx->sweep_sf, stamps, stamp_level);
    else
        hipLaunchKernelGGL(pca_sweep_mid_kernel<KP>, nb, dim3(NTF), lds, ctx->stream, a, state, P, t,
                           ticket, (const double *)ctx->sweep_sf);
    VMP_HIP_CHECK(ctx, hipGetLastError());
    return VMP_OK;
}

int32_t vmp_pca_launch_sweep_mid(vmp_ctx *ctx, int32_t D, int32_t K, int64_t n_total, double x_prec,
                                 double a0t, double b0t, double a0a, double b0a, double *state,
                                 double *P, const vmp_sweep_tail &t, unsigned int *ticket,
                                 unsigned long long *stamps, int32_t stamp_level)
{
    small_args a;
    const int32_t rc = fill_small_args(ctx, a, D, K, n_total, x_prec, a0t, b0t, a0a, b0a);
    if (rc != VMP_OK) return rc;
    if (a.L.KP == 16) return launch_mid<16>(ctx, a, state, P, t, ticket, stamps, stamp_level);
    return launch_mid<32>(ctx, a, state, P, t, ticket, stamps, stamp_level);
}

int32_t vmp_pca_sweep_constants(vmp_ctx *ctx, int32_t D, int32_t K, int64_t n_total, double x_prec,
                                double a0t, double b0t, double a0a, double b0a)
{
    small_args a;
    const int32_t rc = fill_small_args(ctx, a, D, K, n_total, x_prec, a0t, b0t, a0a, b0a);
    if (rc != VMP_OK) return rc;
    const double key[7] = {a0t, b0t, a0a, b0a, (double)D, (double)n_total, x_prec};
    if (ctx->sweep_sf && ctx->sweep_sf_valid && memcmp(key, ctx->sweep_sf_key, sizeof(key)) == 0)
        return VMP_OK;
    if (!ctx->sweep_sf) VMP_HIP_CHECK(ctx, hipMalloc(&ctx->sweep_sf, VMP_SWEEP_SF_LEN * sizeof(double)));
    ctx->sweep_sf_valid = 0;
    hipLaunchKernelGGL(pca_sweep_sf_kernel, dim3(1), dim3(64), 0, ctx->stream, a, ctx->sweep_sf);
    VMP_HIP_CHECK(ctx, hipGetLastError());
    memcpy(ctx->sweep_sf_key, key, sizeof(key));
    ctx->sweep_sf_valid = 1;
    return VMP_OK;
}

int32_t vmp_pca_launch_sweep_head_wide(vmp_ctx *ctx, int32_t D, int32_t K, int64_t n_total,
                                       double x_prec, double a0t, double b0t, double a0a, double b0a,
                                       double *state)
{
    small_args a;
    const int32_t rc = fill_small_args(ctx, a, D, K, n_total, x_prec, a0t, b0t, a0a, b0a);
    if (rc != VMP_OK) return rc;
    if (a.L.KP == 16)
        hipLaunchKernelGGL(pca_head_wide_kernel<16>, dim3(1), dim3(NTF), 0, ctx->stream, a, state);
    else
        hipLaunchKernelGGL(pca_head_wide_kernel<32>, dim3(1), dim3(NTF), 0, ctx->stream, a, state);
    VMP_HIP_CHECK(ctx, hipGetLastError());
    return VMP_OK;
}

extern "C" {

int32_t vmp_mfma_order_probe(vmp_ctx *ctx, int32_t form, int32_t ntiles, const double *A,
                             const double *B, const double *C, double *D)
{
    VMP_REQUIRE(ctx, ctx && A && B && C && D, VMP_ERR_INVALID, "null argument");
    VMP_REQUIRE(ctx, form == 0 || form == 1, VMP_ERR_INVALID, "form %d (0 or 1)", form);
    VMP_REQUIRE(ctx, ntiles >= 1 && ntiles <= (1 << 20), VMP_ERR_INVALID, "ntiles %d out of range",
                ntiles);
    if (form == 0)
        hipLaunchKernelGGL(mfma_order_probe_kernel<0>, dim3(1), dim3(64), 0, ctx->stream, ntiles, A, B, C, D);
    else
        hipLaunchKernelGGL(mfma_order_probe_kernel<1>, dim3(1), dim3(64), 0, ctx->stream, ntiles, A, B, C, D);
    VMP_HIP_CHECK(ctx, hipGetLastError());
    return VMP_OK;
}

int32_t vmp_pca_small_ops(vmp_ctx *ctx, int32_t D, int32_t K, int64_t n_total, double x_prec,
                          double a0_tau, double b0_tau, double a0_alpha, double b0_alpha,
                          int32_t nops, const int32_t *ops, double *state)
{
    return launch_small(ctx, D, K, n_total, x_prec, a0_tau, b0_tau, a0_alpha, b0_alpha, nops, ops,
                        state);
}

int32_t vmp_pca_small_ops_mean(vmp_ctx *ctx, int32_t D, int32_t K, int64_t n_total, double x_prec,
                               double a0_tau, double b0_tau, double a0_alpha, double b0_alpha,
                               int32_t nops, const int32_t *ops, int32_t has_mean, double *state)
{
    return launch_small(ctx, D, K, n_total, x_prec, a0_tau, b0_tau, a0_alpha, b0_alpha, nops, ops,
                        state, has_mean);
}

int32_t vmp_pca_update_w(vmp_ctx *ctx, int32_t D, int32_t K, int64_t n_total, double *state)
{
    const int32_t op = VMP_PCA_OP_W;
    return launch_small(ctx, D, K, n_total, 0.0, 0.0, 0.0, 0.0, 0.0, 1, &op, state);
}

int32_t vmp_pca_prepare_x(vmp_ctx *ctx, int32_t D, int32_t K, double x_prec, double *state)
{
    const int32_t op = VMP_PCA_OP_XPREP;
    return launch_small(ctx, D, K, 0, x_prec, 0.0, 0.0, 0.0, 0.0, 1, &op, state);
}

int32_t vmp_pca_update_tau(vmp_ctx *ctx, int32_t D, int32_t K, int64_t n_total, double a0,
                           double b0, double *state)
{
    const int32_t op = VMP_PCA_OP_TAU;
    return launch_small(ctx, D, K, n_total, 0.0, a0, b0, 0.0, 0.0, 1, &op, state);
}

int32_t vmp_pca_update_alpha(vmp_ctx *ctx, int32_t D, int32_t K, double a0, double b0,
                             double *state)
{
    const int32_t op = VMP_PCA_OP_ALPHA;
    return launch_small(ctx, D, K, 0, 0.0, 0.0, 0.0, a0, b0, 1, &op, state);
}

int32_t vmp_pca_lower_bound(vmp_ctx *ctx, int32_t D, int32_t K, int64_t n_total, double x_prec,
                            double a0_tau, double b0_tau, double a0_alpha, double b0_alpha,
                            double *state)
{
    const int32_t op = VMP_PCA_OP_ELBO;
    return launch_small(ctx, D, K, n_total, x_prec, a0_tau, b0_tau, a0_alpha, b0_alpha, 1, &op,
                        state);
}

}
```

Measured before the change: 28250.

## Write A into xpass buffer from sweep kernels and add register-resident A variant

The final head or mid sweep kernel now writes the updated loading matrix straight into the plate-stream double buffer. This lets the later x-pass skip its separate device-to-device memcpy of A. The change also adds an opt-in x-pass kernel form that holds A fragments in registers instead of LDS, plus a grid cap for it. That form is off by default (form_dflt=0). The extra writes add a little work to a single-block kernel and require the event wait on the buffer to move earlier onto the main stream.

```diff
diff --git a/bayespy_amd/csrc/vmp_common.h b/bayespy_amd/csrc/vmp_common.h
--- a/bayespy_amd/csrc/vmp_common.h
+++ b/bayespy_amd/csrc/vmp_common.h
@@ -36,6 +36,7 @@
     hipEvent_t ev_xbuf[2];
     int x_buf_pending[2];
     int64_t x_count;
+    double *x_prefilled;
     int xs_cus;
     int x_hold, x_held;
     vmp_xpass_desc x_desc;
@@ -84,7 +85,7 @@
 int32_t vmp_pca_sweep_covered(int32_t D, int32_t K);
 int32_t vmp_pca_launch_sweep_head(vmp_ctx *ctx, int32_t D, int32_t K, int64_t n_total, double x_prec,
                                   double a0t, double b0t, double a0a, double b0a, double *state,
-                                  const double *stop);
+                                  const double *stop, double *Ax);
 int32_t vmp_pca_launch_sweep_tail(vmp_ctx *ctx, int32_t D, int32_t K, int64_t n_total, double x_prec,
                                   double a0t, double b0t, double a0a, double b0a, double *state,
                                   const vmp_sweep_tail &t);
@@ -92,12 +93,12 @@
 int32_t vmp_pca_launch_sweep_mid(vmp_ctx *ctx, int32_t D, int32_t K, int64_t n_total, double x_prec,
                                  double a0t, double b0t, double a0a, double b0a, double *state,
                                  double *P, const vmp_sweep_tail &t, unsigned int *ticket,
-                                 unsigned long long *stamps, int32_t stamp_level);
+                                 unsigned long long *stamps, int32_t stamp_level, double *Ax);
 int32_t vmp_pca_sweep_constants(vmp_ctx *ctx, int32_t D, int32_t K, int64_t n_total, double x_prec,
                                 double a0t, double b0t, double a0a, double b0a);
 int32_t vmp_pca_launch_sweep_head_wide(vmp_ctx *ctx, int32_t D, int32_t K, int64_t n_total,
                                        double x_prec, double a0t, double b0t, double a0a, double b0a,
-                                       double *state);
+                                       double *state, double *Ax);
 int32_t vmp_pca_launch_gram_fast(vmp_ctx *ctx, int32_t D, int32_t K, double *state);
 
 int32_t vmp_pca_ensure_gram(vmp_ctx *ctx);
diff --git a/bayespy_amd/csrc/vmp_ctx.hip b/bayespy_amd/csrc/vmp_ctx.hip
--- a/bayespy_amd/csrc/vmp_ctx.hip
+++ b/bayespy_amd/csrc/vmp_ctx.hip
@@ -88,6 +88,7 @@
     ctx->x_pending = 0;
     ctx->x_buf_pending[0] = ctx->x_buf_pending[1] = 0;
     ctx->x_count = 0;
+    ctx->x_prefilled = nullptr;
     ctx->ev_xbuf[0] = ctx->ev_xbuf[1] = nullptr;
     ctx->xs_cus = 0;
     ctx->x_hold = ctx->x_held = 0;
diff --git a/bayespy_amd/csrc/vmp_pca.hip b/bayespy_amd/csrc/vmp_pca.hip
--- a/bayespy_amd/csrc/vmp_pca.hip
+++ b/bayespy_amd/csrc/vmp_pca.hip
@@ -242,13 +242,15 @@
     if (threadIdx.x == 0) out[0] = s;
 }
 
-constexpr int xpass_occ(int DB, int KT, int OCC)
-{
+constexpr int xpass_occ(int DB, int KT, int OCC, int FORM = 0)
+{
+    if (FORM) return OCC < 2 ? 1 : 2;
     return KT * DB * 4096 > 80 * 1024 ? 1 : (KT * DB * 4096 > 53 * 1024 ? (OCC < 2 ? OCC : 2) : OCC);
 }
 
-template <int DB, int KT, bool GUARD, int OCC, int NTM = 0, int LAY = 0, int MF = 0, bool IL = false>
-__global__ void __launch_bounds__(NT, xpass_occ(DB, KT, OCC))
+template <int DB, int KT, bool GUARD, int OCC, int NTM = 0, int LAY = 0, int MF = 0, bool IL = false,
+          int FORM = 0>
+__global__ void __launch_bounds__(NT, xpass_occ(DB, KT, OCC, FORM))
 pca_xpass_kernel(const double *__restrict__ Y, int64_t ldy, int64_t N, int D, int K,
                  const double *__restrict__ Apad, double *__restrict__ X, int64_t ldx,
                  int64_t tile0, int64_t tile1)
@@ -259,20 +261,30 @@
     constexpr int CH = KS / NCH;
     constexpr bool YT = (LAY & 1) != 0, XT = (LAY & 2) != 0;
     static_assert(!(GUARD && LAY != 0), "tile-major arrays are padded: no guarded instance");
-
-    __shared__ double Af[KT * KS * 64];
+    static_assert(FORM == 0 || (YT && !MF && !IL && KT * DB <= 8), "FORM 1: see launch_xpass");
+
+    __shared__ double Af[FORM ? 1 : KT * KS * 64];
 
     const int tid = threadIdx.x;
     const int l = tid & 63;
     const int l15 = l & 15, l4 = l >> 4;
     const int w = __builtin_amdgcn_readfirstlane(tid >> 6);
 
-    for (int e = tid; e < KT * KS * 64; e += NT) {
-        const int lane = e & 63, fq = e >> 6;
-        const int it = fq / KS, q = fq - it * KS;
-        Af[e] = Apad[(int64_t)(it * 16 + (lane & 15)) * DP + 4 * q + (lane >> 4)];
-    }
-    __syncthreads();
+    double af[FORM ? KT : 1][FORM ? KS : 1];
+    if (FORM) {
+#pragma unroll
+        for (int it = 0; it < KT; ++it)
+#pragma unroll
+            for (int q = 0; q < KS; ++q)
+                af[FORM ? it : 0][FORM ? q : 0] = Apad[(it * 16 + l15) * DP + 4 * q + l4];
+    } else {
+        for (int e = tid; e < KT * KS * 64; e += NT) {
+            const int lane = e & 63, fq = e >> 6;
+            const int it = fq / KS, q = fq - it * KS;
+            Af[e] = Apad[(int64_t)(it * 16 + (lane & 15)) * DP + 4 * q + (lane >> 4)];
+        }
+        __syncthreads();
+    }
 
     const double *Afl = MF ? Af + 16 * l4 + (l & 3) : Af + l;
     const uint32_t yoff = (uint32_t)(((int64_t)l4 * ldy + 2 * l15) * 8);
@@ -337,7 +349,7 @@
             const int cc = STG ? ((c + rot) & (NCH - 1)) : c;
             if (c + 1 < NCH) issue(tile, STG ? ((c + 1 + rot) & (NCH - 1)) : c + 1, buf[(c + 1) & 1]);
             else if (tile + stride < tile1) issue(tile + stride, first_chunk(tile + stride), buf[(c + 1) & 1]);
-            asm volatile("" ::: "memory");
+            if (!FORM) asm volatile("" ::: "memory");
             const double *Afc = Afl + cc * (CH * 64);
 #pragma unroll
             for (int i = 0; i < CH; ++i) {
@@ -352,7 +364,8 @@
                             acc[it][1][R] = __builtin_amdgcn_mfma_f64_4x4x4f64(a, b.y, acc[it][1][R], 0, 0, 0);
                         }
                     } else {
-                        const double a = Afc[(it * KS + i) * 64];
+                        const double a = FORM ? af[FORM ? it : 0][FORM ? c * CH + i : 0]
+                                              : Afc[(it * KS + i) * 64];
                         acc[it][0] = mfma_f64(a, b.x, acc[it][0]);
                         acc[it][1] = mfma_f64(a, b.y, acc[it][1]);
                     }
@@ -709,6 +722,12 @@
     const int occ = xpass_occupancy();
     const int ntm = vmp_tune_get("xpass_nt", env_int("VMP_PCA_XPASS_NT", 3, 0, 3));
     const int mf4 = vmp_tune_get("xpass_mfma4", env_int("VMP_PCA_XPASS_MFMA4", 0, 0, 1));
+    const int form_dflt = 0;
+    int form = vmp_tune_get("xpass_form", env_int("VMP_PCA_XPASS_FORM", -1, -1, 1));
+    if (form < 0) form = form_dflt;
+    const bool form1 = form == 1 &&
+                       (lay == 1 || lay == 3) && KT * DB <= 8 && !mf4 && ntm == 3 &&
+                       !pca_interleave();
     hipStream_t s = on_plate ? ctx->xs : ctx->stream;
     const int64_t gmax = (int64_t)(on_plate ? ctx->xs_cus : ctx->num_cu) * xpass_wgs_per_cu();
     hipEvent_t *ev = ctx->timing ? vmp_next_events(ctx) : nullptr;
@@ -719,6 +738,13 @@
         if (t1 <= t0) continue;
         int64_t g = (t1 - t0 + 3) / 4;
         if (g > gmax) g = gmax;
+        const int cap = vmp_tune_get("xpass_grid_cap", 0);
+        if (cap > 0 && g > cap) g = cap;
+        const int fw = (DB == 2 && KT == 4) || vmp_tune_get("xpass_form_wgs", 1) < 2 ? 1 : 2;
+        if (form1 && !guard) {
+            const int64_t gf = (int64_t)(on_plate ? ctx->xs_cus : ctx->num_cu) * fw;
+            if (g > gf) g = gf;
+        }
         const dim3 grid((unsigned)g);
 #define VMP_XP(db, kt, gd, oc, nt, ly)                                                          \
     hipLaunchKernelGGL((pca_xpass_kernel<db, kt, gd, oc, nt, ly>), grid, dim3(NT), 0, s, Y, ldy, \
@@ -740,6 +766,16 @@
             VMP_HIP_CHECK(ctx, hipGetLastError());
             continue;
         }
+#define VMP_XPF(db, kt, oc, ly)                                                                  \
+    hipLaunchKernelGGL((pca_xpass_kernel<db, kt, false, oc, 3, ly, 0, false, 1>), grid, dim3(NT), 0, \
+                       s, Y, ldy, N, D, K, A, X, ldx, t0, t1)
+#define VMP_CASE_F(db, kt)                                                                      \
+    if (form1 && !guard && DB == db && KT == kt) {                                              \
+        if (lay == 3) VMP_XPF(db, kt, (db == 2 && kt == 4 ? 1 : 2), 3);                         \
+        else VMP_XPF(db, kt, (db == 2 && kt == 4 ? 1 : 2), 1);                                  \
+    } else
+        VMP_CASE_F(1, 1) VMP_CASE_F(2, 1) VMP_CASE_F(4, 1) VMP_CASE_F(8, 1) VMP_CASE_F(1, 2)
+        VMP_CASE_F(2, 2) VMP_CASE_F(4, 2) VMP_CASE_F(1, 4) VMP_CASE_F(2, 4)
 #define VMP_CASE(db, kt)                                                                        \
     if (DB == db && KT == kt) {                                                                 \
         if (guard) VMP_XP(db, kt, true, 2, 0, 0);                                               \
@@ -761,6 +797,8 @@
             return VMP_ERR_UNSUPPORTED;
         }
 #undef VMP_CASE
+#undef VMP_CASE_F
+#undef VMP_XPF
 #undef VMP_XP4
 #undef VMP_XP
         VMP_HIP_CHECK(ctx, hipGetLastError());
@@ -786,6 +824,24 @@
     const int64_t whole = (d.N + TN - 1) / TN * TN;
     const bool exact = (d.D == L.DP && d.K == L.KP);
     return (d.lay || (exact && d.ldy >= whole && d.ldx >= whole)) ? whole : d.N;
+}
+
+double *reserve_xpass_A(vmp_ctx *ctx, int D, int K, void *workspace)
+{
+    vmp_pca_layout L;
+    fill_layout(D, K, &L);
+    ctx->x_prefilled = nullptr;
+    if (!vmp_tune_get("plate_stream", env_int("VMP_PCA_PLATE_STREAM", 1, 0, 1))) return nullptr;
+    if (vmp_tune_get("pca_fork_copy", env_int("VMP_PCA_FORK_COPY", 0, 0, 1))) return nullptr;
+    if (D != L.DP || K != L.KP) return nullptr;
+    if (ensure_plate_stream(ctx) != VMP_OK) return nullptr;
+    const int b = (int)(ctx->x_count & 1);
+    if (ctx->x_buf_pending[b]) {
+        if (hipStreamWaitEvent(ctx->stream, ctx->ev_xbuf[b], 0) != hipSuccess) return nullptr;
+        ctx->x_buf_pending[b] = 0;
+    }
+    ctx->x_prefilled = plate_stream_A(ctx, L, workspace) + (int64_t)b * L.KP * L.DP;
+    return ctx->x_prefilled;
 }
 
 bool xpass_supersedes(const vmp_xpass_desc &d, const vmp_xpass_desc &old)
@@ -821,13 +877,17 @@
         const int b = (int)(ctx->x_count & 1);
         ctx->x_count += 1;
         double *Ax = plate_stream_A(ctx, L, workspace) + (int64_t)b * L.KP * L.DP;
-        if (ctx->x_buf_pending[b]) {
-            VMP_HIP_CHECK(ctx, hipStreamWaitEvent(m, ctx->ev_xbuf[b], 0));
-            ctx->x_buf_pending[b] = 0;
-        }
-        VMP_HIP_CHECK(ctx, hipMemcpyAsync(Ax, state + L.off_A,
-                                          (size_t)(L.KP * L.DP) * sizeof(double),
-                                          hipMemcpyDeviceToDevice, m));
+        const bool prefilled = ctx->x_prefilled == Ax;
+        ctx->x_prefilled = nullptr;
+        if (!prefilled) {
+            if (ctx->x_buf_pending[b]) {
+                VMP_HIP_CHECK(ctx, hipStreamWaitEvent(m, ctx->ev_xbuf[b], 0));
+                ctx->x_buf_pending[b] = 0;
+            }
+            VMP_HIP_CHECK(ctx, hipMemcpyAsync(Ax, state + L.off_A,
+                                              (size_t)(L.KP * L.DP) * sizeof(double),
+                                              hipMemcpyDeviceToDevice, m));
+        }
         VMP_HIP_CHECK(ctx, hipEventRecord(ctx->ev_xfork, m));
         VMP_HIP_CHECK(ctx, hipStreamWaitEvent(ctx->xs, ctx->ev_xfork, 0));
         d.A = Ax;
@@ -846,6 +906,7 @@
 int32_t run_xpass(vmp_ctx *ctx, const double *Y, int64_t ldy, int64_t N, int D, int K, double *X,
                   int64_t ldx, double *state, void *workspace, int lay)
 {
+    ctx->x_prefilled = nullptr;
     int32_t rc = issue_xpass(ctx, Y, ldy, N, D, K, X, ldx, state, workspace, lay);
     if (rc != VMP_OK) return rc;
     vmp_pca_layout L;
@@ -1199,16 +1260,21 @@
         head_wide = hipEventQuery(ctx->ev_xdone) == hipSuccess;
         (void)hipGetLastError();
     }
+    ctx->x_prefilled = nullptr;
     for (int i = 0; i < n; ++i) {
         const double *stop = i == 0 ? nullptr : ctx->sweep_ctl;
         const bool last = i + 1 == n;
+        const bool own_head = !ticket || i == 0;
+        const bool mid = ticket && !last;
+        const bool fills = last ? own_head : (mid && i + 2 == n);
+        double *Ax = fills ? reserve_xpass_A(ctx, D, K, workspace) : nullptr;
         if (i == 0 && head_wide) {
             rc = vmp_pca_launch_sweep_head_wide(ctx, D, K, n_total, x_prec, a0_tau, b0_tau, a0_alpha,
-                                                b0_alpha, state);
+                                                b0_alpha, state, last ? Ax : nullptr);
             if (rc != VMP_OK) return rc;
-        } else if (!ticket || i == 0) {
+        } else if (own_head) {
             rc = vmp_pca_launch_sweep_head(ctx, D, K, n_total, x_prec, a0_tau, b0_tau, a0_alpha,
-                                           b0_alpha, state, stop);
+                                           b0_alpha, state, stop, last ? Ax : nullptr);
             if (rc != VMP_OK) return rc;
         }
         if (last) {
@@ -1219,11 +1285,11 @@
         }
         t.slot = ring + (int64_t)i * VMP_PCA_SWEEP_SLOT;
         t.first = i == 0;
-        if (ticket && !last) {
+        if (mid) {
             rc = vmp_pca_launch_sweep_mid(ctx, D, K, n_total, x_prec, a0_tau, b0_tau, a0_alpha,
                                           b0_alpha, state, P, t, ctx->sweep_tickets + i,
                                           stamps ? ctx->sweep_stamps + (size_t)i * VMP_SWEEP_NSTAMP
-                                                 : nullptr, stamp_level);
+                                                 : nullptr, stamp_level, Ax);
             if (rc != VMP_OK) return rc;
             ctx->sweep_mid_launches += 1;
         } else {
diff --git a/bayespy_amd/csrc/vmp_pca_small.hip b/bayespy_amd/csrc/vmp_pca_small.hip
--- a/bayespy_amd/csrc/vmp_pca_small.hip
+++ b/bayespy_amd/csrc/vmp_pca_small.hip
@@ -15,6 +15,13 @@
     double n_total, x_prec, a0t, b0t, a0a, b0a;
     int has_mean;
 };
+
+template <int NTQ>
+__device__ __forceinline__ void copy_A_for_pass(const vmp_pca_layout &L, const double *st, double *Ax)
+{
+    const int n = (int)(L.KP * L.DP);
+    for (int e = threadIdx.x; e < n; e += NTQ) Ax[e] = st[L.off_A + e];
+}
 
 __device__ inline double ww_centred(const small_args &a, const double *st, int k)
 {
@@ -475,7 +482,7 @@
 }
 
 template <int KP>
-__device__ __forceinline__ void pca_head_body(const small_args &a, double *st)
+__device__ __forceinline__ void pca_head_body(const small_args &a, double *st, double *Ax = nullptr)
 {
     constexpr int LDM = KP + 1, E = KP * KP / NTF, RB = 32;
     __shared__ double M[KP * LDM];
@@ -666,7 +673,10 @@
 #pragma unroll
                     for (int r = 0; r < 4; ++r) {
                         const int k = tk * 16 + l4 + 4 * r, d = b * RB + td * 16 + l15;
-                        if (k < K && d < D) st[L.off_A + k * DP + d] = tau * acc[r];
+                        if (k < K && d < D) {
+                            st[L.off_A + k * DP + d] = tau * acc[r];
+                            if (Ax) Ax[k * DP + d] = tau * acc[r];
+                        }
                     }
                 }
             }
@@ -681,10 +691,13 @@
 
 template <int KP>
 __global__ void __launch_bounds__(NTF, 5)
-pca_head_fast_kernel(small_args a, double *st, const double *stop)
-{
-    if (stop && stop[VMP_SWEEP_STOP] != 0.0) return;
-    pca_head_body<KP>(a, st);
+pca_head_fast_kernel(small_args a, double *st, const double *stop, double *Ax)
+{
+    if (stop && stop[VMP_SWEEP_STOP] != 0.0) {
+        if (Ax) copy_A_for_pass<NTF>(a.L, st, Ax);
+        return;
+    }
+    pca_head_body<KP>(a, st, Ax);
 }
 
 constexpr int GB = 32;
@@ -1264,7 +1277,7 @@
 __device__ __forceinline__ void pca_head_wide(const small_args &a, double *st, double *M, double *T,
                                               const double *alm, double tau, double *SW,
                                               const STAMP &stamp, const SIDE &side = SIDE(),
-                                              const double *stopw = nullptr)
+                                              const double *stopw = nullptr, double *Ax = nullptr)
 {
     constexpr bool DEFER = !std::is_same<SIDE, no_side>::value;
     constexpr int LDM = KP + 1, E = KP * KP / NTF, KT = KP / 16;
@@ -1301,7 +1314,10 @@
     stamp(SP_H_LAMBDA);
     if constexpr (DEFER) {
         sweep_inverse<KP>(M, K, &logdet, &bad, side);
-        if (*stopw != 0.0) return;
+        if (*stopw != 0.0) {
+            if (Ax) copy_A_for_pass<NTF>(a.L, st, Ax);
+            return;
+        }
     } else {
         sweep_inverse<KP>(M, K, &logdet, &bad);
     }
@@ -1386,7 +1402,10 @@
 #pragma unroll
             for (int r = 0; r < 4; ++r) {
                 const int k = tk * 16 + l4 + 4 * r, d = td * 16 + l15;
-                if (k < K && d < D) st[L.off_A + k * DP + d] = tau * acc[r];
+                if (k < K && d < D) {
+                    st[L.off_A + k * DP + d] = tau * acc[r];
+                    if (Ax) Ax[k * DP + d] = tau * acc[r];
+                }
             }
         }
     }
@@ -1406,7 +1425,7 @@
 template <int KP, class STAMP>
 __device__ __forceinline__ void pca_sweep_mid_body(const small_args &a, double *st,
                                                    const vmp_sweep_tail &sw, unsigned int *ticket,
-                                                   const double *sf, const STAMP &stamp)
+                                                   const double *sf, const STAMP &stamp, double *Ax)
 {
     extern __shared__ __align__(16) double gl[];
     __shared__ tail_lds<KP> ts;
@@ -1416,6 +1435,7 @@
             sw.slot[7] = 0.0;
             sw.ctl[VMP_SWEEP_SKIPPED] += 1.0;
         }
+        if (Ax && blockIdx.x == 0) copy_A_for_pass<NTF>(a.L, st, Ax);
         return;
     }
     stamp(SP_ENTRY);
@@ -1444,34 +1464,35 @@
     sweep_tail_wide<KP>(a, st, sw, ts, SW, gl, stamp);
     __syncthreads();
     const defer_side<KP, STAMP> side{a, st, sw, ts, sf, stamp};
-    pca_head_wide<KP>(a, st, ts.Cx, ts.Sx, ts.al + 2 * KP, ts.sc[2], SW, stamp, side, &ts.stop);
+    pca_head_wide<KP>(a, st, ts.Cx, ts.Sx, ts.al + 2 * KP, ts.sc[2], SW, stamp, side, &ts.stop, Ax);
 }
 
 template <int KP>
 __global__ void __launch_bounds__(NTF)
 pca_sweep_mid_kernel(small_args a, double *st, double *P, vmp_sweep_tail sw, unsigned int *ticket,
-                     const double *sf)
-{
-    pca_sweep_mid_body<KP>(a, st, sw, ticket, sf, stamps_off());
+                     const double *sf, double *Ax)
+{
+    pca_sweep_mid_body<KP>(a, st, sw, ticket, sf, stamps_off(), Ax);
 }
 
 template <int KP>
 __global__ void __launch_bounds__(NTF)
 pca_sweep_mid_stamped_kernel(small_args a, double *st, double *P, vmp_sweep_tail sw,
-                             unsigned int *ticket, const double *sf, unsigned long long *out, int level)
+                             unsigned int *ticket, const double *sf, unsigned long long *out, int level,
+                             double *Ax)
 {
     __shared__ unsigned long long stl[VMP_SWEEP_NSTAMP];
     if (threadIdx.x < VMP_SWEEP_NSTAMP) stl[threadIdx.x] = 0;
     __syncthreads();
     const stamps_on stamp{stl, level};
-    pca_sweep_mid_body<KP>(a, st, sw, ticket, sf, stamp);
+    pca_sweep_mid_body<KP>(a, st, sw, ticket, sf, stamp, Ax);
     if (threadIdx.x == 0 && stl[SP_T_LOADS] != 0)
         for (int i = 0; i < VMP_SWEEP_NSTAMP; ++i) out[i] = stl[i];
 }
 
 template <int KP>
 __global__ void __launch_bounds__(NTF)
-pca_head_wide_kernel(small_args a, double *st)
+pca_head_wide_kernel(small_args a, double *st, double *Ax)
 {
     constexpr int LDM = KP + 1, E = KP * KP / NTF, NW = FAST_D * KP / NTF;
     __shared__ __align__(16) double M[KP * LDM], T[KP * LDM], SW[FAST_D * LDM], alm[KP];
@@ -1506,7 +1527,7 @@
         if (e < nsw) SW[(e / KP) * LDM + (e % KP)] = wy[j];
     }
     __syncthreads();
-    pca_head_wide<KP>(a, st, M, T, alm, tau, SW, stamps_off());
+    pca_head_wide<KP>(a, st, M, T, alm, tau, SW, stamps_off(), no_side(), nullptr, Ax);
 }
 
 __global__ void __launch_bounds__(64)
@@ -1643,10 +1664,10 @@
         if (o0 == VMP_PCA_OP_W && o1 == VMP_PCA_OP_XPREP) {
             if (fast && a.L.KP == 16)
                 hipLaunchKernelGGL(pca_head_fast_kernel<16>, dim3(1), dim3(NTF), 0, ctx->stream, a,
-                                   state, (const double *)nullptr);
+                                   state, (const double *)nullptr, (double *)nullptr);
             else if (fast)
                 hipLaunchKernelGGL(pca_head_fast_kernel<32>, dim3(1), dim3(NTF), 0, ctx->stream, a,
-                                   state, (const double *)nullptr);
+                                   state, (const double *)nullptr, (double *)nullptr);
             else
                 launch_sequence<VMP_PCA_OP_W, VMP_PCA_OP_XPREP, 0>(ctx, a, state);
             i += 2;
@@ -1707,15 +1728,15 @@
 
 int32_t vmp_pca_launch_sweep_head(vmp_ctx *ctx, int32_t D, int32_t K, int64_t n_total, double x_prec,
                                   double a0t, double b0t, double a0a, double b0a, double *state,
-                                  const double *stop)
+                                  const double *stop, double *Ax)
 {
     small_args a;
     const int32_t rc = fill_small_args(ctx, a, D, K, n_total, x_prec, a0t, b0t, a0a, b0a);
     if (rc != VMP_OK) return rc;
     if (a.L.KP == 16)
-        hipLaunchKernelGGL(pca_head_fast_kernel<16>, dim3(1), dim3(NTF), 0, ctx->stream, a, state, stop);
+        hipLaunchKernelGGL(pca_head_fast_kernel<16>, dim3(1), dim3(NTF), 0, ctx->stream, a, state, stop, Ax);
     else
-        hipLaunchKernelGGL(pca_head_fast_kernel<32>, dim3(1), dim3(NTF), 0, ctx->stream, a, state, stop);
+        hipLaunchKernelGGL(pca_head_fast_kernel<32>, dim3(1), dim3(NTF), 0, ctx->stream, a, state, stop, Ax);
     VMP_HIP_CHECK(ctx, hipGetLastError());
     return VMP_OK;
 }
@@ -1774,7 +1795,7 @@
 template <int KP>
 static int32_t launch_mid(vmp_ctx *ctx, const small_args &a, double *state, double *P,
                           const vmp_sweep_tail &t, unsigned int *ticket, unsigned long long *stamps,
-                          int stamp_level)
+                          int stamp_level, double *Ax)
 {
     VMP_REQUIRE(ctx, ctx->sweep_sf, VMP_ERR_INVALID,
                 "the one-launch sweep needs vmp_pca_sweep_constants first");
@@ -1791,10 +1812,10 @@
     const dim3 nb((unsigned)(a.L.DP / GRA));
     if (stamps)
         hipLaunchKernelGGL(pca_sweep_mid_stamped_kernel<KP>, nb, dim3(NTF), lds, ctx->stream, a, state,
-                           P, t, ticket, (const double *)ctx->sweep_sf, stamps, stamp_level);
+                           P, t, ticket, (const double *)ctx->sweep_sf, stamps, stamp_level, Ax);
     else
         hipLaunchKernelGGL(pca_sweep_mid_kernel<KP>, nb, dim3(NTF), lds, ctx->stream, a, state, P, t,
-                           ticket, (const double *)ctx->sweep_sf);
+                           ticket, (const double *)ctx->sweep_sf, Ax);
     VMP_HIP_CHECK(ctx, hipGetLastError());
     return VMP_OK;
 }
@@ -1802,13 +1823,13 @@
 int32_t vmp_pca_launch_sweep_mid(vmp_ctx *ctx, int32_t D, int32_t K, int64_t n_total, double x_prec,
                                  double a0t, double b0t, double a0a, double b0a, double *state,
                                  double *P, const vmp_sweep_tail &t, unsigned int *ticket,
-                                 unsigned long long *stamps, int32_t stamp_level)
+                                 unsigned long long *stamps, int32_t stamp_level, double *Ax)
 {
     small_args a;
     const int32_t rc = fill_small_args(ctx, a, D, K, n_total, x_prec, a0t, b0t, a0a, b0a);
     if (rc != VMP_OK) return rc;
-    if (a.L.KP == 16) return launch_mid<16>(ctx, a, state, P, t, ticket, stamps, stamp_level);
-    return launch_mid<32>(ctx, a, state, P, t, ticket, stamps, stamp_level);
+    if (a.L.KP == 16) return launch_mid<16>(ctx, a, state, P, t, ticket, stamps, stamp_level, Ax);
+    return launch_mid<32>(ctx, a, state, P, t, ticket, stamps, stamp_level, Ax);
 }
 
 int32_t vmp_pca_sweep_constants(vmp_ctx *ctx, int32_t D, int32_t K, int64_t n_total, double x_prec,
@@ -1831,15 +1852,15 @@
 
 int32_t vmp_pca_launch_sweep_head_wide(vmp_ctx *ctx, int32_t D, int32_t K, int64_t n_total,
                                        double x_prec, double a0t, double b0t, double a0a, double b0a,
-                                       double *state)
+                                       double *state, double *Ax)
 {
     small_args a;
     const int32_t rc = fill_small_args(ctx, a, D, K, n_total, x_prec, a0t, b0t, a0a, b0a);
     if (rc != VMP_OK) return rc;
     if (a.L.KP == 16)
-        hipLaunchKernelGGL(pca_head_wide_kernel<16>, dim3(1), dim3(NTF), 0, ctx->stream, a, state);
+        hipLaunchKernelGGL(pca_head_wide_kernel<16>, dim3(1), dim3(NTF), 0, ctx->stream, a, state, Ax);
     else
-        hipLaunchKernelGGL(pca_head_wide_kernel<32>, dim3(1), dim3(NTF), 0, ctx->stream, a, state);
+        hipLaunchKernelGGL(pca_head_wide_kernel<32>, dim3(1), dim3(NTF), 0, ctx->stream, a, state, Ax);
     VMP_HIP_CHECK(ctx, hipGetLastError());
     return VMP_OK;
 }
```

New measurement: 28660 (median of 6 runs). Within noise of the previous version (+1.4%).
